# arunsethuraman/multiclust

Measured on AMD Instinct MI355X. Metric: EM iterations/sec, IxLxK admixture, higher is better.
Workload: dtype f64; 1 GPU; c3: 10000 diploid x 100000 loci, M_l~U{2,3,4}, admixture K=8, SQUAREM-3 (-s 3); I=10000, L=100000, T=300302, ploidy=2, K=8, accel_scheme=3, units=1 initialisation(s), one per GPU

## Files before the change

multiclust_amd/csrc/mchip.hip:

```cpp
#include "mchip_context.h"
#include "mchip_finalize.h"

#include <math.h>
#include <stdio.h>
#include <stdlib.h>
#include <string.h>
#include <sys/syscall.h>
#include <unistd.h>

mchip_progress_slot mchip_progress_slots[MCHIP_PROGRESS_SLOTS];
std::atomic<unsigned long long> mchip_progress_events{0};
static std::atomic<int> progress_next_slot{0};

mchip_progress_slot *mchip_progress_my_slot(void)
{
	static thread_local mchip_progress_slot *mine = nullptr;
	if (!mine) {
		int x = progress_next_slot.fetch_add(1, std::memory_order_relaxed);
		if (x >= MCHIP_PROGRESS_SLOTS) x = MCHIP_PROGRESS_SLOTS - 1;
		mine = &mchip_progress_slots[x];
		mine->tid.store((long)syscall(SYS_gettid), std::memory_order_relaxed);
	}
	return mine;
}

#define DECL_KT(n) const mchip_ktable *mchip_ktable_get_##n();
DECL_KT(1) DECL_KT(2) DECL_KT(3) DECL_KT(4) DECL_KT(5) DECL_KT(6) DECL_KT(7) DECL_KT(8)
DECL_KT(9) DECL_KT(10) DECL_KT(11) DECL_KT(12) DECL_KT(13) DECL_KT(14) DECL_KT(15) DECL_KT(16)
DECL_KT(17) DECL_KT(18) DECL_KT(19) DECL_KT(20) DECL_KT(21) DECL_KT(22) DECL_KT(23) DECL_KT(24)
DECL_KT(25) DECL_KT(26) DECL_KT(27) DECL_KT(28) DECL_KT(29) DECL_KT(30) DECL_KT(31) DECL_KT(32)
DECL_KT(33) DECL_KT(34) DECL_KT(35) DECL_KT(36) DECL_KT(37) DECL_KT(38) DECL_KT(39) DECL_KT(40)
DECL_KT(41) DECL_KT(42) DECL_KT(43) DECL_KT(44) DECL_KT(45) DECL_KT(46) DECL_KT(47) DECL_KT(48)
DECL_KT(49) DECL_KT(50) DECL_KT(51) DECL_KT(52) DECL_KT(53) DECL_KT(54) DECL_KT(55) DECL_KT(56)
DECL_KT(57) DECL_KT(58) DECL_KT(59) DECL_KT(60) DECL_KT(61) DECL_KT(62) DECL_KT(63) DECL_KT(64)

const mchip_ktable *mchip_get_ktable(int K)
{
	typedef const mchip_ktable *(*getter)();
	static const getter tabs[MCHIP_MAX_K + 1] = {
		nullptr,
		mchip_ktable_get_1, mchip_ktable_get_2, mchip_ktable_get_3, mchip_ktable_get_4, mchip_ktable_get_5, mchip_ktable_get_6, mchip_ktable_get_7, mchip_ktable_get_8,
		mchip_ktable_get_9, mchip_ktable_get_10, mchip_ktable_get_11, mchip_ktable_get_12, mchip_ktable_get_13, mchip_ktable_get_14, mchip_ktable_get_15, mchip_ktable_get_16,
		mchip_ktable_get_17, mchip_ktable_get_18, mchip_ktable_get_19, mchip_ktable_get_20, mchip_ktable_get_21, mchip_ktable_get_22, mchip_ktable_get_23, mchip_ktable_get_24,
		mchip_ktable_get_25, mchip_ktable_get_26, mchip_ktable_get_27, mchip_ktable_get_28, mchip_ktable_get_29, mchip_ktable_get_30, mchip_ktable_get_31, mchip_ktable_get_32,
		mchip_ktable_get_33, mchip_ktable_get_34, mchip_ktable_get_35, mchip_ktable_get_36, mchip_ktable_get_37, mchip_ktable_get_38, mchip_ktable_get_39, mchip_ktable_get_40,
		mchip_ktable_get_41, mchip_ktable_get_42, mchip_ktable_get_43, mchip_ktable_get_44, mchip_ktable_get_45, mchip_ktable_get_46, mchip_ktable_get_47, mchip_ktable_get_48,
		mchip_ktable_get_49, mchip_ktable_get_50, mchip_ktable_get_51, mchip_ktable_get_52, mchip_ktable_get_53, mchip_ktable_get_54, mchip_ktable_get_55, mchip_ktable_get_56,
		mchip_ktable_get_57, mchip_ktable_get_58, mchip_ktable_get_59, mchip_ktable_get_60, mchip_ktable_get_61, mchip_ktable_get_62, mchip_ktable_get_63, mchip_ktable_get_64,
	};
	static_assert(MCHIP_MAX_K == 64, "one kernel translation unit per K (Makefile: KS)");
	return (K >= 1 && K <= MCHIP_MAX_K) ? tabs[K]() : nullptr;
}

static void read_knobs(mchip_context *ctx)
{
	auto on = [](const char *name) { return getenv(name) != nullptr ? 1 : 0; };
	auto num = [](const char *name, int dflt) { const char *e = getenv(name); return (e && atoi(e) > 0) ? atoi(e) : dflt; };
	ctx->knob.no_bial = on("MCHIP_NO_BIAL");
	ctx->knob.no_counts = on("MCHIP_NO_COUNTS");
	ctx->knob.force_dense = on("MCHIP_FORCE_DENSE");
	ctx->knob.force_safe = on("MCHIP_FORCE_SAFE");
	ctx->knob.no_graph = on("MCHIP_NO_GRAPH");
	ctx->knob.no_dual = on("MCHIP_NO_DUAL");
	ctx->knob.no_slab_sum = on("MCHIP_NO_SLAB_SUM");
	ctx->knob.no_fused_finalize = on("MCHIP_NO_FUSED_FINALIZE");
	ctx->knob.no_pair = on("MCHIP_NO_PAIR");
	ctx->knob.no_col_split = on("MCHIP_NO_COL_SPLIT");
	ctx->knob.part_no_tile = on("MCHIP_PART_NO_TILE");
	ctx->knob.sim_no_tile = on("MCHIP_SIM_NO_TILE");
	const int both = num("MCHIP_BLOCKS_PER_CU", 64);
	ctx->knob.per_cu_col = num("MCHIP_BLOCKS_PER_CU_COL", both);
	ctx->knob.per_cu_ind = num("MCHIP_BLOCKS_PER_CU_IND", both);
	const char *f = getenv("MCHIP_SLAB_FRAC");
	ctx->knob.slab_frac = (f && atof(f) > 0) ? atof(f) : 0.3;
	ctx->knob.no_roundup = on("MCHIP_NO_CHUNK_ROUNDUP");
	ctx->knob.geometry_given = on("MCHIP_BLOCKS_PER_CU") || on("MCHIP_BLOCKS_PER_CU_COL") || on("MCHIP_SLAB_FRAC");
}


constexpr int RT_I = 64;

__global__ __launch_bounds__(256) void k_relayout(const uint8_t *__restrict__ raw, int I, int L, int pl, const int32_t *__restrict__ ua,
			   int limit, uint8_t *gtA, uint8_t *gtS, int n_ltiles, int RT_L, int *bad)
{
	extern __shared__ __attribute__((aligned(16))) uint8_t tile[];
	const int rowb = RT_L * pl;
	const int l0 = (blockIdx.x % n_ltiles) * RT_L, i0 = (blockIdx.x / n_ltiles) * RT_I;
	int flags = 0;
	const int roww = rowb / 4;
	const bool words = ((((size_t)L * pl) | ((size_t)l0 * pl) | (size_t)raw) & 3) == 0 && l0 + RT_L <= L;
	for (int x = threadIdx.x; x < RT_I * roww; x += 256) {
		const int r = x / roww, w = x % roww;
		const int i = i0 + r;
		uint32_t v4 = 0xFFFFFFFFu;
		if (i < I) {
			const uint8_t *src = raw + ((size_t)i * L + l0) * pl + (size_t)w * 4;
			if (words) {
				v4 = *reinterpret_cast<const uint32_t *>(src);
			} else {
				v4 = 0;
				for (int y = 0; y < 4; y++) {
					const int l = l0 + (w * 4 + y) / pl;
					const uint32_t v = l < L ? src[y] : 0xFFu;
					v4 |= v << (8 * y);
				}
			}
			for (int y = 0; y < 4; y++) {
				const int l = l0 + (w * 4 + y) / pl;
				const uint32_t v = (v4 >> (8 * y)) & 0xFFu;
				if (l >= L) continue;
				const int lim = ua ? ua[l] : limit;
				if (v != 0xFFu && (int)v >= lim) flags |= 1;
				if (v == 0xFFu) flags |= 2;
			}
		}
		reinterpret_cast<uint32_t *>(tile)[x] = v4;
	}
	if (flags) atomicOr(bad, flags);
	__syncthreads();
	const int grp = 8 * pl, grpw = 2 * pl;
	for (int x = threadIdx.x; x < (RT_I / 8) * RT_L * grpw; x += 256) {
		const int w = x % grpw, ll = (x / grpw) % RT_L, ibl = x / (grpw * RT_L);
		const int l = l0 + ll;
		const size_t ib = (size_t)(i0 / 8) + ibl;
		if (l >= L || ib * 8 >= (size_t)I) continue;
		uint32_t v4 = 0;
		for (int y = 0; y < 4; y++) {
			const int e = w * 4 + y, j = e / pl, a = e % pl;
			v4 |= (uint32_t)tile[(ibl * 8 + j) * rowb + ll * pl + a] << (8 * y);
		}
		reinterpret_cast<uint32_t *>(gtA + (ib * L + l) * (size_t)grp)[w] = v4;
	}
	for (int x = threadIdx.x; x < (RT_L / 8) * RT_I * grpw; x += 256) {
		const int w = x % grpw, r = (x / grpw) % RT_I, lbl = x / (grpw * RT_I);
		const int i = i0 + r;
		const size_t lb = (size_t)(l0 / 8) + lbl;
		if (i >= I || lb * 8 >= (size_t)L) continue;
		reinterpret_cast<uint32_t *>(gtS + (lb * I + i) * (size_t)grp)[w] = reinterpret_cast<const uint32_t *>(tile + r * rowb + lbl * grp)[w];
	}
}

static int launch_relayout(hipStream_t stream, const uint8_t *raw, int I, int L, int pl, const int32_t *ua, int limit,
			   uint8_t *gtA, uint8_t *gtS, int *bad)
{
	int RT_L = 64;
	while (RT_L > 8 && RT_I * RT_L * pl > 32 * 1024) RT_L -= 8;
	const int n_ltiles = (L + RT_L - 1) / RT_L, n_itiles = (I + RT_I - 1) / RT_I;
	const size_t blocks = (size_t)n_ltiles * n_itiles;
	if (blocks >= ((size_t)1 << 31) || (size_t)RT_I * RT_L * pl > 64 * 1024) return -1;
	hipLaunchKernelGGL(k_relayout, dim3((unsigned)blocks), dim3(256), (size_t)RT_I * RT_L * pl, stream, raw, I, L, pl, ua, limit, gtA, gtS,
			   n_ltiles, RT_L, bad);
	return 0;
}

template <int PLT>
__global__ __launch_bounds__(256) void k_center_distance(const uint8_t *__restrict__ gtS, int I, int L, int pl_rt, int K,
		const int32_t *__restrict__ centers, int chunk_groups, int tile_groups, uint32_t *__restrict__ part)
{
	extern __shared__ uint32_t cd_lds[];
	const int pl = PLT ? PLT : pl_rt, nthr = blockDim.x, tid = threadIdx.x, grp = 8 * pl;
	uint32_t *acc = cd_lds;
	uint32_t *cen32 = acc + (size_t)K * nthr;
	const uint8_t *cen = reinterpret_cast<const uint8_t *>(cen32);
	uint8_t *own = reinterpret_cast<uint8_t *>(cen32 + (size_t)tile_groups * K * 2 * pl);
	const int i = blockIdx.x * nthr + tid;
	const bool live = i < I;
	const int n_groups = (L + 7) >> 3;
	const int g_begin = blockIdx.y * chunk_groups, g_end = n_groups - g_begin < chunk_groups ? n_groups : g_begin + chunk_groups;
	for (int k = 0; k < K; k++) acc[k * nthr + tid] = 0;
	for (int g0 = g_begin; g0 < g_end; g0 += tile_groups) {
		const int ng = g_end - g0 < tile_groups ? g_end - g0 : tile_groups;
		__syncthreads();
		for (int x = tid; x < ng * K * 2 * pl; x += nthr) {
			const int w = x % (2 * pl), k = (x / (2 * pl)) % K, g = x / (2 * pl * K);
			cen32[x] = reinterpret_cast<const uint32_t *>(gtS + ((size_t)(g0 + g) * I + centers[k]) * grp)[w];
		}
		__syncthreads();
		if (!live) continue;
		for (int g = 0; g < ng; g++) {
			const uint8_t *src = gtS + ((size_t)(g0 + g) * I + i) * grp;
			if constexpr (PLT > 0) {
				unsigned long long run[PLT ? PLT : 1];
#pragma unroll
				for (int x = 0; x < PLT; x++) run[x] = reinterpret_cast<const unsigned long long *>(src)[x];
				for (int k = 0; k < K; k++) {
					unsigned long long crun[PLT ? PLT : 1];
#pragma unroll
					for (int x = 0; x < PLT; x++) crun[x] = reinterpret_cast<const unsigned long long *>(cen + (size_t)(g * K + k) * grp)[x];
					int d = 0;
#pragma unroll
					for (int t = 0; t < 8; t++) {
						unsigned used = 0;
#pragma unroll
						for (int b = 0; b < PLT; b++) {
							const int at = t * PLT + b;
							d += ((unsigned)(crun[at >> 3] >> (8 * (at & 7))) & 0xFFu) != MCHIP_MISSING;
						}
#pragma unroll
						for (int a = 0; a < PLT; a++) {
							const int at = t * PLT + a;
							const unsigned gi = (unsigned)(run[at >> 3] >> (8 * (at & 7))) & 0xFFu;
							const bool obs = gi != MCHIP_MISSING;
							bool found = false;
#pragma unroll
							for (int b = 0; b < PLT; b++) {
								const int bt = t * PLT + b;
								const unsigned cb = (unsigned)(crun[bt >> 3] >> (8 * (bt & 7))) & 0xFFu;
								const bool hit = obs && !found && !((used >> b) & 1u) && cb == gi;
								used |= (unsigned)hit << b;
								found = found || hit;
							}
							d += (int)obs - 2 * (int)found;
						}
					}
					acc[k * nthr + tid] += (uint32_t)d;
				}
			} else {
				for (int t = 0; t < 8; t++) {
					for (int a = 0; a < pl; a++) own[a * nthr + tid] = src[t * pl + a];
// ... 73 lines not shown
					for (int y = 0; y < 4; y++) {
						const uint32_t mb = (v4 >> (8 * y)) & 0xFFu;
						const int l = g * 8 + (w * 4 + y) / pl;
						if (mb == MCHIP_MISSING || l >= t1) continue;
						const int c = toff[l] + (int)mb;
						if (tile) atomicAdd(&cc_lds[(size_t)(c - col0) * K + k], 1u);
						else atomicAdd(&cnt[(size_t)c * K + k], 1u);
					}
				}
			}
		if (tile) {
			__syncthreads();
			for (int x = threadIdx.x; x < nwords; x += 256)
				if (cc_lds[x]) atomicAdd(&cnt[(size_t)col0 * K + x], cc_lds[x]);
			__syncthreads();
		}
	}
}

__global__ void k_center_finish(int I, int L, int K, const int32_t *__restrict__ toff, const uint32_t *__restrict__ cnt,
		const uint32_t *__restrict__ nk, double *__restrict__ eta, double *__restrict__ P)
{
	const size_t idx = (size_t)blockIdx.x * blockDim.x + threadIdx.x;
	if (idx < (size_t)K) eta[idx] = (double)(1u + nk[idx]) / (double)(I + K);
	if (idx >= (size_t)K * L) return;
	const int k = (int)(idx % K), l = (int)(idx / K);
	const int c0 = toff[l], M = toff[l + 1] - c0;
	double temp = 0.0;
	for (int m = 0; m < M; m++) temp += 1.0 + (double)(K - k) * (double)cnt[(size_t)(c0 + m) * K + k];
	for (int m = 0; m < M; m++) P[(size_t)(c0 + m) * K + k] = (1.0 + (double)(K - k) * (double)cnt[(size_t)(c0 + m) * K + k]) / temp;
}

__global__ __launch_bounds__(256) void k_assign_by_centers(const uint8_t *__restrict__ gtA, int I, int L, int pl, int K,
		const uint8_t *__restrict__ centers, const unsigned long long *__restrict__ draw_offset,
		const uint8_t *__restrict__ draws, unsigned long long n_draws, uint8_t *raw, int *bad)
{
	const int l = blockIdx.x * 256 + threadIdx.x;
	if (l >= L) return;
	uint8_t cen[MCHIP_MAX_K];
	for (int k = 0; k < K; k++) cen[k] = centers[(size_t)l * K + k];
	unsigned long long next = draw_offset[l];
	for (int ib = 0; ib < (I + 7) / 8; ib++) {
		const uint8_t *src = gtA + ((size_t)ib * L + l) * 8 * (size_t)pl;
		for (int j = 0; j < 8; j++) {
			const int i = ib * 8 + j;
			if (i >= I) break;
			for (int b = 0; b < pl; b++) {
				const uint8_t g = src[j * pl + b];
				int kk = -1;
				if (g != MCHIP_MISSING)
					for (int k = 0; k < K; k++) {
						if (cen[k] == 0xFF) break;
						if (cen[k] == g) { kk = k; break; }
					}
				if (kk < 0) {
					if (K == 1) kk = 0;
					else if (next < n_draws) kk = draws[next++];
					else { kk = 0; atomicOr(bad, 1); }
				}
				raw[((size_t)i * L + l) * pl + b] = (uint8_t)kk;
			}
		}
	}
}

__global__ void k_unlayout(const uint8_t *__restrict__ gtA, int I, int L, int pl, uint8_t *raw)
{
	const size_t n = (size_t)I * L * pl, stride = (size_t)gridDim.x * blockDim.x;
	for (size_t idx = (size_t)blockIdx.x * blockDim.x + threadIdx.x; idx < n; idx += stride) {
		size_t r = idx;
		const int a = (int)(r % pl); r /= pl;
		const int l = (int)(r % L);
		const size_t i = r / L;
		raw[idx] = gtA[(((i >> 3) * L + l) * 8 + (i & 7)) * (size_t)pl + a];
	}
}

template <int BITS>
__global__ void k_build_counts(const uint8_t *__restrict__ gtA, int I, int L, int pl, int T,
			       const int32_t *__restrict__ col_locus, const uint8_t *__restrict__ col_allele, uint4 *gtC)
{
	constexpr int PERWORD = 32 / BITS, G = 4 * PERWORD;
	const size_t idx = (size_t)blockIdx.x * blockDim.x + threadIdx.x;
	const size_t ngroups = (size_t)(I + G - 1) / G;
	if (idx >= ngroups * T) return;
	const int c = (int)(idx % T);
	const size_t g = idx / T;
	const int l = col_locus[c];
	const unsigned m = col_allele[c];
	unsigned out[4] = {0, 0, 0, 0};
	for (int x = 0; x < G; x++) {
		const size_t i = g * G + x;
		if (i >= (size_t)I) break;
		const uint8_t *src = gtA + (((i >> 3) * L + l) * 8 + (i & 7)) * (size_t)pl;
		unsigned n = 0;
		for (int b = 0; b < pl; b++) n += (src[b] == m);
		out[x / PERWORD] |= n << (BITS * (x % PERWORD));
	}
	gtC[idx] = make_uint4(out[0], out[1], out[2], out[3]);
}

__global__ __launch_bounds__(256) void k_count_cells(const uint8_t *__restrict__ gtA, int I, int L, int pl, int T,
		const int32_t *__restrict__ col_locus, const uint8_t *__restrict__ col_allele, unsigned long long *out)
{
	__shared__ unsigned red[2][256];
	const size_t n = (size_t)((I + 7) / 8) * T, stride = (size_t)gridDim.x * 256;
	unsigned cells = 0, copies = 0;
	for (size_t idx = (size_t)blockIdx.x * 256 + threadIdx.x; idx < n; idx += stride) {
		const int c = (int)(idx % T);
		const size_t ib = idx / T;
		const int l = col_locus[c];
		const unsigned m = col_allele[c];
		const uint8_t *src = gtA + (ib * L + l) * 8 * (size_t)pl;
		for (int j = 0; j < 8; j++) {
			unsigned cnt = 0;
			for (int b = 0; b < pl; b++) cnt += (src[j * pl + b] == m);
			cells += cnt != 0;
			copies += cnt;
		}
	}
	red[0][threadIdx.x] = cells;
	red[1][threadIdx.x] = copies;
	__syncthreads();
	for (int w = 128; w > 0; w >>= 1) {
		if ((int)threadIdx.x < w) {
			red[0][threadIdx.x] += red[0][threadIdx.x + w];
			red[1][threadIdx.x] += red[1][threadIdx.x + w];
		}
		__syncthreads();
	}
	if (threadIdx.x == 0) {
		atomicAdd(&out[0], (unsigned long long)red[0][0]);
		atomicAdd(&out[1], (unsigned long long)red[1][0]);
	}
}

__global__ void k_transpose_kt_to_tk(const double *__restrict__ src, double *__restrict__ dst, int K, int T)
{
	const size_t idx = (size_t)blockIdx.x * blockDim.x + threadIdx.x;
	if (idx >= (size_t)K * T) return;
	const int k = (int)(idx % K);
	const size_t c = idx / K;
	dst[idx] = src[(size_t)k * T + c];
}
__global__ void k_transpose_tk_to_kt(const double *__restrict__ src, double *__restrict__ dst, int K, int T)
{
	const size_t idx = (size_t)blockIdx.x * blockDim.x + threadIdx.x;
	if (idx >= (size_t)K * T) return;
	const size_t c = idx % T;
	const int k = (int)(idx / T);
	dst[idx] = src[c * K + k];
}

__device__ __forceinline__ double ordered_sum(double acc, const double *__restrict__ in, size_t first, size_t stride, int count)
{
	int x = 0;
	for (; x + 8 <= count; x += 8) {
		double v[8];
#pragma unroll
		for (int y = 0; y < 8; y++) v[y] = in[first + (size_t)(x + y) * stride];
#pragma unroll
		for (int y = 0; y < 8; y++) acc += v[y];
	}
	for (; x < count; x++) acc += in[first + (size_t)x * stride];
	return acc;
}

__device__ __forceinline__ double block_ordered_sum(const double *__restrict__ in, int n, double *red)
{
	const double s = (int)threadIdx.x < n ? ordered_sum(0.0, in, threadIdx.x, MCHIP_BLOCK, (n - (int)threadIdx.x + MCHIP_BLOCK - 1) / MCHIP_BLOCK) : 0.0;
	red[threadIdx.x] = s;
	__syncthreads();
	for (int w = MCHIP_BLOCK / 2; w > 0; w >>= 1) {
		if ((int)threadIdx.x < w) red[threadIdx.x] += red[threadIdx.x + w];
		__syncthreads();
	}
	const double v = red[0];
	__syncthreads();
	return v;
}
__global__ __launch_bounds__(MCHIP_BLOCK) void k_reduce_sum(const double *__restrict__ in, int n, double *out, const int *stop = nullptr)
{
	__shared__ double red[MCHIP_BLOCK];
	if (stop && *stop) return;
	const double v = block_ordered_sum(in, n, red);
	if (threadIdx.x == 0) *out = v;
}
__global__ __launch_bounds__(MCHIP_BLOCK) void k_reduce_accept(const double *__restrict__ in1, const double *__restrict__ in2, int n, double *sc,
		int *cyc, const int *stop)
{
	__shared__ double red[MCHIP_BLOCK];
	if (stop && *stop) return;
	if (in1) {
		const double v = block_ordered_sum(in1, n, red);
		if (threadIdx.x == 0) sc[1] = v;
	}
	const double v2 = block_ordered_sum(in2, n, red);
	if (threadIdx.x == 0) {
		sc[2] = v2;
		cyc[1] = (!cyc[0] && sc[2] > sc[1]) ? 1 : 0;
	}
}

__global__ __launch_bounds__(MCHIP_BLOCK) void k_reduce_dots(const double *__restrict__ part_q, int gq, const double *__restrict__ part_p, int gp,
		int nout, double *sc, const int *stop)
{
	__shared__ double red[MCHIP_BLOCK];
	if (stop && *stop) return;
	const int x = blockIdx.x;
	const double *in = x < nout ? part_q + (size_t)x * gq : part_p + (size_t)(x - nout) * gp;
	const int n = x < nout ? gq : gp;
	double *out = x < nout ? sc + 16 + x : sc + 20 + (x - nout);
	const double v = block_ordered_sum(in, n, red);
	if (threadIdx.x == 0) *out = v;
}

__global__ __launch_bounds__(MCHIP_BLOCK) void k_sum_slabs(const double *__restrict__ slabs, int n_slabs, size_t n, double *out,
		const int *stop)
{
	__shared__ double part[8][32];
	if (stop && *stop) return;
	const int e_local = threadIdx.x & 31, s = threadIdx.x >> 5;
	const size_t e = (size_t)blockIdx.x * 32 + e_local;
	double acc = 0.0;
	if (e < n && s < n_slabs) acc = ordered_sum(0.0, slabs, (size_t)s * n + e, 8 * n, (n_slabs - s + 7) / 8);
	part[s][e_local] = acc;
	__syncthreads();
	if (s == 0 && e < n) {
		double t = part[0][e_local];
#pragma unroll
		for (int x = 1; x < 8; x++) t += part[x][e_local];
		out[e] = t;
	}
}


__global__ __launch_bounds__(MCHIP_BLOCK) void k_finalize_p(int L, int K, int T, const int32_t *__restrict__ toff,
		int n_ichunks, const double *__restrict__ Apart, const double *Pfrom, double *Pto,
		int weighted, double add_lb, int do_projection, double lb, uint8_t *flags, const int *stop = nullptr)
{
	const size_t idx = (size_t)blockIdx.x * MCHIP_BLOCK + threadIdx.x;
	if (idx >= (size_t)L * K || (stop && *stop)) return;
	const int k = (int)(idx % K);
	const int l = (int)(idx / K);
	const int c0 = toff[l], M = toff[l + 1] - c0;
	double temp = 0.0;
	if (M <= 8) {
		double v[8];
#pragma unroll
		for (int m = 0; m < 8; m++) {
			v[m] = 0.0;
			if (m < M) {
				const size_t e = (size_t)(c0 + m) * K + k;
				double s = ordered_sum(0.0, Apart, e, (size_t)T * K, n_ichunks);
				if (weighted) s *= Pfrom[e];
				s += add_lb;
				v[m] = s;
				temp += s;
			}
		}
#pragma unroll
		for (int m = 0; m < 8; m++)
			if (m < M) v[m] /= temp;
		if (do_projection) michelot_small(v, M, lb);
#pragma unroll
		for (int m = 0; m < 8; m++)
			if (m < M) Pto[(size_t)(c0 + m) * K + k] = v[m];
		return;
	}
	for (int m = 0; m < M; m++) {
		const size_t e = (size_t)(c0 + m) * K + k;
		double s = ordered_sum(0.0, Apart, e, (size_t)T * K, n_ichunks);
		if (weighted) s *= Pfrom[e];
		s += add_lb;
		Pto[e] = s;
		temp += s;
	}
	for (int m = 0; m < M; m++) Pto[(size_t)(c0 + m) * K + k] /= temp;
	if (do_projection) michelot_strided(Pto + (size_t)c0 * K + k, K, M, lb, flags ? flags + (size_t)c0 * K + k : nullptr);
}

__global__ __launch_bounds__(MCHIP_BLOCK) void k_finalize_p_tile(int L, int K, int T, const int32_t *__restrict__ toff, int loci_per_block,
		int n_slabs, const double *__restrict__ Apart, const double *Pfrom, double *Pto,
		int weighted, double add_lb, int do_projection, double lb, const int *stop = nullptr)
{
	__shared__ double tile[FP_TILE];
	if (stop && *stop) return;
	finalize_p_tile_body(blockIdx.x, tile, L, K, T, toff, loci_per_block, n_slabs, Apart, Pfrom, Pto, weighted, add_lb, do_projection, lb);
}

static int finalize_p_loci(int K, int max_M)
{
	if (max_M > 64 || max_M < 1) return 0;
	const int n = FP_TILE / (max_M * K);
	return n >= 4 ? n : 0;
}

__global__ __launch_bounds__(MCHIP_BLOCK) void k_project_p(int L, int K, const int32_t *__restrict__ toff, double *P,
		double lb, uint8_t *flags, const int *stop = nullptr)
{
	const size_t idx = (size_t)blockIdx.x * MCHIP_BLOCK + threadIdx.x;
	if (idx >= (size_t)L * K || (stop && *stop)) return;
	const int k = (int)(idx % K);
	const int l = (int)(idx / K);
	const int c0 = toff[l], M = toff[l + 1] - c0;
	if (M <= 8) {
		double v[8];
#pragma unroll
		for (int m = 0; m < 8; m++) v[m] = m < M ? P[(size_t)(c0 + m) * K + k] : 0.0;
		michelot_small(v, M, lb);
#pragma unroll
		for (int m = 0; m < 8; m++)
			if (m < M) P[(size_t)(c0 + m) * K + k] = v[m];
		return;
	}
	michelot_strided(P + (size_t)c0 * K + k, K, M, lb, flags ? flags + (size_t)c0 * K + k : nullptr);
}

__global__ __launch_bounds__(MCHIP_BLOCK) void k_column_sums(const double *__restrict__ sik, int I, int K, double *out, const int *stop = nullptr)
{
	__shared__ double red[MCHIP_BLOCK];
	if (stop && *stop) return;
	const int k = blockIdx.x;
	double s = 0.0;
	for (int i = threadIdx.x; i < I; i += MCHIP_BLOCK) s += sik[(size_t)i * K + k];
	red[threadIdx.x] = s;
	__syncthreads();
	for (int w = MCHIP_BLOCK / 2; w > 0; w >>= 1) {
		if ((int)threadIdx.x < w) red[threadIdx.x] += red[threadIdx.x + w];
		__syncthreads();
	}
	if (threadIdx.x == 0) out[k] = red[0];
}
__global__ void k_normalize_row(const double *__restrict__ sums, int K, double *eta, const int *stop = nullptr, double add = 0.0)
{
	if (threadIdx.x || blockIdx.x || (stop && *stop)) return;
	double temp = 0.0;
	for (int k = 0; k < K; k++) temp += sums[k] + add;
	for (int k = 0; k < K; k++) eta[k] = (sums[k] + add) / temp;
}

__global__ void k_logp(const double *__restrict__ p, double *__restrict__ out, size_t n, int skip_zero, const int *stop = nullptr)
{
	const size_t idx = (size_t)blockIdx.x * blockDim.x + threadIdx.x;
	if (idx >= n || (stop && *stop)) return;
	const double v = p[idx];
	out[idx] = (skip_zero && v == 0.0) ? 0.0 : log(v);
}

__global__ __launch_bounds__(MCHIP_BLOCK) void k_stop_check(mchip_run_state *s, double *ll, const double *__restrict__ part = nullptr, int n = 0)
{
	__shared__ double red[MCHIP_BLOCK];
	if (s->stopped) return;
	if (part) {
		const double acc = (int)threadIdx.x < n ? ordered_sum(0.0, part, threadIdx.x, MCHIP_BLOCK, (n - (int)threadIdx.x + MCHIP_BLOCK - 1) / MCHIP_BLOCK) : 0.0;
		red[threadIdx.x] = acc;
		__syncthreads();
		for (int w = MCHIP_BLOCK / 2; w > 0; w >>= 1) {
			if ((int)threadIdx.x < w) red[threadIdx.x] += red[threadIdx.x + w];
			__syncthreads();
		}
		if (threadIdx.x == 0) *ll = red[0];
	}
	if (threadIdx.x) return;
	const double loglik = part ? red[0] : *ll;
	s->n_iter++;
	if (loglik != loglik) {
		s->fatal = 1;
		s->bad_loglik = loglik;
		s->stopped = 1;
		return;
	}
	int stop;
	if (s->max_iter && s->n_iter > s->max_iter) {
		s->iter_stop = 1;
		stop = 1;
	} else {
		double abs_diff = 0, rel_diff = 0;
		stop = 1;
		if (s->abs_error != 0) abs_diff = fabs(loglik - s->logL);
		if (s->rel_error != 0) rel_diff = abs_diff / fabs(s->logL);
		if (s->abs_error != 0 && abs_diff > s->abs_error) stop = 0;
		if (s->rel_error != 0 && rel_diff > s->rel_error) stop = 0;
		if (stop) s->converged = 1;
	}
	s->stopped = stop;
	if (loglik < s->logL && !stop) {
		s->fatal = 2;
		s->bad_loglik = loglik;
		s->stopped = 1;
		return;
	}
	s->logL = loglik;
}

__global__ void k_diff(const double *__restrict__ a, const double *__restrict__ b, double *out, size_t n, const int *stop = nullptr)
{
	const size_t idx = (size_t)blockIdx.x * blockDim.x + threadIdx.x;
	if (stop && *stop) return;
	if (idx < n) out[idx] = a[idx] - b[idx];
}

__global__ __launch_bounds__(MCHIP_BLOCK) void k_dots(const double *__restrict__ u, const double *__restrict__ v,
		const double *__restrict__ u2, size_t n, int mode, double *part, const int *stop = nullptr)
{
	__shared__ double red[3][MCHIP_BLOCK];
	if (stop && *stop) return;
	double s0 = 0, s1 = 0, s2 = 0;
	for (size_t x = (size_t)blockIdx.x * MCHIP_BLOCK + threadIdx.x; x < n; x += (size_t)gridDim.x * MCHIP_BLOCK) {
		if (mode == 0) {
			const double uu = u[x], d = v[x] - uu;
			s0 += uu * uu; s1 += uu * d; s2 += d * d;
		} else {
			const double uu = u[x];
			s0 += uu * u2[x]; s1 += uu * v[x];
		}
	}
	red[0][threadIdx.x] = s0; red[1][threadIdx.x] = s1; red[2][threadIdx.x] = s2;
	__syncthreads();
	for (int w = MCHIP_BLOCK / 2; w > 0; w >>= 1) {
		if ((int)threadIdx.x < w) {
			red[0][threadIdx.x] += red[0][threadIdx.x + w];
			red[1][threadIdx.x] += red[1][threadIdx.x + w];
			red[2][threadIdx.x] += red[2][threadIdx.x + w];
		}
		__syncthreads();
	}
	if (threadIdx.x == 0) {
		part[blockIdx.x] = red[0][0];
		part[gridDim.x + blockIdx.x] = red[1][0];
		part[2 * gridDim.x + blockIdx.x] = red[2][0];
	}
}

__device__ __forceinline__ void dots_slots_body(const double *__restrict__ x0, const double *__restrict__ x1, const double *__restrict__ x2,
		size_t n, double *part, unsigned bid, unsigned gdim, double (*red)[MCHIP_BLOCK])
{
	double s0 = 0, s1 = 0, s2 = 0;
	for (size_t x = (size_t)bid * MCHIP_BLOCK + threadIdx.x; x < n; x += (size_t)gdim * MCHIP_BLOCK) {
		const double uu = x1[x] - x0[x], vv = x2[x] - x1[x];
		const double d = vv - uu;
		s0 += uu * uu; s1 += uu * d; s2 += d * d;
	}
	red[0][threadIdx.x] = s0; red[1][threadIdx.x] = s1; red[2][threadIdx.x] = s2;
	__syncthreads();
	for (int w = MCHIP_BLOCK / 2; w > 0; w >>= 1) {
		if ((int)threadIdx.x < w) {
			red[0][threadIdx.x] += red[0][threadIdx.x + w];
			red[1][threadIdx.x] += red[1][threadIdx.x + w];
			red[2][threadIdx.x] += red[2][threadIdx.x + w];
		}
		__syncthreads();
	}
	if (threadIdx.x == 0) {
		part[bid] = red[0][0];
		part[gdim + bid] = red[1][0];
		part[2 * gdim + bid] = red[2][0];
	}
}
__global__ __launch_bounds__(MCHIP_BLOCK) void k_dots_slots(const double *__restrict__ q0, const double *__restrict__ q1,
		const double *__restrict__ q2, size_t nq, double *part_q, unsigned gq, const double *__restrict__ p0,
		const double *__restrict__ p1, const double *__restrict__ p2, size_t np, double *part_p, const int *stop)
{
	__shared__ double red[3][MCHIP_BLOCK];
	if (stop && *stop) return;
	if (blockIdx.x < gq) dots_slots_body(q0, q1, q2, nq, part_q, blockIdx.x, gq, red);
	else dots_slots_body(p0, p1, p2, np, part_p, blockIdx.x - gq, gridDim.x - gq, red);
}
__global__ void k_accel_update_slots(const double *__restrict__ q0, const double *q1, const double *__restrict__ q2, double *qout, size_t nq,
				     const double *__restrict__ p0, const double *p1, const double *__restrict__ p2, double *pout, size_t np,
				     int qn_form, const double *s_dev, const int *stop)
{
#pragma clang fp contract(off)
	size_t idx = (size_t)blockIdx.x * blockDim.x + threadIdx.x;
	if (idx >= nq + np || (stop && *stop)) return;
	const double *x0 = q0, *x1 = q1, *x2 = q2;
	double *out = qout;
	if (idx >= nq) { idx -= nq; x0 = p0; x1 = p1; x2 = p2; out = pout; }
	const double s = *s_dev;
	const double u = x1[idx] - x0[idx], v = x2[idx] - x1[idx];
	if (qn_form) out[idx] = x0[idx] + u + s * v;
	else out[idx] = x0[idx] - 2 * s * u + s * s * (v - u);
}

__global__ void k_accel_update(const double *__restrict__ base, const double *__restrict__ u, const double *__restrict__ v,
			       double *out, size_t n, double s, int qn_form, const double *s_dev = nullptr, const int *stop = nullptr)
{
#pragma clang fp contract(off)
	const size_t idx = (size_t)blockIdx.x * blockDim.x + threadIdx.x;
	if (idx >= n || (stop && *stop)) return;
	if (s_dev) s = *s_dev;
	if (qn_form) out[idx] = base[idx] + u[idx] + s * v[idx];
	else out[idx] = base[idx] - 2 * s * u[idx] + s * s * (v[idx] - u[idx]);
}
__global__ void k_axpy2(const double *__restrict__ v, double *out, size_t n, double ca, double cb)
{
#pragma clang fp contract(off)
	const size_t idx = (size_t)blockIdx.x * blockDim.x + threadIdx.x;
	if (idx < n) out[idx] += v[idx] * ca * cb;
}
__global__ void k_add(const double *__restrict__ a, const double *__restrict__ b, double *out, size_t n)
{
	const size_t idx = (size_t)blockIdx.x * blockDim.x + threadIdx.x;
	if (idx < n) out[idx] = a[idx] + b[idx];
}

__device__ __forceinline__ void step_size_body(double *sc, int scheme, int *cyc)
{
	const double utu = sc[16] + sc[20], utvu = sc[17] + sc[21], vutvu = sc[18] + sc[22];
	double s;
	if (scheme == 1) s = utu / utvu;
	else if (scheme == 2) s = utvu / vutvu;
	else if (scheme == 3) s = (sqrt(utu) < 1e-8) ? (double)NAN : -sqrt(utu / vutvu);
	else s = -utu / utvu;
	if (scheme < 4 && s > -1) s = -1;
	sc[24] = s;
	cyc[0] = (s != s || s - s != 0.0) ? 1 : 0;
}
__global__ __launch_bounds__(MCHIP_BLOCK) void k_reduce_dots_step(const double *__restrict__ part_q, int gq, const double *__restrict__ part_p,
		int gp, double *sc, int scheme, int *cyc, const int *stop)
{
	__shared__ double red[MCHIP_BLOCK];
	if (stop && *stop) return;
	for (int x = 0; x < 6; x++) {
		const double *in = x < 3 ? part_q + (size_t)x * gq : part_p + (size_t)(x - 3) * gp;
		const int n = x < 3 ? gq : gp;
		const double v = block_ordered_sum(in, n, red);
		if (threadIdx.x == 0) sc[(x < 3 ? 16 : 20) + (x % 3)] = v;
	}
	if (threadIdx.x == 0) step_size_body(sc, scheme, cyc);
}
__global__ void k_accept(const double *sc, int *cyc, const int *stop)
{
	if (threadIdx.x || blockIdx.x || (stop && *stop)) return;
	cyc[1] = (!cyc[0] && sc[2] > sc[1]) ? 1 : 0;
}

__global__ void k_select_copy(double *qdst, const double *__restrict__ q_if_accepted, const double *__restrict__ q_otherwise, size_t nq,
			      double *pdst, const double *__restrict__ p_if_accepted, const double *__restrict__ p_otherwise, size_t np,
			      const int *cyc, const int *stop)
{
	size_t idx = (size_t)blockIdx.x * blockDim.x + threadIdx.x;
	if (idx >= nq + np || (stop && *stop)) return;
	if (idx < nq) qdst[idx] = cyc[1] ? q_if_accepted[idx] : q_otherwise[idx];
	else { idx -= nq; pdst[idx] = cyc[1] ? p_if_accepted[idx] : p_otherwise[idx]; }
}

int check_slot(mchip_context *ctx, int slot)
{
	if (!ctx) return MCHIP_ERR_INVALID;
	if (!ctx->K) return fail(ctx, MCHIP_ERR_STATE, "no model set%s", nullptr);
	if (slot < 0 || slot > 2) return fail(ctx, MCHIP_ERR_INVALID, "slot out of range%s", nullptr);
	return MCHIP_OK;
}

static void prof_mark(mchip_context *ctx, int kind, bool start)
{
	if (!ctx->profiling) return;
	if (ctx->ev_used >= ctx->ev_pool.size()) {
		hipEvent_t e;
		if (hipEventCreate(&e) != hipSuccess) return;
		ctx->ev_pool.push_back(e);
	}
	(void)hipEventRecord(ctx->ev_pool[ctx->ev_used++], ctx->stream);
	if (start) ctx->ev_kind.push_back(kind);
}

constexpr size_t PAIR_SPAN_CHUNK = 1024;
constexpr int PAIR_SPAN_THREADS = 1024;
__global__ __launch_bounds__(PAIR_SPAN_THREADS) void k_pair_spans(const unsigned long long *__restrict__ marks, unsigned n_blocks, mchip_pair_runs runs,
								  mchip_pair_span *out)
{
	__shared__ unsigned long long red[4][PAIR_SPAN_THREADS];
	unsigned long long lo[2] = { ~0ull, ~0ull }, hi[2] = { 0ull, 0ull };
	for (unsigned r = threadIdx.x; r < n_blocks / MCHIP_PAIR_RUN; r += PAIR_SPAN_THREADS) {
		unsigned logical;
		const int kind = mchip_pair_is_ind(r * MCHIP_PAIR_RUN, runs, &logical) ? 1 : 0;
#pragma unroll
		for (int x = 0; x < MCHIP_PAIR_RUN; x++) {
			const size_t b = (size_t)r * MCHIP_PAIR_RUN + x;
			const unsigned long long t0 = marks[2 * b], t1 = marks[2 * b + 1];
			if (t0 > t1) continue;
			lo[kind] = t0 < lo[kind] ? t0 : lo[kind];
			hi[kind] = t1 > hi[kind] ? t1 : hi[kind];
		}
	}
	red[0][threadIdx.x] = lo[0]; red[1][threadIdx.x] = lo[1]; red[2][threadIdx.x] = hi[0]; red[3][threadIdx.x] = hi[1];
	__syncthreads();
	for (int s = PAIR_SPAN_THREADS / 2; s > 0; s >>= 1) {
		if ((int)threadIdx.x < s) {
			for (int x = 0; x < 2; x++) {
				const unsigned long long l2 = red[x][threadIdx.x + s], h2 = red[2 + x][threadIdx.x + s];
				if (l2 < red[x][threadIdx.x]) red[x][threadIdx.x] = l2;
				if (h2 > red[2 + x][threadIdx.x]) red[2 + x][threadIdx.x] = h2;
			}
		}
		__syncthreads();
	}
	if (threadIdx.x == 0) {
		out->start[0] = red[0][0]; out->start[1] = red[1][0];
		out->end[0] = red[2][0]; out->end[1] = red[3][0];
	}
}

static int pair_profile_slot(mchip_context *ctx, const mchip_pass_args &a, unsigned long long **marks)
{
	mchip_pair_runs runs;
	const size_t n_blocks = ctx->kt->pair_blocks(a, &runs);
	if (n_blocks > ctx->pair_marks_cap) {
		HIPCHK(hipStreamSynchronize(ctx->stream));
		dfree(ctx->d_pair_marks);
		ctx->pair_marks_cap = 0;
		HIPCHK(hipMalloc((void **)&ctx->d_pair_marks, 2 * n_blocks * sizeof(unsigned long long)));
		ctx->pair_marks_cap = n_blocks;
	}
	if (ctx->pair_used / PAIR_SPAN_CHUNK >= ctx->pair_spans.size()) {
		mchip_pair_span *chunk = nullptr;
		HIPCHK(hipMalloc((void **)&chunk, PAIR_SPAN_CHUNK * sizeof(mchip_pair_span)));
		ctx->pair_spans.push_back(chunk);
	}
	*marks = ctx->d_pair_marks;
	return MCHIP_OK;
}

static void drop_graphs(mchip_context *ctx)
{
	for (int s = 0; s < 3; s++)
		if (ctx->step_graph[s]) { (void)MCHIP_WAIT(hipGraphExecDestroy(ctx->step_graph[s])); ctx->step_graph[s] = nullptr; }
	for (int s = 0; s < 3; s++)
		for (int m = 0; m < 5; m++)
			if (ctx->cycle_graph[s][m]) { (void)MCHIP_WAIT(hipGraphExecDestroy(ctx->cycle_graph[s][m])); ctx->cycle_graph[s][m] = nullptr; }
}

void free_model(mchip_context *ctx)
{
	drop_graphs(ctx);
	for (int s = 0; s < 3; s++) { dfree(ctx->d_p[s]); dfree(ctx->d_q[s]); }
	for (int s = 0; s < MCHIP_MAX_SECANTS; s++) { dfree(ctx->d_up[s]); dfree(ctx->d_vp[s]); dfree(ctx->d_uq[s]); dfree(ctx->d_vq[s]); }
	dfree(ctx->d_sik); dfree(ctx->d_stage); dfree(ctx->d_logp); dfree(ctx->d_Apart); dfree(ctx->d_Spart); dfree(ctx->d_llpart); dfree(ctx->d_llpart2);
	dfree(ctx->d_redpart); dfree(ctx->d_flags);
	ctx->K = 0;
	ctx->parked_K = 0;
	ctx->kt = nullptr;
	ctx->have_ll = 0;
	ctx->s_cache_slot = -1;
}

void drop_saved(saved_set &set)
{
	dfree(set.d_raw);
	set.L = 0;
	set.ua.clear();
	set.empty.clear();
}

void free_data(mchip_context *ctx, int keep)
{
	drop_cv(ctx);
	drop_generators(ctx);
	if (!(keep & KEEP_RS_BASE)) drop_saved(ctx->rs_base);
	dfree(ctx->d_ua); dfree(ctx->d_toff); dfree(ctx->d_col_locus); dfree(ctx->d_col_allele);
	dfree(ctx->d_gtA); dfree(ctx->d_gtS); dfree(ctx->d_gtC); dfree(ctx->d_asA); dfree(ctx->d_asS);
	dfree(ctx->d_initA); dfree(ctx->d_initS);
	dfree(ctx->d_draw);
	dfree(ctx->d_cand_span); dfree(ctx->d_cand_centers); dfree(ctx->d_cand_off);
	ctx->cand_span_bytes = ctx->cand_loci = ctx->cand_center_bytes = 0;
	dfree(ctx->d_cen_part); dfree(ctx->d_cen_work);
	ctx->cen_part_bytes = ctx->cen_work_bytes = 0;
	ctx->init_geno_set = 0;
	ctx->h_ua.clear();
	ctx->I = ctx->L = ctx->T = 0;
}

static mchip_pass_args pass_args(mchip_context *ctx, int slot)
{
	mchip_pass_args a;
	memset(&a, 0, sizeof a);
	a.I = ctx->I; a.L = ctx->L; a.T = ctx->T; a.ploidy = ctx->ploidy; a.K = ctx->K;
	a.gtA = ctx->d_gtA; a.gtS = ctx->d_gtS; a.gtC = ctx->d_gtC; a.count_bits = ctx->count_bits; a.has_missing = ctx->has_missing;
	a.ua = ctx->d_ua; a.toff = ctx->d_toff; a.col_locus = ctx->d_col_locus; a.col_allele = ctx->d_col_allele;
	a.P = ctx->d_p[slot]; a.Q = ctx->d_q[slot]; a.qstride = ctx->qstride;
	a.ichunk = ctx->ichunk; a.n_ichunks = ctx->n_ichunks; a.Apart = ctx->d_Apart; a.llpart = ctx->d_llpart;
	a.flush_blocks = ctx->flush_blocks;
	a.safe_rcp = ctx->safe_rcp;
	a.lchunk = ctx->lchunk; a.n_lchunks = ctx->n_lchunks; a.Spart = ctx->d_Spart;
	a.asA = ctx->d_asA; a.asS = ctx->d_asS;
	a.sparse = ctx->sparse; a.tile_cols = 8 * ctx->max_M;
	a.biallelic = (ctx->min_M == 2 && ctx->max_M == 2 && !ctx->knob.no_bial) ? 1 : 0;
	a.ind_waves = ctx->ind_waves;
	a.xcd_rows = ctx->xcd_rows;
	a.no_col_split = ctx->knob.no_col_split;
	return a;
}

static void launch_finalize_p(mchip_context *ctx, int n_slabs, const double *slabs, int from, int to, int weighted, double add_lb,
			      int do_projection, const int *stop)
{
	const int per = finalize_p_loci(ctx->K, ctx->max_M);
	if (per)
		hipLaunchKernelGGL(k_finalize_p_tile, dim3((ctx->L + per - 1) / per), dim3(MCHIP_BLOCK), 0, ctx->stream,
				   ctx->L, ctx->K, ctx->T, ctx->d_toff, per, n_slabs, slabs, ctx->d_p[from], ctx->d_p[to],
				   weighted, add_lb, do_projection, ctx->p_lb, stop);
	else
		hipLaunchKernelGGL(k_finalize_p, dim3(nblk((size_t)ctx->L * ctx->K)), dim3(MCHIP_BLOCK), 0, ctx->stream,
				   ctx->L, ctx->K, ctx->T, ctx->d_toff, n_slabs, slabs, ctx->d_p[from], ctx->d_p[to],
				   weighted, add_lb, do_projection, ctx->p_lb, ctx->d_flags, stop);
}

extern "C" {

int mchip_abi_version(void) { return MCHIP_ABI_VERSION; }

int mchip_device_count(int *count)
{
	MCHIP_ENTRY();
	if (!count) return MCHIP_ERR_INVALID;
	int n = 0;
	if (MCHIP_WAIT(hipGetDeviceCount(&n)) != hipSuccess) n = 0;
	*count = n;
	return MCHIP_OK;
}

int mchip_create(mchip_context **out, int device)
{
	MCHIP_ENTRY();
	if (!out) return MCHIP_ERR_INVALID;
	*out = nullptr;
	int n = 0;
	if (MCHIP_WAIT(hipGetDeviceCount(&n)) != hipSuccess || n <= 0) return MCHIP_ERR_NO_DEVICE;
	if (device < 0 || device >= n) return MCHIP_ERR_INVALID;
	mchip_context *ctx = new mchip_context();
	ctx->first_empty = -1;
	ctx->cv_fold = -1;
	ctx->device = device;
	ctx->err[0] = 0;
	ctx->ind_waves = 1;
	read_knobs(ctx);
	if (MCHIP_WAIT(hipSetDevice(device)) != hipSuccess || MCHIP_WAIT(hipStreamCreateWithFlags(&ctx->stream, hipStreamNonBlocking)) != hipSuccess) {
		delete ctx;
		return MCHIP_ERR_HIP;
	}
	hipDeviceProp_t prop;
	ctx->n_cu = (MCHIP_WAIT(hipGetDeviceProperties(&prop, device)) == hipSuccess) ? prop.multiProcessorCount : 256;
	if (MCHIP_WAIT(hipHostMalloc((void **)&ctx->h_pinned, 64 * sizeof(double), hipHostMallocDefault)) != hipSuccess ||
	    MCHIP_WAIT(hipMalloc((void **)&ctx->d_scalars, 64 * sizeof(double))) != hipSuccess ||
	    MCHIP_WAIT(hipMalloc((void **)&ctx->d_run, sizeof(mchip_run_state))) != hipSuccess ||
	    MCHIP_WAIT(hipMalloc((void **)&ctx->d_cyc, 4 * sizeof(int))) != hipSuccess ||
	    MCHIP_WAIT(hipEventCreate(&ctx->ev_begin)) != hipSuccess || MCHIP_WAIT(hipEventCreate(&ctx->ev_end)) != hipSuccess) {
		delete ctx;
		return MCHIP_ERR_ALLOC;
	}
	*out = ctx;
	return MCHIP_OK;
}

int mchip_destroy(mchip_context *ctx)
{
	MCHIP_ENTRY();
	if (!ctx) return MCHIP_OK;
	(void)MCHIP_WAIT(hipSetDevice(ctx->device));
	(void)MCHIP_WAIT(hipStreamSynchronize(ctx->stream));
	free_model(ctx);
	free_data(ctx);
	dfree(ctx->d_scalars);
	dfree(ctx->d_cyc);
	dfree(ctx->d_run);
	if (ctx->h_pinned) (void)MCHIP_WAIT(hipHostFree(ctx->h_pinned));
	for (hipEvent_t e : ctx->ev_pool) (void)MCHIP_WAIT(hipEventDestroy(e));
	dfree(ctx->d_pair_marks);
	for (mchip_pair_span *&chunk : ctx->pair_spans) dfree(chunk);
	(void)MCHIP_WAIT(hipEventDestroy(ctx->ev_begin));
	(void)MCHIP_WAIT(hipEventDestroy(ctx->ev_end));
	(void)MCHIP_WAIT(hipStreamDestroy(ctx->stream));
	delete ctx;
	return MCHIP_OK;
}

const char *mchip_last_error(const mchip_context *ctx) { return ctx ? ctx->err : "null context"; }

int mchip_synchronize(mchip_context *ctx)
{
	MCHIP_ENTRY();
	if (!ctx) return MCHIP_ERR_INVALID;
	HIPCHK(hipStreamSynchronize(ctx->stream));
	return MCHIP_OK;
}

int mchip_device_info(mchip_context *ctx, char *name, int name_len, int *compute_units, double *hbm_bytes)
{
	MCHIP_ENTRY();
	if (!ctx) return MCHIP_ERR_INVALID;
	hipDeviceProp_t prop;
	HIPCHK(hipGetDeviceProperties(&prop, ctx->device));
	if (name && name_len > 0) snprintf(name, name_len, "%s (%s)", prop.name, prop.gcnArchName);
	if (compute_units) *compute_units = prop.multiProcessorCount;
	if (hbm_bytes) *hbm_bytes = (double)prop.totalGlobalMem;
	return MCHIP_OK;
}

}

static int set_shape_impl(mchip_context *ctx, int I, int L, int ploidy, const int32_t *ua, int keep)
{
	if (I <= 0 || L <= 0 || ploidy <= 0 || ploidy > 64 || !ua)
		return fail(ctx, MCHIP_ERR_INVALID, "set_genotypes: bad shape or null pointer%s", nullptr);
	read_knobs(ctx);
	HIPCHK(hipSetDevice(ctx->device));
	HIPCHK(hipStreamSynchronize(ctx->stream));
	drop_cv(ctx);
	if (!(keep & KEEP_RS_BASE)) drop_saved(ctx->rs_base);
	if (ctx->T && ctx->I == I && ctx->L == L && ctx->ploidy == ploidy && (int)ctx->h_ua.size() == L &&
	    !memcmp(ctx->h_ua.data(), ua, sizeof(int32_t) * (size_t)L)) {
		if (ctx->K) ctx->parked_K = ctx->K;
		ctx->K = 0;
		ctx->have_ll = 0;
		ctx->s_cache_slot = -1;
		if (!(keep & KEEP_INIT)) ctx->init_geno_set = 0;
		return MCHIP_OK;
	}
	free_model(ctx);
	free_data(ctx, keep);

	std::vector<int32_t> toff(L + 25);
	toff[0] = 0;
	int maxM = 0, minM = 1 << 30;
	for (int l = 0; l < L; l++) {
		if (ua[l] < minM) minM = ua[l];
		if (ua[l] < 0 || ua[l] > 255) return fail(ctx, MCHIP_ERR_INVALID, "uniquealleles[l] must be in [0,255]%s", nullptr);
		if ((long long)toff[l] + ua[l] > 2000000000LL) return fail(ctx, MCHIP_ERR_INVALID, "too many allele columns%s", nullptr);
		toff[l + 1] = toff[l] + ua[l];
		if (ua[l] > maxM) maxM = ua[l];
	}
	const int T = toff[L];
	for (int x = L + 1; x < L + 25; x++) toff[x] = T;
	if (T <= 0) return fail(ctx, MCHIP_ERR_INVALID, "no alleles%s", nullptr);
	std::vector<int32_t> col_locus(T);
	std::vector<uint8_t> col_allele(T);
	for (int l = 0; l < L; l++)
		for (int m = 0; m < ua[l]; m++) {
			col_locus[toff[l] + m] = l;
			col_allele[toff[l] + m] = (uint8_t)m;
		}
	ctx->I = I; ctx->L = L; ctx->ploidy = ploidy; ctx->T = T; ctx->max_M = maxM; ctx->min_M = minM;
	ctx->h_ua.assign(ua, ua + L);
	ctx->geno_bytes_A = (size_t)((I + 7) / 8) * L * 8 * ploidy;
	ctx->geno_bytes_S = (size_t)((L + 7) / 8) * I * 8 * ploidy;
	HIPCHK(hipMalloc((void **)&ctx->d_ua, sizeof(int32_t) * L));
	HIPCHK(hipMalloc((void **)&ctx->d_toff, sizeof(int32_t) * (L + 25)));
	HIPCHK(hipMalloc((void **)&ctx->d_col_locus, sizeof(int32_t) * T));
	HIPCHK(hipMalloc((void **)&ctx->d_col_allele, T));
	HIPCHK(hipMalloc((void **)&ctx->d_gtA, ctx->geno_bytes_A));
	HIPCHK(hipMalloc((void **)&ctx->d_gtS, ctx->geno_bytes_S));
	HIPCHK(hipMemcpyAsync(ctx->d_ua, ua, sizeof(int32_t) * L, hipMemcpyHostToDevice, ctx->stream));
	HIPCHK(hipMemcpyAsync(ctx->d_toff, toff.data(), sizeof(int32_t) * (L + 25), hipMemcpyHostToDevice, ctx->stream));
	HIPCHK(hipMemcpyAsync(ctx->d_col_locus, col_locus.data(), sizeof(int32_t) * T, hipMemcpyHostToDevice, ctx->stream));
	HIPCHK(hipMemcpyAsync(ctx->d_col_allele, col_allele.data(), T, hipMemcpyHostToDevice, ctx->stream));
	HIPCHK(hipStreamSynchronize(ctx->stream));
	return MCHIP_OK;
}

int set_shape(mchip_context *ctx, int I, int L, int ploidy, const int32_t *ua, int keep)
{
	const int rc = set_shape_impl(ctx, I, L, ploidy, ua, keep);
	if (rc == MCHIP_ERR_HIP || rc == MCHIP_ERR_ALLOC) {
		free_model(ctx);
		free_data(ctx, keep);
	}
	return rc;
}

int stream_buffer(mchip_context *ctx)
{
	if (ctx->d_draw) return MCHIP_OK;
	const size_t n = (size_t)ctx->I * ctx->L * ctx->ploidy;
	HIPCHK(hipMalloc((void **)&ctx->d_draw, ((n + RNG_CHUNK - 1) / RNG_CHUNK) * RNG_CHUNK));
	return MCHIP_OK;
}

int install_layouts(mchip_context *ctx, int has_missing)
{
	const int I = ctx->I, L = ctx->L, ploidy = ctx->ploidy, T = ctx->T;
	if (ctx->has_missing != has_missing) drop_graphs(ctx);
	ctx->has_missing = has_missing;
	ctx->counts_valid = 0;
	ctx->count_bits = ploidy <= 3 ? 2 : (ploidy <= 15 ? 4 : 0);
	if (ctx->knob.no_counts) ctx->count_bits = 0;
	if (ctx->count_bits) {
		const int G = 128 / ctx->count_bits;
		const size_t nwords = (size_t)((I + G - 1) / G) * T;
		if (!ctx->d_gtC) HIPCHK(hipMalloc((void **)&ctx->d_gtC, nwords * 16));
		if (ctx->count_bits == 2)
			hipLaunchKernelGGL(k_build_counts<2>, dim3(nblk(nwords)), dim3(256), 0, ctx->stream, ctx->d_gtA, I, L, ploidy, T,
					   ctx->d_col_locus, ctx->d_col_allele, (uint4 *)ctx->d_gtC);
		else
			hipLaunchKernelGGL(k_build_counts<4>, dim3(nblk(nwords)), dim3(256), 0, ctx->stream, ctx->d_gtA, I, L, ploidy, T,
					   ctx->d_col_locus, ctx->d_col_allele, (uint4 *)ctx->d_gtC);
		HIPCHK(hipGetLastError());
		HIPCHK(hipStreamSynchronize(ctx->stream));
	}
	return MCHIP_OK;
}

int install_raw(mchip_context *ctx, const uint8_t *d_raw)
{
	const int I = ctx->I, L = ctx->L, ploidy = ctx->ploidy;
	int *d_bad = bad_flag(ctx);
	HIPCHK(hipMemsetAsync(d_bad, 0, sizeof(int), ctx->stream));
	if (launch_relayout(ctx->stream, d_raw, I, L, ploidy, ctx->d_ua, 0, ctx->d_gtA, ctx->d_gtS, d_bad))
		return fail(ctx, MCHIP_ERR_UNSUPPORTED, "data set too large for the layout kernel%s", nullptr);
	HIPCHK(hipGetLastError());
	int bad = 0;
	HIPCHK(hipMemcpyAsync(&bad, d_bad, sizeof(int), hipMemcpyDeviceToHost, ctx->stream));
	HIPCHK(hipStreamSynchronize(ctx->stream));
	if (bad & 1) {
		free_data(ctx);
		return fail(ctx, MCHIP_ERR_INVALID, "genotype allele index >= uniquealleles[l]%s", nullptr);
	}
	return install_layouts(ctx, (bad & 2) ? 1 : 0);
}

void set_empty_rows(mchip_context *ctx, std::vector<int> rows)
{
// ... 334 lines not shown
int mchip_q_length(const mchip_context *ctx, int *n)
{
	MCHIP_ENTRY();
	if (!ctx || !n || !ctx->K) return MCHIP_ERR_STATE;
	*n = ctx->nq;
	return MCHIP_OK;
}
int mchip_p_length(const mchip_context *ctx, int *n)
{
	MCHIP_ENTRY();
	if (!ctx || !n || !ctx->K) return MCHIP_ERR_STATE;
	*n = ctx->K * ctx->T;
	return MCHIP_OK;
}

int mchip_set_p(mchip_context *ctx, int slot, const double *p)
{
	MCHIP_ENTRY();
	int rc = check_slot(ctx, slot);
	if (rc) return rc;
	ctx->s_cache_slot = -1;
	if (!p) return fail(ctx, MCHIP_ERR_INVALID, "null pointer%s", nullptr);
	const size_t KT = (size_t)ctx->K * ctx->T;
	HIPCHK(hipSetDevice(ctx->device));
	HIPCHK(hipMemcpyAsync(ctx->d_stage, p, KT * sizeof(double), hipMemcpyHostToDevice, ctx->stream));
	hipLaunchKernelGGL(k_transpose_kt_to_tk, dim3(nblk(KT)), dim3(256), 0, ctx->stream, ctx->d_stage, ctx->d_p[slot], ctx->K, ctx->T);
	HIPCHK(hipGetLastError());
	HIPCHK(hipStreamSynchronize(ctx->stream));
	return MCHIP_OK;
}

int mchip_get_p(mchip_context *ctx, int slot, double *p)
{
	MCHIP_ENTRY();
	int rc = check_slot(ctx, slot);
	if (rc) return rc;
	if (!p) return fail(ctx, MCHIP_ERR_INVALID, "null pointer%s", nullptr);
	const size_t KT = (size_t)ctx->K * ctx->T;
	HIPCHK(hipSetDevice(ctx->device));
	hipLaunchKernelGGL(k_transpose_tk_to_kt, dim3(nblk(KT)), dim3(256), 0, ctx->stream, ctx->d_p[slot], ctx->d_stage, ctx->K, ctx->T);
	HIPCHK(hipGetLastError());
	HIPCHK(hipMemcpyAsync(p, ctx->d_stage, KT * sizeof(double), hipMemcpyDeviceToHost, ctx->stream));
	HIPCHK(hipStreamSynchronize(ctx->stream));
	return MCHIP_OK;
}

int mchip_set_q(mchip_context *ctx, int slot, const double *q)
{
	MCHIP_ENTRY();
	int rc = check_slot(ctx, slot);
	if (rc) return rc;
	ctx->s_cache_slot = -1;
	if (!q) return fail(ctx, MCHIP_ERR_INVALID, "null pointer%s", nullptr);
	HIPCHK(hipSetDevice(ctx->device));
	int nan_rows = 0;
	if (ctx->qstride)
		for (int i : ctx->empty_rows)
			for (int k = 0; k < ctx->K; k++) nan_rows |= (q[(size_t)i * ctx->K + k] != q[(size_t)i * ctx->K + k]);
	if (nan_rows) {
		std::vector<double> clean(q, q + ctx->nq);
		for (int i : ctx->empty_rows) {
			bool bad = false;
			for (int k = 0; k < ctx->K; k++) bad |= (clean[(size_t)i * ctx->K + k] != clean[(size_t)i * ctx->K + k]);
			if (bad)
				for (int k = 0; k < ctx->K; k++) clean[(size_t)i * ctx->K + k] = 1.0 / ctx->K;
		}
		HIPCHK(hipMemcpyAsync(ctx->d_q[slot], clean.data(), (size_t)ctx->nq * sizeof(double), hipMemcpyHostToDevice, ctx->stream));
		HIPCHK(hipStreamSynchronize(ctx->stream));
	} else {
		HIPCHK(hipMemcpyAsync(ctx->d_q[slot], q, (size_t)ctx->nq * sizeof(double), hipMemcpyHostToDevice, ctx->stream));
		HIPCHK(hipStreamSynchronize(ctx->stream));
	}
	ctx->empty_rows_nan[slot] = nan_rows;
	return MCHIP_OK;
}

int mchip_get_q(mchip_context *ctx, int slot, double *q)
{
	MCHIP_ENTRY();
	int rc = check_slot(ctx, slot);
	if (rc) return rc;
	if (!q) return fail(ctx, MCHIP_ERR_INVALID, "null pointer%s", nullptr);
	HIPCHK(hipSetDevice(ctx->device));
	HIPCHK(hipMemcpyAsync(q, ctx->d_q[slot], (size_t)ctx->nq * sizeof(double), hipMemcpyDeviceToHost, ctx->stream));
	HIPCHK(hipStreamSynchronize(ctx->stream));
	if (ctx->qstride && ctx->empty_rows_nan[slot])
		for (int i : ctx->empty_rows)
			for (int k = 0; k < ctx->K; k++) q[(size_t)i * ctx->K + k] = -__builtin_nan("");
	return MCHIP_OK;
}

int mchip_empty_individuals(const mchip_context *ctx, int *first)
{
	MCHIP_ENTRY();
	if (!ctx) return 0;
	if (first) *first = ctx->first_empty;
	return (int)ctx->empty_rows.size();
}

static int fetch_scalars(mchip_context *ctx, int first, int count, double *out)
{
	HIPCHK(hipMemcpyAsync(ctx->h_pinned, ctx->d_scalars + first, count * sizeof(double), hipMemcpyDeviceToHost, ctx->stream));
	HIPCHK(hipStreamSynchronize(ctx->stream));
	for (int x = 0; x < count; x++) out[x] = ctx->h_pinned[x];
	return MCHIP_OK;
}

static int finalize_shared_eta(mchip_context *ctx, int to, const int *stop = nullptr, double add = 0.0, int project = 1)
{
	hipLaunchKernelGGL(k_column_sums, dim3(ctx->K), dim3(MCHIP_BLOCK), 0, ctx->stream, ctx->d_sik, ctx->I, ctx->K, ctx->d_scalars + 8, stop);
	hipLaunchKernelGGL(k_normalize_row, dim3(1), dim3(64), 0, ctx->stream, ctx->d_scalars + 8, ctx->K, ctx->d_q[to], stop, add);
	if (ctx->do_projection && project) ctx->kt->project_q(1, ctx->K, ctx->d_q[to], ctx->eta_lb, stop, ctx->stream);
	HIPCHK(hipGetLastError());
	return MCHIP_OK;
}

static int run_mixture(mchip_context *ctx, int from, int to, int do_mstep, int mode, const int *stop = nullptr, int ll_slot = -1,
		       bool defer_ll = false)
{
	if (ll_slot < 0) ll_slot = mode ? 1 : 0;
	const size_t KT = (size_t)ctx->K * ctx->T;
	hipLaunchKernelGGL(k_logp, dim3(nblk(KT)), dim3(256), 0, ctx->stream, ctx->d_p[from], ctx->d_logp, KT, mode == 0, stop);
	mchip_pass_args a = pass_args(ctx, from);
	a.P = ctx->d_logp;
	a.stop = stop;
	prof_mark(ctx, mode == 0 ? MCHIP_KERN_ACCUM_Q : MCHIP_KERN_LOGLIK, true);
	ctx->kt->mix_gather(a, ctx->stream);
	prof_mark(ctx, mode == 0 ? MCHIP_KERN_ACCUM_Q : MCHIP_KERN_LOGLIK, false);
	const int nb = (ctx->I + MCHIP_BLOCK - 1) / MCHIP_BLOCK;
	ctx->kt->mix_finalize(ctx->I, ctx->n_lchunks, ctx->d_Spart, ctx->d_q[from], ctx->d_sik, ctx->d_llpart, mode, stop, ctx->stream);
	ctx->ll_parts = nb;
	if (!defer_ll)
		hipLaunchKernelGGL(k_reduce_sum, dim3(1), dim3(MCHIP_BLOCK), 0, ctx->stream, ctx->d_llpart, nb, ctx->d_scalars + ll_slot, stop);
	if (do_mstep) {
		int rc = finalize_shared_eta(ctx, to, stop);
		if (rc) return rc;
		mchip_pass_args b = pass_args(ctx, from);
		b.Q = ctx->d_sik;
		b.qstride = ctx->K;
		b.stop = stop;
		prof_mark(ctx, MCHIP_KERN_ACCUM_P, true);
		ctx->kt->mix_column(b, ctx->stream);
		prof_mark(ctx, MCHIP_KERN_ACCUM_P, false);
		launch_finalize_p(ctx, ctx->kt->col_slabs(b, 1), ctx->d_Apart, from, to, 0, ctx->p_lb, ctx->do_projection, stop);
	}
	HIPCHK(hipGetLastError());
	if (mode == 0) ctx->have_ll = 1;
	return MCHIP_OK;
}

static int run_estep(mchip_context *ctx, int from, int to, int do_mstep, const int *stop = nullptr, const int *skip_ind = nullptr,
		     bool defer_ll = false)
{
	if (!ctx->admixture) return run_mixture(ctx, from, to, do_mstep, 0, stop, -1, defer_ll);
	mchip_pass_args a = pass_args(ctx, from);
	a.stop = stop;
	a.skip_ind = skip_ind;
	const bool s_cached = ctx->sparse && do_mstep && !stop && ctx->s_cache_slot == from;
	const bool paired = do_mstep && !s_cached && !ctx->knob.no_pair && ctx->kt->pair_available(a);
	if (paired) {
		unsigned long long *marks = nullptr;
		if (ctx->profiling) {
			int rc = pair_profile_slot(ctx, a, &marks);
			if (rc) return rc;
		}
		ctx->kt->estep_pair(a, marks, ctx->stream);
		if (marks) {
			mchip_pair_runs runs;
			const unsigned n_blocks = ctx->kt->pair_blocks(a, &runs);
			hipLaunchKernelGGL(k_pair_spans, dim3(1), dim3(PAIR_SPAN_THREADS), 0, ctx->stream, marks, n_blocks, runs,
					   ctx->pair_spans[ctx->pair_used / PAIR_SPAN_CHUNK] + ctx->pair_used % PAIR_SPAN_CHUNK);
			ctx->pair_used++;
		}
		ctx->ll_parts = ctx->kt->ind_ll_parts(a);
		if (!defer_ll)
			hipLaunchKernelGGL(k_reduce_sum, dim3(1), dim3(MCHIP_BLOCK), 0, ctx->stream, ctx->d_llpart, ctx->ll_parts, ctx->d_scalars, stop);
	}
	if (!paired && (do_mstep || !ctx->sparse)) {
		prof_mark(ctx, MCHIP_KERN_ACCUM_P, true);
		if (do_mstep) ctx->kt->accum_p(a, ctx->stream); else ctx->kt->loglik(a, ctx->stream);
		prof_mark(ctx, MCHIP_KERN_ACCUM_P, false);
	}
	if (paired) {
	} else if (s_cached) {
		HIPCHK(hipMemcpyAsync(ctx->d_scalars, ctx->d_scalars + 2, sizeof(double), hipMemcpyDeviceToDevice, ctx->stream));
	} else {
		prof_mark(ctx, MCHIP_KERN_ACCUM_Q, true);
		ctx->kt->accum_q(a, ctx->stream);
		prof_mark(ctx, MCHIP_KERN_ACCUM_Q, false);
		ctx->ll_parts = ctx->kt->ind_ll_parts(a);
		if (!defer_ll)
			hipLaunchKernelGGL(k_reduce_sum, dim3(1), dim3(MCHIP_BLOCK), 0, ctx->stream, ctx->d_llpart, ctx->ll_parts, ctx->d_scalars, stop);
	}
	ctx->s_cache_slot = -1;
	const int indiv = ctx->qstride != 0;
	const int s_slabs = ctx->kt->ind_slabs(a), n_slabs = ctx->kt->col_slabs(a, 0);
	const int p_loci = finalize_p_loci(ctx->K, ctx->max_M);
	if (do_mstep && indiv && p_loci && !(n_slabs > 8 && !ctx->knob.no_slab_sum) && !ctx->knob.no_fused_finalize) {
		mchip_finalize_p_args p;
		p.L = ctx->L; p.K = ctx->K; p.T = ctx->T; p.loci_per_block = p_loci; p.n_slabs = n_slabs; p.weighted = 1;
		p.do_projection = ctx->do_projection; p.toff = ctx->d_toff; p.Apart = ctx->d_Apart; p.Pfrom = ctx->d_p[from];
		p.Pto = ctx->d_p[to]; p.add_lb = 0.0; p.lb = ctx->p_lb;
		ctx->kt->finalize_qp(ctx->I, s_slabs, ctx->d_Spart, ctx->d_q[from], ctx->qstride, ctx->d_q[to], ctx->d_sik,
				     ctx->do_projection, ctx->eta_lb, p, stop, ctx->stream);
		ctx->empty_rows_nan[to] = 1;
		HIPCHK(hipGetLastError());
		ctx->have_ll = 1;
		return MCHIP_OK;
	}
	ctx->kt->finalize_q(ctx->I, ctx->K, s_slabs, ctx->d_Spart, ctx->d_q[from], ctx->qstride,
			    ctx->d_q[to], ctx->d_sik, do_mstep && indiv, 1, ctx->do_projection, ctx->eta_lb, stop, ctx->stream, 0.0);
	if (do_mstep && indiv) ctx->empty_rows_nan[to] = 1;
	if (do_mstep) {
		if (!indiv) {
			int rc = finalize_shared_eta(ctx, to, stop);
			if (rc) return rc;
		}
		if (n_slabs > 8 && !ctx->knob.no_slab_sum) {
			const size_t n = (size_t)ctx->K * ctx->T;
			hipLaunchKernelGGL(k_sum_slabs, dim3(nblk(n, 32)), dim3(MCHIP_BLOCK), 0, ctx->stream, ctx->d_Apart, n_slabs, n, ctx->d_stage, stop);
			launch_finalize_p(ctx, 1, ctx->d_stage, from, to, 1, 0.0, ctx->do_projection, stop);
		} else {
			launch_finalize_p(ctx, n_slabs, ctx->d_Apart, from, to, 1, 0.0, ctx->do_projection, stop);
		}
	}
	HIPCHK(hipGetLastError());
	ctx->have_ll = 1;
	return MCHIP_OK;
}

int mchip_em_run(mchip_context *ctx, int slot, int n_steps, mchip_run_state *state)
{
	MCHIP_ENTRY();
	int rc = check_slot(ctx, slot);
	if (rc) return rc;
	if (!state || n_steps < 1) return fail(ctx, MCHIP_ERR_INVALID, "em_run: bad arguments%s", nullptr);
	if (ctx->qstride) ctx->empty_rows_nan[slot] = 1;
	HIPCHK(hipSetDevice(ctx->device));
	HIPCHK(hipMemcpyAsync(ctx->d_run, state, sizeof *state, hipMemcpyHostToDevice, ctx->stream));
	const int *stop = &ctx->d_run->stopped;
	bool use_graph = !ctx->profiling && n_steps >= 4 && !ctx->knob.no_graph;
	if (use_graph && !ctx->step_graph[slot]) {
		hipGraph_t graph = nullptr;
		if (MCHIP_WAIT(hipStreamBeginCapture(ctx->stream, hipStreamCaptureModeThreadLocal)) == hipSuccess) {
			rc = run_estep(ctx, slot, slot, 1, stop, nullptr, true);
			hipLaunchKernelGGL(k_stop_check, dim3(1), dim3(MCHIP_BLOCK), 0, ctx->stream, ctx->d_run, ctx->d_scalars, ctx->d_llpart, ctx->ll_parts);
			const hipError_t e = MCHIP_WAIT(hipStreamEndCapture(ctx->stream, &graph));
			if (rc || e != hipSuccess || !graph || MCHIP_WAIT(hipGraphInstantiate(&ctx->step_graph[slot], graph, nullptr, nullptr, 0)) != hipSuccess)
				ctx->step_graph[slot] = nullptr;
			if (graph) (void)MCHIP_WAIT(hipGraphDestroy(graph));
			(void)hipGetLastError();
		}
		if (!ctx->step_graph[slot]) use_graph = false;
	}
	for (int s = 0; s < n_steps; s++) {
		if (use_graph) {
			HIPCHK(hipGraphLaunch(ctx->step_graph[slot], ctx->stream));
			continue;
		}
		if ((rc = run_estep(ctx, slot, slot, 1, stop, nullptr, true))) return rc;
		hipLaunchKernelGGL(k_stop_check, dim3(1), dim3(MCHIP_BLOCK), 0, ctx->stream, ctx->d_run, ctx->d_scalars, ctx->d_llpart, ctx->ll_parts);
	}
	HIPCHK(hipGetLastError());
	HIPCHK(hipMemcpyAsync(state, ctx->d_run, sizeof *state, hipMemcpyDeviceToHost, ctx->stream));
	HIPCHK(hipStreamSynchronize(ctx->stream));
	return MCHIP_OK;
}

int mchip_em_step(mchip_context *ctx, int from, int to, double *loglik)
{
	MCHIP_ENTRY();
	int rc = check_slot(ctx, from);
	if (rc) return rc;
	if ((rc = check_slot(ctx, to))) return rc;
	HIPCHK(hipSetDevice(ctx->device));
	if ((rc = run_estep(ctx, from, to, 1))) return rc;
	if (ctx->qstride) ctx->empty_rows_nan[to] = 1;
	if (loglik) return fetch_scalars(ctx, 0, 1, loglik);
	return MCHIP_OK;
}

int mchip_last_loglik(mchip_context *ctx, double *loglik)
{
	MCHIP_ENTRY();
	if (!ctx || !loglik) return MCHIP_ERR_INVALID;
	if (!ctx->have_ll) return fail(ctx, MCHIP_ERR_STATE, "no log likelihood computed yet%s", nullptr);
	HIPCHK(hipSetDevice(ctx->device));
	return fetch_scalars(ctx, 0, 1, loglik);
}

int mchip_e_step(mchip_context *ctx, int slot, double *loglik)
{
	MCHIP_ENTRY();
	int rc = check_slot(ctx, slot);
	if (rc) return rc;
	HIPCHK(hipSetDevice(ctx->device));
	if ((rc = run_estep(ctx, slot, slot, 0))) return rc;
	if (loglik) return fetch_scalars(ctx, 0, 1, loglik);
	return MCHIP_OK;
}

int mchip_loglik(mchip_context *ctx, int slot, double *loglik)
{
	MCHIP_ENTRY();
	int rc = check_slot(ctx, slot);
	if (rc) return rc;
	HIPCHK(hipSetDevice(ctx->device));
	if (!ctx->admixture) {
		if ((rc = run_mixture(ctx, slot, slot, 0, 1))) return rc;
		if (loglik) return fetch_scalars(ctx, 1, 1, loglik);
		return MCHIP_OK;
	}
	mchip_pass_args a = pass_args(ctx, slot);
	prof_mark(ctx, MCHIP_KERN_LOGLIK, true);
	ctx->kt->loglik(a, ctx->stream);
	prof_mark(ctx, MCHIP_KERN_LOGLIK, false);
	hipLaunchKernelGGL(k_reduce_sum, dim3(1), dim3(MCHIP_BLOCK), 0, ctx->stream, ctx->d_llpart, ctx->kt->ind_ll_parts(a), ctx->d_scalars + 1);
	HIPCHK(hipGetLastError());
	if (loglik) return fetch_scalars(ctx, 1, 1, loglik);
	return MCHIP_OK;
}

int mchip_loglik_prefetch(mchip_context *ctx, int slot, double *loglik)
{
	MCHIP_ENTRY();
	int rc = check_slot(ctx, slot);
	if (rc) return rc;
	if (!ctx->admixture || !ctx->sparse) return mchip_loglik(ctx, slot, loglik);
	HIPCHK(hipSetDevice(ctx->device));
	mchip_pass_args a = pass_args(ctx, slot);
	prof_mark(ctx, MCHIP_KERN_ACCUM_Q, true);
	ctx->kt->accum_q(a, ctx->stream);
	prof_mark(ctx, MCHIP_KERN_ACCUM_Q, false);
	hipLaunchKernelGGL(k_reduce_sum, dim3(1), dim3(MCHIP_BLOCK), 0, ctx->stream, ctx->d_llpart, ctx->kt->ind_ll_parts(a), ctx->d_scalars + 2);
	HIPCHK(hipGetLastError());
	ctx->s_cache_slot = slot;
	if (loglik) return fetch_scalars(ctx, 2, 1, loglik);
	return MCHIP_OK;
}

}

int partition_finalize(mchip_context *ctx, int to, int counts, int n_aslabs)
{
	int rc;
	const int indiv = ctx->qstride != 0;
	const int project = counts ? 0 : ctx->do_projection;
	const double add = counts ? 1.0 : 0.0;
	ctx->empty_rows_nan[to] = counts ? 0 : (ctx->qstride ? 1 : 0);
	ctx->kt->finalize_q(ctx->I, ctx->K, ctx->n_lchunks, ctx->d_Spart, ctx->d_q[to], ctx->qstride,
			    ctx->d_q[to], ctx->d_sik, indiv, 0, project, ctx->eta_lb, nullptr, ctx->stream, add);
	if (!indiv && (rc = finalize_shared_eta(ctx, to, nullptr, add, !counts))) return rc;
	hipLaunchKernelGGL(k_finalize_p, dim3(nblk((size_t)ctx->L * ctx->K)), dim3(MCHIP_BLOCK), 0, ctx->stream,
			   ctx->L, ctx->K, ctx->T, ctx->d_toff, n_aslabs, ctx->d_Apart, ctx->d_p[to], ctx->d_p[to],
			   0, add, project, ctx->p_lb, ctx->d_flags);
	HIPCHK(hipGetLastError());
	HIPCHK(hipStreamSynchronize(ctx->stream));
	return MCHIP_OK;
}

int partition_mstep(mchip_context *ctx, const uint8_t *d_raw, int to, int counts)
{
	if (!ctx->d_asA) HIPCHK(hipMalloc((void **)&ctx->d_asA, ctx->geno_bytes_A));
	if (!ctx->d_asS) HIPCHK(hipMalloc((void **)&ctx->d_asS, ctx->geno_bytes_S));
	int *d_bad = bad_flag(ctx);
	HIPCHK(hipMemsetAsync(d_bad, 0, sizeof(int), ctx->stream));
	if (launch_relayout(ctx->stream, d_raw, ctx->I, ctx->L, ctx->ploidy, nullptr, ctx->K, ctx->d_asA, ctx->d_asS, d_bad))
		return fail(ctx, MCHIP_ERR_UNSUPPORTED, "data set too large for the layout kernel%s", nullptr);
	HIPCHK(hipGetLastError());
	int bad = 0;
	HIPCHK(hipMemcpyAsync(&bad, d_bad, sizeof(int), hipMemcpyDeviceToHost, ctx->stream));
	HIPCHK(hipStreamSynchronize(ctx->stream));
	if (bad) return fail(ctx, MCHIP_ERR_INVALID, "partition assignment >= K%s", nullptr);

	mchip_pass_args a = pass_args(ctx, to);
	if (ctx->init_geno_set) {
		a.gtA = ctx->d_initA;
		a.gtS = ctx->d_initS;
	}
	a.part_counts = counts;
	ctx->kt->part_p(a, ctx->stream);
	ctx->kt->part_q(a, ctx->stream);
	return partition_finalize(ctx, to, counts, ctx->n_ichunks);
}

int check_partition_call(mchip_context *ctx, const void *arg, int to)
{
	int rc = check_slot(ctx, to);
	if (rc) return rc;
	ctx->s_cache_slot = -1;
	if (!arg) return fail(ctx, MCHIP_ERR_INVALID, "null pointer%s", nullptr);
	if (!ctx->admixture) return fail(ctx, MCHIP_ERR_STATE, "allele partitions initialise the admixture model only%s", nullptr);
	return MCHIP_OK;
}

void launch_reduce_sum(mchip_context *ctx, const double *in, int n, double *out)
{
	hipLaunchKernelGGL(k_reduce_sum, dim3(1), dim3(MCHIP_BLOCK), 0, ctx->stream, in, n, out, (const int *)nullptr);
}

extern "C" {

int mchip_mstep_from_partition(mchip_context *ctx, const uint8_t *assign, int to)
{
	MCHIP_ENTRY();
	int rc = check_partition_call(ctx, assign, to);
	if (rc) return rc;
	HIPCHK(hipSetDevice(ctx->device));
	const size_t raw_bytes = (size_t)ctx->I * ctx->L * ctx->ploidy;
	scoped_dev<uint8_t> d_raw;
	HIPCHK(d_raw.alloc(raw_bytes));
	HIPCHK(hipMemcpyAsync(d_raw, assign, raw_bytes, hipMemcpyHostToDevice, ctx->stream));
	return partition_mstep(ctx, d_raw, to);
}
// ... 122 lines not shown
			   ctx->d_p[to]);
	HIPCHK(hipGetLastError());
	ctx->empty_rows_nan[to] = 0;
	if (assign_out) HIPCHK(hipMemcpyAsync(assign_out, d_assign, sizeof(int32_t) * (size_t)I, hipMemcpyDeviceToHost, ctx->stream));
	HIPCHK(hipStreamSynchronize(ctx->stream));
	return MCHIP_OK;
}

int mchip_get_expected_counts(mchip_context *ctx, double *sik)
{
	MCHIP_ENTRY();
	if (!ctx || !sik) return MCHIP_ERR_INVALID;
	if (!ctx->K) return fail(ctx, MCHIP_ERR_STATE, "no model set%s", nullptr);
	HIPCHK(hipSetDevice(ctx->device));
	HIPCHK(hipMemcpyAsync(sik, ctx->d_sik, (size_t)ctx->I * ctx->K * sizeof(double), hipMemcpyDeviceToHost, ctx->stream));
	HIPCHK(hipStreamSynchronize(ctx->stream));
	return MCHIP_OK;
}

static int check_secant(mchip_context *ctx, int j)
{
	if (!ctx) return MCHIP_ERR_INVALID;
	if (!ctx->K) return fail(ctx, MCHIP_ERR_STATE, "no model set%s", nullptr);
	if (j < 0 || j >= ctx->nsec) return fail(ctx, MCHIP_ERR_INVALID, "secant index out of range%s", nullptr);
	return MCHIP_OK;
}

int mchip_set_secant(mchip_context *ctx, int which, int j, const double *p_part, const double *q_part)
{
	MCHIP_ENTRY();
	int rc = check_secant(ctx, j);
	if (rc) return rc;
	if (!p_part || !q_part || (which != 0 && which != 1)) return fail(ctx, MCHIP_ERR_INVALID, "set_secant: bad arguments%s", nullptr);
	const size_t KT = (size_t)ctx->K * ctx->T;
	HIPCHK(hipSetDevice(ctx->device));
	HIPCHK(hipMemcpyAsync(ctx->d_stage, p_part, KT * sizeof(double), hipMemcpyHostToDevice, ctx->stream));
	hipLaunchKernelGGL(k_transpose_kt_to_tk, dim3(nblk(KT)), dim3(256), 0, ctx->stream, ctx->d_stage, which ? ctx->d_vp[j] : ctx->d_up[j], ctx->K, ctx->T);
	HIPCHK(hipGetLastError());
	HIPCHK(hipMemcpyAsync(which ? ctx->d_vq[j] : ctx->d_uq[j], q_part, (size_t)ctx->nq * sizeof(double), hipMemcpyHostToDevice, ctx->stream));
	HIPCHK(hipStreamSynchronize(ctx->stream));
	return MCHIP_OK;
}
int mchip_get_secant(mchip_context *ctx, int which, int j, double *p_part, double *q_part)
{
	MCHIP_ENTRY();
	int rc = check_secant(ctx, j);
	if (rc) return rc;
	if (!p_part || !q_part || (which != 0 && which != 1)) return fail(ctx, MCHIP_ERR_INVALID, "get_secant: bad arguments%s", nullptr);
	const size_t KT = (size_t)ctx->K * ctx->T;
	HIPCHK(hipSetDevice(ctx->device));
	hipLaunchKernelGGL(k_transpose_tk_to_kt, dim3(nblk(KT)), dim3(256), 0, ctx->stream, which ? ctx->d_vp[j] : ctx->d_up[j], ctx->d_stage, ctx->K, ctx->T);
	HIPCHK(hipGetLastError());
	HIPCHK(hipMemcpyAsync(p_part, ctx->d_stage, KT * sizeof(double), hipMemcpyDeviceToHost, ctx->stream));
	HIPCHK(hipMemcpyAsync(q_part, which ? ctx->d_vq[j] : ctx->d_uq[j], (size_t)ctx->nq * sizeof(double), hipMemcpyDeviceToHost, ctx->stream));
	HIPCHK(hipStreamSynchronize(ctx->stream));
	return MCHIP_OK;
}

int mchip_secant(mchip_context *ctx, int which, int j, int to, int from)
{
	MCHIP_ENTRY();
	int rc = check_secant(ctx, j);
	if (rc) return rc;
	if ((rc = check_slot(ctx, to)) || (rc = check_slot(ctx, from))) return rc;
	HIPCHK(hipSetDevice(ctx->device));
	const size_t KT = (size_t)ctx->K * ctx->T;
	double *dp = which ? ctx->d_vp[j] : ctx->d_up[j];
	double *dq = which ? ctx->d_vq[j] : ctx->d_uq[j];
	hipLaunchKernelGGL(k_diff, dim3(nblk(KT)), dim3(256), 0, ctx->stream, ctx->d_p[to], ctx->d_p[from], dp, KT);
	hipLaunchKernelGGL(k_diff, dim3(nblk(ctx->nq)), dim3(256), 0, ctx->stream, ctx->d_q[to], ctx->d_q[from], dq, (size_t)ctx->nq);
	HIPCHK(hipGetLastError());
	return MCHIP_OK;
}

static void dots_enqueue(mchip_context *ctx, const double *uq, const double *vq, const double *u2q,
			 const double *up, const double *vp, const double *u2p, int mode, int nout, const int *stop = nullptr)
{
	const size_t KT = (size_t)ctx->K * ctx->T;
	const int gq = (int)((ctx->nq + 4095) / 4096) > 512 ? 512 : (int)((ctx->nq + 4095) / 4096);
	const int gp = (int)((KT + 4095) / 4096) > 512 ? 512 : (int)((KT + 4095) / 4096);
	double *part_q = ctx->d_redpart, *part_p = ctx->d_redpart + 3 * 512;
	hipLaunchKernelGGL(k_dots, dim3(gq), dim3(MCHIP_BLOCK), 0, ctx->stream, uq, vq, u2q, (size_t)ctx->nq, mode, part_q, stop);
	hipLaunchKernelGGL(k_dots, dim3(gp), dim3(MCHIP_BLOCK), 0, ctx->stream, up, vp, u2p, KT, mode, part_p, stop);
	hipLaunchKernelGGL(k_reduce_dots, dim3(2 * nout), dim3(MCHIP_BLOCK), 0, ctx->stream, part_q, gq, part_p, gp, nout, ctx->d_scalars, stop);
}

static int dots_common(mchip_context *ctx, const double *uq, const double *vq, const double *u2q,
		       const double *up, const double *vp, const double *u2p, int mode, int nout, double *out)
{
	dots_enqueue(ctx, uq, vq, u2q, up, vp, u2p, mode, nout);
	HIPCHK(hipGetLastError());
	double tmp[8];
	int rc = fetch_scalars(ctx, 16, 8, tmp);
	if (rc) return rc;
	for (int x = 0; x < nout; x++) out[x] = tmp[x] + tmp[4 + x];
	return MCHIP_OK;
}

int mchip_step_dots(mchip_context *ctx, int j, double *out3)
{
	MCHIP_ENTRY();
	int rc = check_secant(ctx, j);
	if (rc) return rc;
	if (!out3) return MCHIP_ERR_INVALID;
	HIPCHK(hipSetDevice(ctx->device));
	return dots_common(ctx, ctx->d_uq[j], ctx->d_vq[j], nullptr, ctx->d_up[j], ctx->d_vp[j], nullptr, 0, 3, out3);
}

int mchip_secant_dots(mchip_context *ctx, int j1, int j2, double *out2)
{
	MCHIP_ENTRY();
	int rc = check_secant(ctx, j1);
	if (rc) return rc;
	if ((rc = check_secant(ctx, j2))) return rc;
	if (!out2) return MCHIP_ERR_INVALID;
	HIPCHK(hipSetDevice(ctx->device));
	return dots_common(ctx, ctx->d_uq[j1], ctx->d_vq[j2], ctx->d_uq[j2], ctx->d_up[j1], ctx->d_vp[j2], ctx->d_up[j2], 1, 2, out2);
}

static int project_slot(mchip_context *ctx, int to, const int *stop = nullptr)
{
	if (!ctx->do_projection) return MCHIP_OK;
	hipLaunchKernelGGL(k_project_p, dim3(nblk((size_t)ctx->L * ctx->K)), dim3(MCHIP_BLOCK), 0, ctx->stream,
			   ctx->L, ctx->K, ctx->d_toff, ctx->d_p[to], ctx->p_lb, ctx->d_flags, stop);
	ctx->kt->project_q(ctx->qstride ? ctx->I : 1, ctx->K, ctx->d_q[to], ctx->eta_lb, stop, ctx->stream);
	HIPCHK(hipGetLastError());
	return MCHIP_OK;
}

int mchip_accel_update(mchip_context *ctx, int to, int base, int j, double s, int qn_form)
{
	MCHIP_ENTRY();
	int rc = check_secant(ctx, j);
	if (rc) return rc;
	ctx->s_cache_slot = -1;
	if ((rc = check_slot(ctx, to)) || (rc = check_slot(ctx, base))) return rc;
	HIPCHK(hipSetDevice(ctx->device));
	const size_t KT = (size_t)ctx->K * ctx->T;
	hipLaunchKernelGGL(k_accel_update, dim3(nblk(KT)), dim3(256), 0, ctx->stream, ctx->d_p[base], ctx->d_up[j], ctx->d_vp[j], ctx->d_p[to], KT, s, qn_form);
	hipLaunchKernelGGL(k_accel_update, dim3(nblk(ctx->nq)), dim3(256), 0, ctx->stream, ctx->d_q[base], ctx->d_uq[j], ctx->d_vq[j], ctx->d_q[to], (size_t)ctx->nq, s, qn_form);
	HIPCHK(hipGetLastError());
	ctx->empty_rows_nan[to] = ctx->empty_rows_nan[base];
	return project_slot(ctx, to);
}

static int accel_cycle_enqueue(mchip_context *ctx, int A, int scheme)
{
	const int B = (A + 1) % 3, C = (A + 2) % 3;
	const int *stop = &ctx->d_run->stopped;
	int *cyc = ctx->d_cyc;
	const size_t KT = (size_t)ctx->K * ctx->T, nq = (size_t)ctx->nq;
	int rc;
	if ((rc = run_estep(ctx, A, B, 1, stop, cyc + 1, true))) return rc;
	hipLaunchKernelGGL(k_stop_check, dim3(1), dim3(MCHIP_BLOCK), 0, ctx->stream, ctx->d_run, ctx->d_scalars, ctx->d_llpart, ctx->ll_parts);
	if ((rc = run_estep(ctx, B, C, 1, stop, nullptr, true))) return rc;
	hipLaunchKernelGGL(k_stop_check, dim3(1), dim3(MCHIP_BLOCK), 0, ctx->stream, ctx->d_run, ctx->d_scalars, ctx->d_llpart, ctx->ll_parts);
	mchip_pass_args dual = pass_args(ctx, B);
	dual.stop = stop;
	dual.P2 = ctx->d_p[C];
	dual.Q2 = ctx->d_q[C];
	dual.llpart2 = ctx->d_llpart2;
	const bool use_dual = ctx->admixture && !ctx->knob.no_dual && ctx->kt->dual_available(dual);
	if (!ctx->admixture) {
		if ((rc = run_mixture(ctx, C, C, 0, 1, stop, 1))) return rc;
	} else if (!use_dual) {
		mchip_pass_args a = pass_args(ctx, C);
		a.stop = stop;
		prof_mark(ctx, MCHIP_KERN_LOGLIK, true);
		ctx->kt->loglik(a, ctx->stream);
		prof_mark(ctx, MCHIP_KERN_LOGLIK, false);
		hipLaunchKernelGGL(k_reduce_sum, dim3(1), dim3(MCHIP_BLOCK), 0, ctx->stream, ctx->d_llpart, ctx->kt->ind_ll_parts(a), ctx->d_scalars + 1, stop);
	}
	{
		const int gq = (int)((ctx->nq + 4095) / 4096) > 512 ? 512 : (int)((ctx->nq + 4095) / 4096);
		const int gp = (int)((KT + 4095) / 4096) > 512 ? 512 : (int)((KT + 4095) / 4096);
		double *part_q = ctx->d_redpart, *part_p = ctx->d_redpart + 3 * 512;
		hipLaunchKernelGGL(k_dots_slots, dim3(gq + gp), dim3(MCHIP_BLOCK), 0, ctx->stream, ctx->d_q[A], ctx->d_q[B], ctx->d_q[C], nq, part_q, (unsigned)gq,
				   ctx->d_p[A], ctx->d_p[B], ctx->d_p[C], KT, part_p, stop);
		hipLaunchKernelGGL(k_reduce_dots_step, dim3(1), dim3(MCHIP_BLOCK), 0, ctx->stream, part_q, gq, part_p, gp, ctx->d_scalars, scheme, cyc, stop);
	}
	hipLaunchKernelGGL(k_accel_update_slots, dim3(nblk(nq + KT)), dim3(256), 0, ctx->stream, ctx->d_q[A], ctx->d_q[B], ctx->d_q[C], ctx->d_q[B], nq,
			   ctx->d_p[A], ctx->d_p[B], ctx->d_p[C], ctx->d_p[B], KT, scheme == 4, ctx->d_scalars + 24, stop);
	if ((rc = project_slot(ctx, B, stop))) return rc;
	if (!ctx->admixture) {
		if ((rc = run_mixture(ctx, B, B, 0, 1, stop, 2))) return rc;
	} else {
		if (use_dual) {
			prof_mark(ctx, MCHIP_KERN_DUAL, true);
			ctx->kt->accum_q_dual(dual, ctx->stream);
			prof_mark(ctx, MCHIP_KERN_DUAL, false);
		} else {
			mchip_pass_args a = pass_args(ctx, B);
			a.stop = stop;
			prof_mark(ctx, MCHIP_KERN_ACCUM_Q, true);
			ctx->kt->accum_q(a, ctx->stream);
			prof_mark(ctx, MCHIP_KERN_ACCUM_Q, false);
		}
	}
	if (ctx->admixture)
		hipLaunchKernelGGL(k_reduce_accept, dim3(1), dim3(MCHIP_BLOCK), 0, ctx->stream, use_dual ? ctx->d_llpart2 : (const double *)nullptr, ctx->d_llpart,
				   ctx->kt->ind_ll_parts(dual), ctx->d_scalars, cyc, stop);
	else
		hipLaunchKernelGGL(k_accept, dim3(1), dim3(64), 0, ctx->stream, ctx->d_scalars, cyc, stop);
	hipLaunchKernelGGL(k_select_copy, dim3(nblk(nq + KT)), dim3(256), 0, ctx->stream, ctx->d_q[A], ctx->d_q[B], ctx->d_q[C], nq,
			   ctx->d_p[A], ctx->d_p[B], ctx->d_p[C], KT, cyc, stop);
	HIPCHK(hipGetLastError());
	return MCHIP_OK;
}

int mchip_accel_run(mchip_context *ctx, int slot, int scheme, int n_cycles, mchip_run_state *state)
{
	MCHIP_ENTRY();
	int rc = check_slot(ctx, slot);
	if (rc) return rc;
	if (!state || n_cycles < 1 || scheme < 1 || scheme > 4) return fail(ctx, MCHIP_ERR_INVALID, "accel_run: bad arguments%s", nullptr);
	if ((ctx->admixture && !ctx->sparse) || ctx->nsec < 1)
		return fail(ctx, MCHIP_ERR_UNSUPPORTED, "accel_run: needs a secant pair; loci with more than 32 alleles run cycle by cycle%s", nullptr);
	if (ctx->qstride) ctx->empty_rows_nan[0] = ctx->empty_rows_nan[1] = ctx->empty_rows_nan[2] = 1;
	HIPCHK(hipSetDevice(ctx->device));
	HIPCHK(hipMemcpyAsync(ctx->d_run, state, sizeof *state, hipMemcpyHostToDevice, ctx->stream));
	const int cyc0[4] = { 0, (ctx->admixture && ctx->s_cache_slot == slot) ? 1 : 0, 0, 0 };
	HIPCHK(hipMemcpyAsync(ctx->d_cyc, cyc0, sizeof cyc0, hipMemcpyHostToDevice, ctx->stream));
	HIPCHK(hipStreamSynchronize(ctx->stream));
	ctx->s_cache_slot = -1;
	bool use_graph = !ctx->profiling && !ctx->knob.no_graph;
	hipGraphExec_t &exec = ctx->cycle_graph[slot][scheme];
	if (use_graph && !exec) {
		hipGraph_t graph = nullptr;
		if (MCHIP_WAIT(hipStreamBeginCapture(ctx->stream, hipStreamCaptureModeThreadLocal)) == hipSuccess) {
			rc = accel_cycle_enqueue(ctx, slot, scheme);
			const hipError_t e = MCHIP_WAIT(hipStreamEndCapture(ctx->stream, &graph));
			if (rc || e != hipSuccess || !graph || MCHIP_WAIT(hipGraphInstantiate(&exec, graph, nullptr, nullptr, 0)) != hipSuccess) exec = nullptr;
			if (graph) (void)MCHIP_WAIT(hipGraphDestroy(graph));
			(void)hipGetLastError();
		}
		if (!exec) use_graph = false;
	}
	for (int c = 0; c < n_cycles; c++) {
		if (use_graph) HIPCHK(hipGraphLaunch(exec, ctx->stream));
		else if ((rc = accel_cycle_enqueue(ctx, slot, scheme))) return rc;
	}
	int cyc_out[4] = { 0, 0, 0, 0 };
	HIPCHK(hipMemcpyAsync(state, ctx->d_run, sizeof *state, hipMemcpyDeviceToHost, ctx->stream));
	HIPCHK(hipMemcpyAsync(cyc_out, ctx->d_cyc, sizeof cyc_out, hipMemcpyDeviceToHost, ctx->stream));
	HIPCHK(hipStreamSynchronize(ctx->stream));
	ctx->s_cache_slot = (ctx->admixture && !state->stopped && cyc_out[1]) ? slot : -1;
	ctx->have_ll = 1;
	return MCHIP_OK;
}

int mchip_multisecant_update(mchip_context *ctx, int to, int base, int u_index, int n_terms,
			     const int *v_index, const double *coef_a, const double *coef_b)
{
	MCHIP_ENTRY();
	int rc = check_secant(ctx, u_index);
	if (rc) return rc;
	ctx->s_cache_slot = -1;
	if ((rc = check_slot(ctx, to)) || (rc = check_slot(ctx, base))) return rc;
	if (n_terms < 0 || (n_terms && (!v_index || !coef_a || !coef_b))) return MCHIP_ERR_INVALID;
	for (int t = 0; t < n_terms; t++) if ((rc = check_secant(ctx, v_index[t]))) return rc;
	HIPCHK(hipSetDevice(ctx->device));
	const size_t KT = (size_t)ctx->K * ctx->T;
	hipLaunchKernelGGL(k_add, dim3(nblk(KT)), dim3(256), 0, ctx->stream, ctx->d_p[base], ctx->d_up[u_index], ctx->d_p[to], KT);
	hipLaunchKernelGGL(k_add, dim3(nblk(ctx->nq)), dim3(256), 0, ctx->stream, ctx->d_q[base], ctx->d_uq[u_index], ctx->d_q[to], (size_t)ctx->nq);
	for (int t = 0; t < n_terms; t++) {
		hipLaunchKernelGGL(k_axpy2, dim3(nblk(KT)), dim3(256), 0, ctx->stream, ctx->d_vp[v_index[t]], ctx->d_p[to], KT, coef_a[t], coef_b[t]);
		hipLaunchKernelGGL(k_axpy2, dim3(nblk(ctx->nq)), dim3(256), 0, ctx->stream, ctx->d_vq[v_index[t]], ctx->d_q[to], (size_t)ctx->nq, coef_a[t], coef_b[t]);
	}
	HIPCHK(hipGetLastError());
	ctx->empty_rows_nan[to] = ctx->empty_rows_nan[base];
	return project_slot(ctx, to);
}

int mchip_profile_begin(mchip_context *ctx)
{
	MCHIP_ENTRY();
	if (!ctx) return MCHIP_ERR_INVALID;
	HIPCHK(hipSetDevice(ctx->device));
	ctx->profiling = 1;
	ctx->ev_used = 0;
	ctx->ev_kind.clear();
	ctx->pair_used = 0;
	HIPCHK(hipEventRecord(ctx->ev_begin, ctx->stream));
	return MCHIP_OK;
}

int mchip_profile_end(mchip_context *ctx, double *total_ms, double *kernel_ms, int *launches)
{
	MCHIP_ENTRY();
	if (!ctx) return MCHIP_ERR_INVALID;
	if (!ctx->profiling) return fail(ctx, MCHIP_ERR_STATE, "profile_end without profile_begin%s", nullptr);
	HIPCHK(hipSetDevice(ctx->device));
	HIPCHK(hipEventRecord(ctx->ev_end, ctx->stream));
	HIPCHK(hipEventSynchronize(ctx->ev_end));
	ctx->profiling = 0;
	float ms = 0;
	HIPCHK(hipEventElapsedTime(&ms, ctx->ev_begin, ctx->ev_end));
	if (total_ms) *total_ms = ms;
	double km[MCHIP_KERN_COUNT] = {0}, longest[MCHIP_KERN_COUNT] = {0};
	int kl[MCHIP_KERN_COUNT] = {0};
	std::vector<float> each(ctx->ev_kind.size(), 0.0f);
	std::vector<int> kind_of(ctx->ev_kind);
	for (size_t p = 0; 2 * p + 1 < ctx->ev_used && p < ctx->ev_kind.size(); p++)
		HIPCHK(hipEventElapsedTime(&each[p], ctx->ev_pool[2 * p], ctx->ev_pool[2 * p + 1]));
	if (ctx->pair_used) {
		int khz = 0;
		if (MCHIP_WAIT(hipDeviceGetAttribute(&khz, hipDeviceAttributeWallClockRate, ctx->device)) != hipSuccess || khz <= 0) khz = 100000;
		std::vector<mchip_pair_span> spans(ctx->pair_used);
		for (size_t p = 0; p < ctx->pair_used; p += PAIR_SPAN_CHUNK) {
			const size_t n = ctx->pair_used - p < PAIR_SPAN_CHUNK ? ctx->pair_used - p : PAIR_SPAN_CHUNK;
			HIPCHK(hipMemcpy(&spans[p], ctx->pair_spans[p / PAIR_SPAN_CHUNK], n * sizeof(mchip_pair_span), hipMemcpyDeviceToHost));
		}
		for (const mchip_pair_span &sp : spans)
			for (int x = 0; x < 2; x++) {
				each.push_back(sp.end[x] > sp.start[x] ? (float)((double)(sp.end[x] - sp.start[x]) / khz) : 0.0f);
				kind_of.push_back(x ? MCHIP_KERN_ACCUM_Q : MCHIP_KERN_ACCUM_P);
			}
		ctx->pair_used = 0;
	}
	for (size_t p = 0; p < each.size(); p++)
		if (each[p] > longest[kind_of[p]]) longest[kind_of[p]] = each[p];
	for (size_t p = 0; p < each.size(); p++) {
		const int kind = kind_of[p];
		if (each[p] <= 0.0f || each[p] < 0.05 * longest[kind]) continue;
		km[kind] += each[p];
		kl[kind]++;
	}
	for (int x = 0; x < MCHIP_KERN_COUNT; x++) {
		if (kernel_ms) kernel_ms[x] = km[x];
		if (launches) launches[x] = kl[x];
	}
	return MCHIP_OK;
}

int mchip_progress_note(const char *what)
{
	mchip_progress_slot *s = mchip_progress_my_slot();
	s->note.store(what, std::memory_order_relaxed);
	s->since_ns.store(mchip_progress_now(), std::memory_order_relaxed);
	mchip_progress_events.fetch_add(1, std::memory_order_relaxed);
	return MCHIP_OK;
}

int mchip_progress_report(char *buf, int buf_len, unsigned long long *events)
{
	if (events) *events = mchip_progress_events.load(std::memory_order_relaxed);
	if (!buf || buf_len <= 0) return MCHIP_OK;
	int n = progress_next_slot.load(std::memory_order_relaxed), used = 0;
	if (n > MCHIP_PROGRESS_SLOTS) n = MCHIP_PROGRESS_SLOTS;
	const long long now = mchip_progress_now();
	buf[0] = 0;
	for (int x = 0; x < n && used < buf_len - 1; x++) {
		const mchip_progress_slot &s = mchip_progress_slots[x];
		const char *entry = s.entry.load(std::memory_order_relaxed), *wait = s.wait.load(std::memory_order_relaxed);
		const char *note = s.note.load(std::memory_order_relaxed);
		const int w = snprintf(buf + used, (size_t)(buf_len - used), "thread %ld: %s%s%s%s%s%s, %.1f s since its last event\n",
				       s.tid.load(std::memory_order_relaxed), entry ? "in " : "outside the library", entry ? entry : "",
				       wait ? ", waiting in " : "", wait ? wait : "", note ? "; last phase: " : "", note ? note : "",
				       1e-9 * (double)(now - s.since_ns.load(std::memory_order_relaxed)));
		if (w < 0) break;
		used += w < buf_len - used ? w : buf_len - used - 1;
	}
	return MCHIP_OK;
}

}
```

multiclust_amd/csrc/mchip_context.h:

```cpp
#ifndef MCHIP_CONTEXT_H
#define MCHIP_CONTEXT_H

#include "mchip_internal.h"
#include "mchip_progress.h"

#include <functional>
#include <type_traits>
#include <stdio.h>
#include <string.h>

constexpr int RNG_LAG = 31;
constexpr int RNG_CHUNK = 4 * RNG_LAG * 32;

struct saved_set {
	uint8_t *d_raw = nullptr;
	int L = 0;
	std::vector<int32_t> ua;
	std::vector<int> empty;
};

struct mchip_context {
	int device;
	hipStream_t stream;
	char err[512];
	int n_cu;
	int I, L, ploidy, T, max_M, min_M;
	std::vector<int32_t> h_ua;
	int parked_K;
	int sig_admixture, sig_constrained, sig_projection, sig_nsec;
	double sig_eta_lb, sig_p_lb;
	int init_geno_set;
	int32_t *d_ua, *d_toff, *d_col_locus;
	uint8_t *d_col_allele;
	uint8_t *d_gtA, *d_gtS, *d_gtC;
	int count_bits, has_missing;
	int first_empty;
	std::vector<int> empty_rows;
	int empty_rows_nan[3];
	unsigned long long nnz_cells, n_copies;
	int counts_valid;
	size_t geno_bytes_A, geno_bytes_S;
	uint8_t *d_asA, *d_asS;
	uint8_t *d_initA, *d_initS;
	uint8_t *d_draw;
	uint8_t *d_cv_fold;
	int cv_n_folds;
	saved_set cv_full;
	int cv_fold;
	double *d_cv_part;
	size_t cv_part_cap;
	unsigned long long *d_cv_out;
	saved_set rs_base;
	uint8_t *d_cand_span, *d_cand_centers;
	unsigned long long *d_cand_off;
	size_t cand_span_bytes, cand_loci, cand_center_bytes;
	uint32_t *d_jump_hi, *d_jump_lo;
	size_t n_jump_hi;
	struct lattice { uint32_t *d_i, *d_r; uint64_t A, B; unsigned nA, nB; } lat[2];
	uint32_t *d_part_slabs;
	size_t part_slab_bytes;
	uint8_t *d_sim_cluster;
	uint32_t *d_cen_part, *d_cen_work;
	size_t cen_part_bytes, cen_work_bytes;
	int K, admixture, constrained, do_projection, nsec, nq, qstride;
	double eta_lb, p_lb;
	const mchip_ktable *kt;
	double *d_p[3], *d_q[3];
	double *d_up[MCHIP_MAX_SECANTS], *d_vp[MCHIP_MAX_SECANTS], *d_uq[MCHIP_MAX_SECANTS], *d_vq[MCHIP_MAX_SECANTS];
	double *d_sik;
	double *d_stage;
	double *d_logp;
	int ichunk, n_ichunks, lchunk, n_lchunks, n_llpart, flush_blocks, safe_rcp, sparse;
	int ind_waves;
	int xcd_rows;
	struct {
		int no_bial, no_counts, force_dense, force_safe, no_graph, no_dual, no_slab_sum, no_col_split, part_no_tile, sim_no_tile;
		int no_fused_finalize, no_pair;
		int per_cu_col, per_cu_ind, geometry_given, no_roundup;
		double slab_frac;
	} knob;
	double *d_Apart, *d_Spart, *d_llpart, *d_scalars;
	double *d_llpart2;
	double *d_redpart;
	uint8_t *d_flags;
	double *h_pinned;
	mchip_run_state *d_run;
	hipGraphExec_t step_graph[3];
	hipGraphExec_t cycle_graph[3][5];
	int *d_cyc;
	int have_ll;
	int ll_parts;
	int s_cache_slot;
	int profiling;
	hipEvent_t ev_begin, ev_end;
	std::vector<hipEvent_t> ev_pool;
	std::vector<int> ev_kind;
	size_t ev_used;
	unsigned long long *d_pair_marks;
	size_t pair_marks_cap;
	std::vector<mchip_pair_span *> pair_spans;
	size_t pair_used;
};

static int fail(mchip_context *ctx, int code, const char *fmt, const char *detail)
{
	if (ctx) snprintf(ctx->err, sizeof ctx->err, fmt, detail ? detail : "");
	return code;
}

#define HIPCHK(call)                                                                                  \
	do {                                                                                          \
		hipError_t e_ = MCHIP_WAIT(call);                                                     \
		if (e_ != hipSuccess) {                                                               \
			snprintf(ctx->err, sizeof ctx->err, "%s failed: %s (%s:%d)", #call,           \
				 hipGetErrorString(e_), __FILE__, __LINE__);                          \
			return MCHIP_ERR_HIP;                                                         \
		}                                                                                     \
	} while (0)

template <typename Tp> static void dfree(Tp *&p)
{
	if (p) (void)MCHIP_WAIT(hipFree(p));
	p = nullptr;
}

template <typename Tp> struct scoped_dev {
	Tp *p = nullptr;
	scoped_dev() = default;
	scoped_dev(const scoped_dev &) = delete;
	scoped_dev &operator=(const scoped_dev &) = delete;
	~scoped_dev() { if (p) (void)MCHIP_WAIT(hipFree(p)); }
	hipError_t alloc(size_t count) { return hipMalloc((void **)&p, count * sizeof(Tp)); }
	operator Tp *() const { return p; }
};

template <typename Tp> static hipError_t grow_dev(mchip_context *ctx, Tp **p, size_t *have_bytes, size_t want_bytes)
{
	if (*have_bytes >= want_bytes) return hipSuccess;
	if (*p) { (void)MCHIP_WAIT(hipStreamSynchronize(ctx->stream)); (void)MCHIP_WAIT(hipFree(*p)); *p = nullptr; *have_bytes = 0; }
	const hipError_t e = hipMalloc((void **)p, want_bytes);
	if (e == hipSuccess) *have_bytes = want_bytes;
	return e;
}

template <typename F> static void with_ploidy(int pl, F &&f)
{
	switch (pl) {
	case 1: f(std::integral_constant<int, 1>()); break;
	case 2: f(std::integral_constant<int, 2>()); break;
	case 3: f(std::integral_constant<int, 3>()); break;
	case 4: f(std::integral_constant<int, 4>()); break;
	case 5: f(std::integral_constant<int, 5>()); break;
	case 6: f(std::integral_constant<int, 6>()); break;
	case 7: f(std::integral_constant<int, 7>()); break;
	default: f(std::integral_constant<int, 8>()); break;
	}
}

static inline unsigned nblk(size_t n, unsigned b = 256) { return (unsigned)((n + b - 1) / b); }
static inline unsigned nblk_capped(size_t n, unsigned b = 256)
{
	const size_t blocks = (n + b - 1) / b, cap = ((size_t)1 << 30) / b;
	return (unsigned)(blocks < cap ? blocks : cap);
}

static int *bad_flag(mchip_context *ctx) { return reinterpret_cast<int *>(ctx->d_scalars + 63); }

#pragma GCC visibility push(hidden)

int check_slot(mchip_context *ctx, int slot);
void free_model(mchip_context *ctx);
enum { KEEP_INIT = 1, KEEP_RS_BASE = 2 };
void free_data(mchip_context *ctx, int keep = 0);
int set_shape(mchip_context *ctx, int I, int L, int ploidy, const int32_t *ua, int keep = 0);
int install_layouts(mchip_context *ctx, int has_missing);

void set_empty_rows(mchip_context *ctx, std::vector<int> rows);
void set_empty_rows_unseen(mchip_context *ctx, const std::vector<uint8_t> &seen);
int save_installed(mchip_context *ctx, saved_set &set);
void drop_saved(saved_set &set);
int install_saved(mchip_context *ctx, const saved_set &set);
int install_derived(mchip_context *ctx, const std::function<void(uint8_t *d_out, uint8_t *d_seen)> &fill);
int stream_buffer(mchip_context *ctx);
int install_raw(mchip_context *ctx, const uint8_t *d_raw);
int check_partition_call(mchip_context *ctx, const void *arg, int to);
int partition_mstep(mchip_context *ctx, const uint8_t *d_raw, int to, int counts = 0);
int partition_finalize(mchip_context *ctx, int to, int counts, int n_aslabs);
void launch_reduce_sum(mchip_context *ctx, const double *in, int n, double *out);

int draw_mod_stream(mchip_context *ctx, const uint32_t *window, size_t n_draws, int m, uint8_t *d_out);
void drop_generators(mchip_context *ctx);

void drop_cv(mchip_context *ctx);

#pragma GCC visibility pop

#endif
```

multiclust_amd/csrc/mchip_finalize.h:

```cpp
#ifndef MCHIP_FINALIZE_H
#define MCHIP_FINALIZE_H

#include <hip/hip_runtime.h>
#include <stdint.h>

#include "mchip_internal.h"

static __device__ void michelot_strided(double *x, int stride, int len, double mn, uint8_t *flags)
{
	unsigned long long fixed = 0ull;
	int n = len;
	if (len > 64) for (int j = 0; j < len; j++) flags[(size_t)j * stride] = 0;
	while (n) {
		double csum = 0.0;
		for (int j = 0; j < len; j++) csum += x[(size_t)j * stride];
		const double shift = (csum - 1.0) / (double)n;
		bool can_terminate = true;
		for (int j = 0; j < len; j++) {
			const bool is_fixed = (len > 64) ? (flags[(size_t)j * stride] != 0) : (((fixed >> j) & 1ull) != 0);
			if (is_fixed) continue;
			double v = x[(size_t)j * stride] - shift;
			if (v < mn) {
				v = mn;
				if (len > 64) flags[(size_t)j * stride] = 1; else fixed |= 1ull << j;
				n--;
				can_terminate = false;
			}
			x[(size_t)j * stride] = v;
		}
		if (can_terminate) break;
	}
}

__device__ __forceinline__ void michelot_small(double (&x)[8], int len, double mn)
{
	unsigned fixed = 0u;
	int n = len;
	while (n) {
		double csum = 0.0;
#pragma unroll
		for (int j = 0; j < 8; j++)
			if (j < len) csum += x[j];
		const double shift = (csum - 1.0) / (double)n;
		bool can_terminate = true;
#pragma unroll
		for (int j = 0; j < 8; j++) {
			if (j >= len || ((fixed >> j) & 1u)) continue;
			double v = x[j] - shift;
			if (v < mn) {
				v = mn;
				fixed |= 1u << j;
				n--;
				can_terminate = false;
			}
			x[j] = v;
		}
		if (can_terminate) break;
	}
}

constexpr int FP_TILE = 1024;
__device__ __forceinline__ void finalize_p_tile_body(int block, double *tile, int L, int K, int T, const int32_t *__restrict__ toff, int loci_per_block,
		int n_slabs, const double *__restrict__ Apart, const double *Pfrom, double *Pto,
		int weighted, double add_lb, int do_projection, double lb)
{
	const int l0 = block * loci_per_block, l1 = min(L, l0 + loci_per_block);
	const int c0 = toff[l0], c1 = toff[l1];
	const int nel = (c1 - c0) * K;
	const size_t e0 = (size_t)c0 * K, slab = (size_t)T * K;
	if (nel > 0) {
		double v[FP_TILE / MCHIP_BLOCK];
#pragma unroll
		for (int y = 0; y < FP_TILE / MCHIP_BLOCK; y++) v[y] = 0.0;
		for (int sl = 0; sl < n_slabs; sl++) {
			double w[FP_TILE / MCHIP_BLOCK];
#pragma unroll
			for (int y = 0; y < FP_TILE / MCHIP_BLOCK; y++) {
				const int x = min((int)threadIdx.x + y * MCHIP_BLOCK, nel - 1);
				w[y] = Apart[(size_t)sl * slab + e0 + x];
			}
#pragma unroll
			for (int y = 0; y < FP_TILE / MCHIP_BLOCK; y++) v[y] += w[y];
		}
#pragma unroll
		for (int y = 0; y < FP_TILE / MCHIP_BLOCK; y++) {
			const int x = threadIdx.x + y * MCHIP_BLOCK;
			if (x < nel) {
				double t = v[y];
				if (weighted) t *= Pfrom[e0 + x];
				tile[x] = t + add_lb;
			}
		}
	}
	__syncthreads();
	for (int y = threadIdx.x; y < (l1 - l0) * K; y += MCHIP_BLOCK) {
		const int k = y % K, l = l0 + y / K;
		const int m0 = toff[l] - c0, M = toff[l + 1] - toff[l];
		double *col = tile + (size_t)m0 * K + k;
		double temp = 0.0;
		if (M <= 8) {
			double v[8];
#pragma unroll
			for (int m = 0; m < 8; m++) {
				v[m] = 0.0;
				if (m < M) {
					v[m] = col[(size_t)m * K];
					temp += v[m];
				}
			}
#pragma unroll
			for (int m = 0; m < 8; m++)
				if (m < M) v[m] /= temp;
			if (do_projection) michelot_small(v, M, lb);
#pragma unroll
			for (int m = 0; m < 8; m++)
				if (m < M) col[(size_t)m * K] = v[m];
		} else {
			for (int m = 0; m < M; m++) temp += col[(size_t)m * K];
			for (int m = 0; m < M; m++) col[(size_t)m * K] /= temp;
			if (do_projection) michelot_strided(col, K, M, lb, nullptr);
		}
	}
	__syncthreads();
	for (int x = threadIdx.x; x < nel; x += MCHIP_BLOCK) Pto[e0 + x] = tile[x];
}


#endif
```

multiclust_amd/csrc/mchip_internal.h:

```cpp
#ifndef MCHIP_INTERNAL_H
#define MCHIP_INTERNAL_H

#include <hip/hip_runtime.h>
#include <stdint.h>
#include <vector>
#include "multiclust_hip.h"

#define MCHIP_BLOCK 256
#define MCHIP_SPARSE_MAX_M 32
#ifndef MCHIP_QBLOCK
#define MCHIP_QBLOCK 128
#endif

#ifdef MCHIP_FORCE_SPLIT1
constexpr int mchip_ind_split(int) { return 1; }
#else
constexpr int mchip_ind_split(int K) { return K <= 27 ? 1 : (K <= 48 ? 2 : 4); }
#endif
#ifdef MCHIP_FORCE_SPLIT1
constexpr int mchip_qblock(int) { return MCHIP_QBLOCK; }
#else
constexpr int mchip_qblock(int K) { return K > 48 ? 2 * MCHIP_QBLOCK : MCHIP_QBLOCK; }
#endif
#ifndef MCHIP_COL_SPLIT2_ABOVE
#define MCHIP_COL_SPLIT2_ABOVE 36
#endif
#ifndef MCHIP_COL_SPLIT4_ABOVE
#define MCHIP_COL_SPLIT4_ABOVE 9999
#endif
constexpr int mchip_col_split(int K) { return K > MCHIP_COL_SPLIT4_ABOVE ? 4 : (K > MCHIP_COL_SPLIT2_ABOVE ? 2 : 1); }
constexpr bool mchip_parts_conflict(int split, int stride)
{
	for (int a = 0; a < split; a++)
		for (int b = a + 1; b < split; b++) {
			const int d = (2 * stride * (b - a)) % 64;
			if (d < 4 || d > 60) return true;
		}
	return false;
}
constexpr int mchip_ind_pstride(int K)
{
	const int split = mchip_ind_split(K);
	int stride = ((((K + split - 1) / split) + 1) & ~1);
	while (split > 1 && mchip_parts_conflict(split, stride)) stride += 2;
	return stride;
}
constexpr int mchip_kp(int K)
{
	const int split = mchip_ind_split(K);
	const int per_lane = mchip_ind_pstride(K) * split;
	const int base = per_lane > ((K + 1) & ~1) ? per_lane : ((K + 1) & ~1);
	return base + ((base % 16 == 0) ? 2 : 0);
}

constexpr int MCHIP_COL_WAVES = MCHIP_BLOCK / 64;
#ifndef MCHIP_IND_WAVES_MAX
#define MCHIP_IND_WAVES_MAX 4
#endif
inline int mchip_ind_waves(int K, int tile_cols);

enum { MCHIP_KERN_ACCUM_P = 0, MCHIP_KERN_ACCUM_Q = 1, MCHIP_KERN_LOGLIK = 2, MCHIP_KERN_DUAL = 3, MCHIP_KERN_COUNT = 4 };

struct mchip_pass_args {
	int I, L, T, ploidy, K;
	const uint8_t *gtA, *gtS;
	const uint8_t *gtC;
	int count_bits;
	int has_missing;
	const int32_t *ua, *toff, *col_locus;
	const uint8_t *col_allele;
	const double *P;
	const double *Q;
	int qstride;
	int ichunk, n_ichunks;
	double *Apart;
	double *llpart;
	int flush_blocks;
	int safe_rcp;
	int lchunk, n_lchunks;
	double *Spart;
	int xcd_rows;
	int no_col_split;
	int ind_waves;
	int sparse;
	int tile_cols;
	int biallelic;
	const int *stop;
	const int *skip_ind;
	const double *P2, *Q2;
	double *llpart2;
	const uint8_t *asA, *asS;
	int part_counts;
};

#define MCHIP_PAIR_RUN 8
struct mchip_pair_runs { unsigned col_runs, ind_runs; };
__host__ __device__ inline bool mchip_pair_is_ind(unsigned block, mchip_pair_runs r, unsigned *logical)
{
	const unsigned run = block / MCHIP_PAIR_RUN, total = r.col_runs + r.ind_runs;
	const unsigned before = run * r.ind_runs / total, upto = (run + 1) * r.ind_runs / total;
	const bool ind = upto > before;
	*logical = (ind ? before : run - before) * MCHIP_PAIR_RUN + block % MCHIP_PAIR_RUN;
	return ind;
}
struct mchip_pair_span { unsigned long long start[2], end[2]; };

struct mchip_finalize_p_args {
	int L, K, T, loci_per_block, n_slabs, weighted, do_projection;
	const int32_t *toff;
	const double *Apart, *Pfrom;
	double *Pto;
	double add_lb, lb;
};

struct mchip_ktable {
	void (*accum_p)(const mchip_pass_args &a, hipStream_t s);
	void (*loglik)(const mchip_pass_args &a, hipStream_t s);
	void (*accum_q)(const mchip_pass_args &a, hipStream_t s);
	void (*part_p)(const mchip_pass_args &a, hipStream_t s);
	void (*part_q)(const mchip_pass_args &a, hipStream_t s);
	void (*finalize_q)(int I, int K, int n_lchunks, const double *Spart, const double *Qfrom, int qstride_from,
			   double *Qto, double *sik, int do_mstep, int weighted, int do_projection, double lb, const int *stop, hipStream_t s,
			   double add);
	void (*project_q)(int nrows, int K, double *Q, double lb, const int *stop, hipStream_t s);
	void (*mix_gather)(const mchip_pass_args &a, hipStream_t s);
	void (*mix_finalize)(int I, int n_lchunks, const double *Vpart, const double *eta, double *vik, double *llpart, int mode,
			     const int *stop, hipStream_t s);
	void (*mix_column)(const mchip_pass_args &a, hipStream_t s);
	int (*dual_available)(const mchip_pass_args &a);
	void (*accum_q_dual)(const mchip_pass_args &a, hipStream_t s);
	int (*col_slabs)(const mchip_pass_args &a, int mix);
	int (*ind_slabs)(const mchip_pass_args &a);
	int (*ind_ll_parts)(const mchip_pass_args &a);
	void (*finalize_qp)(int I, int n_slabs_q, const double *Spart, const double *Qfrom, int qstride_from, double *Qto, double *sik,
			    int do_projection_q, double lb_q, const mchip_finalize_p_args &p, const int *stop, hipStream_t s);
	int (*pair_available)(const mchip_pass_args &a);
	unsigned (*pair_blocks)(const mchip_pass_args &a, mchip_pair_runs *runs);
	void (*estep_pair)(const mchip_pass_args &a, unsigned long long *marks, hipStream_t s);
};

const mchip_ktable *mchip_get_ktable(int K);

inline int mchip_ind_waves(int K, int tile_cols)
{
	const size_t per_wave = (size_t)(K <= 12 ? 4 : 2) * ((((size_t)tile_cols * (size_t)mchip_kp(K) + 127) / 128) * 128) * sizeof(double);
	for (int w = MCHIP_IND_WAVES_MAX; w > 1; w >>= 1)
		if ((size_t)w * per_wave <= 48 * 1024) return w;
	return 1;
}
__host__ __device__ inline int mchip_ind_slabs(const mchip_pass_args &a) { return (a.n_lchunks + a.ind_waves - 1) / a.ind_waves; }
__host__ __device__ inline int mchip_col_slabs(const mchip_pass_args &a) { return (a.n_ichunks + MCHIP_COL_WAVES - 1) / MCHIP_COL_WAVES; }

#endif
```

multiclust_amd/csrc/mchip_kernels_k.hip:

```cpp
#include "mchip_internal.h"
#include "mchip_finalize.h"

#ifndef MCHIP_K
#error "compile with -DMCHIP_K=<K>"
#endif

namespace {

constexpr int K = MCHIP_K;

__device__ __forceinline__ double rcp_full(double t)
{
	const double r = __builtin_amdgcn_rcp(t);
	const double e = __builtin_fma(-t, r, 1.0);
	const double p = __builtin_fma(e, e, e);
	return __builtin_fma(r, p, r);
}

__device__ __forceinline__ void rcp4(const double (&t)[4], double (&rc)[4])
{
	const double p01 = t[0] * t[1], p23 = t[2] * t[3];
	const double rp = rcp_full(p01 * p23);
	const double r01 = rp * p23, r23 = rp * p01;
	rc[0] = r01 * t[1];
// ... 900 lines not shown
						for (int b = 0; b < 4; b++)
#pragma unroll
							for (int k = 0; k < K; k++) acc[k] = __builtin_fma(pc[b][k], r[b], acc[k]);
						prod *= p01;
						prod *= p23;
					} else
#pragma unroll
					for (int b = 0; b < PL; b += 2) {
						const double pp = t[b] * t[b + 1];
						if (ACCUM) {
							double r0, r1;
							if (SAFE) {
								r0 = miss[b] ? 0.0 : rcp_full(t[b]);
								r1 = miss[b + 1] ? 0.0 : rcp_full(t[b + 1]);
							} else {
								const double rp = rcp_full(pp);
								r0 = miss[b] ? 0.0 : rp * t[b + 1];
								r1 = miss[b + 1] ? 0.0 : rp * t[b];
							}
#pragma unroll
							for (int k = 0; k < K; k++) acc[k] = __builtin_fma(pc[b][k], r0, acc[k]);
#pragma unroll
							for (int k = 0; k < K; k++) acc[k] = __builtin_fma(pc[b + 1][k], r1, acc[k]);
						}
						if (SAFE) {
							prod *= t[b] < 0.0 ? __builtin_nan("") : t[b];
							rescale(prod, ex);
							prod *= t[b + 1] < 0.0 ? __builtin_nan("") : t[b + 1];
							rescale(prod, ex);
						} else {
							prod *= pp;
						}
						if constexpr (DUAL) {
							double t2[2];
#pragma unroll
							for (int bb = 0; bb < 2; bb++) {
								const double2 *pr = reinterpret_cast<const double2 *>(tile2 + (size_t)row[b + bb] * KP);
								double pc2[KP];
#pragma unroll
								for (int k = 0; k < KP / 2; k++) {
									const double2 v = pr[k];
									pc2[2 * k] = v.x;
									pc2[2 * k + 1] = v.y;
								}
								t2[bb] = q2[0] * pc2[0];
#pragma unroll
								for (int k = 1; k < K; k++) t2[bb] = __builtin_fma(q2[k], pc2[k], t2[bb]);
								if (!NOMISS) t2[bb] = miss[b + bb] ? 1.0 : t2[bb];
							}
							prod2 *= t2[0] * t2[1];
						}
					}
				} else {
					for (int bb = 0; bb < pl; bb++) {
						const unsigned mraw = g.copy(j, bb, pl);
						const bool miss = (mraw == MCHIP_MISSING) || !active;
						const unsigned mm = miss ? 0u : mraw;
						const double *pr = tile + (size_t)(base + (int)mm) * KP;
						double pc[K];
#pragma unroll
						for (int k = 0; k < K; k++) pc[k] = pr[k];
						double t = q[0] * pc[0];
#pragma unroll
						for (int k = 1; k < K; k++) t = __builtin_fma(q[k], pc[k], t);
						if (ACCUM) {
							const double r = miss ? 0.0 : rcp_full(t);
#pragma unroll
							for (int k = 0; k < K; k++) acc[k] = __builtin_fma(pc[k], r, acc[k]);
						}
						prod *= miss ? 1.0 : (t < 0.0 ? __builtin_nan("") : t);
						rescale(prod, ex);
					}
				}
			};
			auto tick = [&]() __attribute__((always_inline)) {
				if (!SAFE) {
					if (++blk >= a.flush_blocks) {
						blk = 0;
						rescale(prod, ex);
						if (DUAL) rescale(prod2, ex2);
					}
				}
			};
			const int nloc = l1 - lb * 8;
#pragma unroll
			for (int j = 0; j < 8; j++) {
				if (j < nloc) one_locus(j);
				if (PL == 4 && j == 3) tick();
			}
			tick();
			if constexpr (GLDS) {
				glds_wait();
			} else if (staged) {
#pragma unroll
				for (int s2 = 0; s2 < WSTAGE; s2++) {
					const int x = lane + s2 * 64;
					if (x < nel_next) dst[(x / K) * KP + (x % K)] = stage[s2];
					if constexpr (DUAL) { if (x < nel_next) dst2[(x / K) * KP + (x % K)] = stage2[s2]; }
				}
			}
			g = gn;
#pragma unroll
			for (int x = 0; x <= 8; x++) E[x] = E[x + 8];
#pragma unroll
			for (int x = 0; x < 8; x++) E[9 + x] = En[x];
		}
	}
	double ll = (double)ex * 0.693147180559945309417 + log(prod);
	double ll2 = DUAL ? (double)ex2 * 0.693147180559945309417 + log(prod2) : 0.0;
	if (W > 1) {
		__syncthreads();
		for (int x = 1; x < W; x++) {
			if (wv == x) {
#pragma unroll
				for (int k = 0; k < K; k++) lds[k * 64 + lane] = acc[k];
				lds[K * 64 + lane] = ll;
				if (DUAL) lds[(K + 1) * 64 + lane] = ll2;
			}
			__syncthreads();
			if (wv == 0) {
#pragma unroll
				for (int k = 0; k < K; k++) acc[k] += lds[k * 64 + lane];
				ll += lds[K * 64 + lane];
				if (DUAL) ll2 += lds[(K + 1) * 64 + lane];
			}
			__syncthreads();
		}
	}
	if (wv == 0) {
		if (ACCUM && active) {
			double *out = a.Spart + ((size_t)by * a.I + i) * K;
#pragma unroll
			for (int k = 0; k < K; k++) out[k] = acc[k];
		}
		const double tot = wave_total(active ? ll : 0.0);
		if (lane == 0) a.llpart[(size_t)by * n_tiles + bx] = tot;
		if (DUAL) {
			const double tot2 = wave_total(active ? ll2 : 0.0);
			if (lane == 0) a.llpart2[(size_t)by * n_tiles + bx] = tot2;
		}
	}
}

template <int PL, bool ACCUM, bool SAFE, bool NOMISS, bool DUAL = false>
__global__ __launch_bounds__(64 * MCHIP_IND_WAVES_MAX) void k_individual_sparse_w(mchip_pass_args a)
{
	if (a.stop && *a.stop) return;
	if (ACCUM && !DUAL && a.skip_ind && *a.skip_ind) return;
	extern __shared__ __attribute__((aligned(16))) double lds[];
	individual_sparse_w_body<PL, ACCUM, SAFE, NOMISS, DUAL>(a, blockIdx.x, lds);
}

template <int BITS, int PL, bool SAFE, bool NOMISS>
__global__ __launch_bounds__(MCHIP_BLOCK) void k_estep_pair(mchip_pass_args a, mchip_pair_runs runs, unsigned long long *marks)
{
	static_assert(64 * MCHIP_IND_WAVES_MAX == MCHIP_BLOCK, "both bodies at 256 threads");
	extern __shared__ __attribute__((aligned(16))) double lds[];
	unsigned logical;
	const bool ind = mchip_pair_is_ind(blockIdx.x, runs, &logical);
	const unsigned n_col = (unsigned)((a.T + 63) / 64), n_mine = ind ? (unsigned)(((a.I + 63) / 64) * mchip_ind_slabs(a)) : n_col * (unsigned)mchip_col_slabs(a);
	const bool idle = logical >= n_mine || (a.stop && *a.stop) || (ind && a.skip_ind && *a.skip_ind);
	if (idle) {
		if (marks && threadIdx.x == 0) {
			marks[2 * (size_t)blockIdx.x] = ~0ull;
			marks[2 * (size_t)blockIdx.x + 1] = 0ull;
		}
		return;
	}
	const unsigned long long t_start = marks ? __builtin_amdgcn_s_memrealtime() : 0ull;
	if (ind) individual_sparse_w_body<PL, true, SAFE, NOMISS, false>(a, logical, lds);
	else column_counts_body<BITS, false, SAFE>(a, (int)(logical % n_col), (int)(logical / n_col), reinterpret_cast<double (*)[64]>(lds));
	if (marks) {
		unsigned long long (*wave_mark)[MCHIP_COL_WAVES] = reinterpret_cast<unsigned long long (*)[MCHIP_COL_WAVES]>(lds);
		if ((threadIdx.x & 63) == 0) {
			wave_mark[0][threadIdx.x >> 6] = t_start;
			wave_mark[1][threadIdx.x >> 6] = __builtin_amdgcn_s_memrealtime();
		}
		__syncthreads();
		if (threadIdx.x == 0) {
			unsigned long long t0 = wave_mark[0][0], t1 = wave_mark[1][0];
			for (int w = 1; w < MCHIP_COL_WAVES; w++) {
				t0 = wave_mark[0][w] < t0 ? wave_mark[0][w] : t0;
				t1 = wave_mark[1][w] > t1 ? wave_mark[1][w] : t1;
			}
			marks[2 * (size_t)blockIdx.x] = t0;
			marks[2 * (size_t)blockIdx.x + 1] = t1;
		}
	}
}

template <bool ACCUM, bool NOMISS>
__global__ __launch_bounds__(64 * MCHIP_IND_WAVES_MAX) void k_individual_bial(mchip_pass_args a)
{
	if (a.stop && *a.stop) return;
	if (ACCUM && a.skip_ind && *a.skip_ind) return;
	__shared__ double xch[K + 1][64];
	const int lane = threadIdx.x & 63;
	const int wv = __builtin_amdgcn_readfirstlane((int)(threadIdx.x >> 6));
	const int W = a.ind_waves;
	const int i_raw = blockIdx.x * 64 + lane;
	const bool active = i_raw < a.I;
	const int i = active ? i_raw : a.I - 1;
	double q[K], acc[K];
#pragma unroll
	for (int k = 0; k < K; k++) {
		q[k] = a.Q[(size_t)i * a.qstride + k];
		acc[k] = 0.0;
	}
	const int l0raw = (int)(blockIdx.y * W + wv) * a.lchunk;
	const bool any = l0raw < a.L;
	const int l0 = any ? l0raw : 0;
	const int l1 = any ? min(a.L, l0 + a.lchunk) : 0;
	const int lb0 = l0 >> 3, lb_end = any ? (l1 + 7) >> 3 : lb0;
	double prod = 1.0;
	int blk = 0, ex = 0;
	geno_group<2> g, gn;
	g.load(a.gtS, (size_t)lb0 * a.I + i, 2);
	for (int lb = lb0; lb < lb_end; lb++) {
		gn.load(a.gtS, (size_t)min(lb + 1, lb_end - 1) * a.I + i, 2);
		const int nloc = l1 - lb * 8;
#pragma unroll
		for (int j = 0; j < 8; j++) {
			if (j < nloc) {
				const double *__restrict__ r0 = a.P + (size_t)(lb * 8 + j) * 2 * K;
				double t0 = q[0] * r0[0], t1 = q[0] * r0[K];
#pragma unroll
				for (int k = 1; k < K; k++) {
					t0 = __builtin_fma(q[k], r0[k], t0);
					t1 = __builtin_fma(q[k], r0[K + k], t1);
				}
				const unsigned ma = g.copy(j, 0, 2), mb = g.copy(j, 1, 2);
				double ta, tb;
				if (NOMISS) {
					ta = ma ? t1 : t0;
					tb = mb ? t1 : t0;
				} else {
					ta = !active ? 1.0 : (ma == 0u ? t0 : (ma == 1u ? t1 : 1.0));
					tb = !active ? 1.0 : (mb == 0u ? t0 : (mb == 1u ? t1 : 1.0));
				}
				if (ACCUM) {
					const double rp = rcp_full(t0 * t1);
					const double n0 = (double)((int)(ma == 0u) + (int)(mb == 0u)), n1 = (double)((int)(ma == 1u) + (int)(mb == 1u));
					const double R0 = n0 * (rp * t1), R1 = n1 * (rp * t0);
#pragma unroll
					for (int k = 0; k < K; k++) {
						acc[k] = __builtin_fma(r0[k], R0, acc[k]);
						acc[k] = __builtin_fma(r0[K + k], R1, acc[k]);
					}
				}
				prod *= ta * tb;
			}
		}
		if (++blk >= a.flush_blocks) {
			blk = 0;
			rescale(prod, ex);
		}
		g = gn;
	}
	double ll = (double)ex * 0.693147180559945309417 + log(prod);
	for (int x = 1; x < W; x++) {
		if (wv == x) {
#pragma unroll
			for (int k = 0; k < K; k++) xch[k][lane] = acc[k];
			xch[K][lane] = ll;
		}
		__syncthreads();
		if (wv == 0) {
#pragma unroll
			for (int k = 0; k < K; k++) acc[k] += xch[k][lane];
			ll += xch[K][lane];
		}
		__syncthreads();
	}
	if (wv == 0) {
		if (ACCUM && active) {
			double *out = a.Spart + ((size_t)blockIdx.y * a.I + i) * K;
#pragma unroll
			for (int k = 0; k < K; k++) out[k] = acc[k];
		}
		const double tot = wave_total(active ? ll : 0.0);
		if (lane == 0) a.llpart[(size_t)blockIdx.y * gridDim.x + blockIdx.x] = tot;
	}
}

template <int PL, bool STAGED>
__global__ __launch_bounds__(QBLOCK) void k_mix_gather(mchip_pass_args a)
{
	if (a.stop && *a.stop) return;
	extern __shared__ __attribute__((aligned(16))) double lds[];
	const int i_raw = blockIdx.x * QBLOCK + threadIdx.x;
	const bool active = i_raw < a.I;
	const int i = active ? i_raw : a.I - 1;
	const int pl = PL ? PL : a.ploidy;
	double acc[K];
#pragma unroll
	for (int k = 0; k < K; k++) acc[k] = 0.0;
	const int l0 = blockIdx.y * a.lchunk;
	const int l1 = min(a.L, l0 + a.lchunk);
	const int lb0 = l0 >> 3, lb_end = (l1 + 7) >> 3;
	if (STAGED) {
		const int c_lo = a.toff[lb0 * 8], c_hi = a.toff[min(lb0 * 8 + 8, a.L)];
		const int nel = (c_hi - c_lo) * K;
		for (int x = threadIdx.x; x < nel; x += QBLOCK)
			lds[(x / K) * KP + (x % K)] = a.P[(size_t)c_lo * K + x];
		__syncthreads();
	}
	for (int lb = lb0; lb < lb_end; lb++) {
		const int buf = (lb - lb0) & 1;
		const int c_lo = a.toff[lb * 8];
		const double *tile = STAGED ? lds + (size_t)buf * a.tile_cols * KP : a.P + (size_t)c_lo * K;
		if (STAGED && lb + 1 < lb_end) {
			const int n_lo = a.toff[(lb + 1) * 8], n_hi = a.toff[min((lb + 1) * 8 + 8, a.L)];
			const int nel = (n_hi - n_lo) * K;
			double *dst = lds + (size_t)(buf ^ 1) * a.tile_cols * KP;
			for (int x = threadIdx.x; x < nel; x += QBLOCK)
				dst[(x / K) * KP + (x % K)] = a.P[(size_t)n_lo * K + x];
		}
		geno_group<PL> g;
		g.load(a.gtS, (size_t)lb * a.I + i, pl);
		for (int j = 0; j < 8; j++) {
			const int l = lb * 8 + j;
			if (l >= l1) break;
			const int base = a.toff[l] - c_lo;
			for (int b = 0; b < pl; b++) {
				const unsigned mraw = g.copy(j, b, pl);
				if (mraw == MCHIP_MISSING || !active) continue;
				const double *pr = tile + (size_t)(base + (int)mraw) * (STAGED ? KP : K);
#pragma unroll
				for (int k = 0; k < K; k++) acc[k] += pr[k];
			}
		}
		if (STAGED) __syncthreads();
	}
	if (active) {
		double *out = a.Spart + ((size_t)blockIdx.y * a.I + i) * K;
#pragma unroll
		for (int k = 0; k < K; k++) out[k] = acc[k];
	}
}
// ... 154 lines not shown
	const int i = blockIdx.x * QBLOCK + threadIdx.x;
	if (i >= a.I) return;
	const int pl = PL ? PL : a.ploidy;
	double acc[K];
#pragma unroll
	for (int k = 0; k < K; k++) acc[k] = 0.0;
	const int l0 = blockIdx.y * a.lchunk;
	const int l1 = min(a.L, l0 + a.lchunk);
	for (int lb = l0 >> 3; lb < ((l1 + 7) >> 3); lb++) {
		geno_group<PL> g, s;
		g.load(a.gtS, (size_t)lb * a.I + i, pl);
		s.load(a.asS, (size_t)lb * a.I + i, pl);
		for (int j = 0; j < 8; j++) {
			if (lb * 8 + j >= l1) break;
			for (int b = 0; b < pl; b++) {
				const unsigned mb = g.copy(j, b, pl), kb = s.copy(j, b, pl);
				if (!a.part_counts) {
					if (mb == MCHIP_MISSING) continue;
					bool dup = false;
					for (int b2 = 0; b2 < b; b2++)
						dup |= (g.copy(j, b2, pl) == mb) && (s.copy(j, b2, pl) == kb);
					if (dup) continue;
				}
#pragma unroll
				for (int k = 0; k < K; k++) acc[k] += (kb == (unsigned)k) ? 1.0 : 0.0;
			}
		}
	}
	double *out = a.Spart + ((size_t)blockIdx.y * a.I + i) * K;
#pragma unroll
	for (int k = 0; k < K; k++) out[k] = acc[k];
}

__device__ __forceinline__ void michelot_k(double (&x)[K], double mn)
{
	unsigned long long fixed = 0;
	int n = K;
	while (n) {
		double csum = 0.0;
#pragma unroll
		for (int j = 0; j < K; j++) csum += x[j];
		const double shift = (csum - 1.0) / (double)n;
		bool can_terminate = true;
#pragma unroll
		for (int j = 0; j < K; j++)
			if (!((fixed >> j) & 1ull)) {
				x[j] -= shift;
				if (x[j] < mn) {
					x[j] = mn;
					fixed |= 1ull << j;
					n--;
					can_terminate = false;
				}
			}
		if (can_terminate) break;
	}
}

constexpr int FQ_LANES = 8, FQ_IND = MCHIP_BLOCK / FQ_LANES;
constexpr int FQ_XCH = (K <= 16 ? FQ_LANES - 1 : 1) * K * FQ_IND;
__device__ __forceinline__ void finalize_q_body(int block, double *xch_raw, int I, int n_lchunks, const double *__restrict__ Spart,
		const double *__restrict__ Qfrom, int qstride_from, double *Qto, double *sik,
		int do_mstep, int weighted, int do_projection, double lb, double add)
{
	constexpr int TURNS = K <= 16 ? 1 : FQ_LANES - 1;
	double (*xch)[K][FQ_IND] = reinterpret_cast<double (*)[K][FQ_IND]>(xch_raw);
	const int il = threadIdx.x % FQ_IND, g = threadIdx.x / FQ_IND;
	const int i = block * FQ_IND + il;
	const bool active = i < I;
	double s[K];
#pragma unroll
	for (int k = 0; k < K; k++) s[k] = 0.0;
	if (active) {
		const size_t row = (size_t)I * K;
		const double *src = Spart + (size_t)g * row + (size_t)i * K;
		int ch = g;
		for (; ch + 3 * FQ_LANES < n_lchunks; ch += 4 * FQ_LANES, src += 4 * FQ_LANES * row) {
			double v[4][K];
#pragma unroll
			for (int y = 0; y < 4; y++)
#pragma unroll
				for (int k = 0; k < K; k++) v[y][k] = src[(size_t)y * FQ_LANES * row + k];
#pragma unroll
			for (int y = 0; y < 4; y++)
#pragma unroll
				for (int k = 0; k < K; k++) s[k] += v[y][k];
		}
		for (; ch < n_lchunks; ch += FQ_LANES, src += FQ_LANES * row) {
#pragma unroll
			for (int k = 0; k < K; k++) s[k] += src[k];
		}
	}
	if constexpr (TURNS == 1) {
		if (g) {
#pragma unroll
			for (int k = 0; k < K; k++) xch[g - 1][k][il] = s[k];
		}
		__syncthreads();
		if (g == 0) {
#pragma unroll
			for (int x = 0; x < FQ_LANES - 1; x++)
#pragma unroll
				for (int k = 0; k < K; k++) s[k] += xch[x][k][il];
		}
	} else {
		for (int x = 1; x < FQ_LANES; x++) {
			if (g == x) {
#pragma unroll
				for (int k = 0; k < K; k++) xch[0][k][il] = s[k];
			}
			__syncthreads();
			if (g == 0) {
#pragma unroll
				for (int k = 0; k < K; k++) s[k] += xch[0][k][il];
			}
			__syncthreads();
		}
	}
	if (g || !active) return;
	if (weighted) {
#pragma unroll
		for (int k = 0; k < K; k++) s[k] *= Qfrom[(size_t)i * qstride_from + k];
	}
#pragma unroll
	for (int k = 0; k < K; k++) sik[(size_t)i * K + k] = s[k];
	if (!do_mstep) return;
	double temp = 0.0;
#pragma unroll
	for (int k = 0; k < K; k++) {
		s[k] += add;
		temp += s[k];
	}
	if (temp == 0.0) {
#pragma unroll
		for (int k = 0; k < K; k++) Qto[(size_t)i * K + k] = 1.0 / K;
		return;
	}
#pragma unroll
	for (int k = 0; k < K; k++) s[k] /= temp;
	if (do_projection) michelot_k(s, lb);
#pragma unroll
	for (int k = 0; k < K; k++) Qto[(size_t)i * K + k] = s[k];
}
__global__ __launch_bounds__(MCHIP_BLOCK) void k_finalize_q(int I, int n_lchunks, const double *__restrict__ Spart,
		const double *__restrict__ Qfrom, int qstride_from, double *Qto, double *sik,
		int do_mstep, int weighted, int do_projection, double lb, const int *stop, double add)
{
	__shared__ double xch[FQ_XCH];
	if (stop && *stop) return;
	finalize_q_body(blockIdx.x, xch, I, n_lchunks, Spart, Qfrom, qstride_from, Qto, sik, do_mstep, weighted, do_projection, lb, add);
}
__global__ __launch_bounds__(MCHIP_BLOCK) void k_finalize_qp(int q_blocks, int I, int n_lchunks, const double *__restrict__ Spart,
		const double *__restrict__ Qfrom, int qstride_from, double *Qto, double *sik,
		int do_projection_q, double lb_q, mchip_finalize_p_args p, const int *stop)
{
	__shared__ double lds[FQ_XCH > FP_TILE ? FQ_XCH : FP_TILE];
	if (stop && *stop) return;
	if ((int)blockIdx.x < q_blocks)
		finalize_q_body(blockIdx.x, lds, I, n_lchunks, Spart, Qfrom, qstride_from, Qto, sik, 1, 1, do_projection_q, lb_q, 0.0);
	else
		finalize_p_tile_body((int)blockIdx.x - q_blocks, lds, p.L, p.K, p.T, p.toff, p.loci_per_block, p.n_slabs, p.Apart, p.Pfrom, p.Pto,
				     p.weighted, p.add_lb, p.do_projection, p.lb);
}

__global__ __launch_bounds__(MCHIP_BLOCK) void k_project_q(int nrows, double *Q, double lb, const int *stop)
{
	const int i = blockIdx.x * MCHIP_BLOCK + threadIdx.x;
	if (i >= nrows || (stop && *stop)) return;
	double s[K];
#pragma unroll
	for (int k = 0; k < K; k++) s[k] = Q[(size_t)i * K + k];
	michelot_k(s, lb);
#pragma unroll
	for (int k = 0; k < K; k++) Q[(size_t)i * K + k] = s[k];
}

inline dim3 column_grid(const mchip_pass_args &a) { return dim3((a.T + MCHIP_BLOCK - 1) / MCHIP_BLOCK, a.n_ichunks); }
inline dim3 counts_grid(const mchip_pass_args &a) { return dim3((a.T + 63) / 64, mchip_col_slabs(a)); }
inline dim3 indiv_grid(const mchip_pass_args &a) { return dim3((a.I + QBLOCK - 1) / QBLOCK, a.n_lchunks); }
inline dim3 sparse_grid(const mchip_pass_args &a) { return dim3((a.I + QBLOCK / SPLIT - 1) / (QBLOCK / SPLIT), a.n_lchunks); }
inline dim3 coop_grid(const mchip_pass_args &a) { return dim3((a.I + 63) / 64, mchip_ind_slabs(a)); }
inline dim3 coop_rows(const mchip_pass_args &a) { return dim3((unsigned)(((a.I + 63) / 64) * mchip_ind_slabs(a))); }
inline size_t coop_lds_bytes(const mchip_pass_args &a, int sets)
{
	const size_t tiles = (size_t)a.ind_waves * 2 * sets * tile_stride(a.tile_cols), hand_over = (size_t)(K + 2) * 64;
	return (tiles > hand_over ? tiles : hand_over) * sizeof(double);
}

void launch_accum_p(const mchip_pass_args &a, hipStream_t s)
{
	if constexpr (CSPLIT > 1) {
		if (a.sparse && a.count_bits && !a.no_col_split) {
			const dim3 grid((a.T + MCHIP_BLOCK / CSPLIT - 1) / (MCHIP_BLOCK / CSPLIT), a.n_ichunks);
			if (a.count_bits == 2 && a.safe_rcp) hipLaunchKernelGGL((k_column_counts_split<2, true>), grid, dim3(MCHIP_BLOCK), 0, s, a);
			else if (a.count_bits == 2) hipLaunchKernelGGL((k_column_counts_split<2, false>), grid, dim3(MCHIP_BLOCK), 0, s, a);
			else if (a.safe_rcp) hipLaunchKernelGGL((k_column_counts_split<4, true>), grid, dim3(MCHIP_BLOCK), 0, s, a);
			else hipLaunchKernelGGL((k_column_counts_split<4, false>), grid, dim3(MCHIP_BLOCK), 0, s, a);
			return;
		}
	}
	if (a.sparse && a.count_bits == 2 && a.safe_rcp) { hipLaunchKernelGGL((k_column_counts<2, false, true>), counts_grid(a), dim3(MCHIP_BLOCK), 0, s, a); return; }
	if (a.sparse && a.count_bits == 4 && a.safe_rcp) { hipLaunchKernelGGL((k_column_counts<4, false, true>), counts_grid(a), dim3(MCHIP_BLOCK), 0, s, a); return; }
	if (a.sparse && a.count_bits == 2) { hipLaunchKernelGGL((k_column_counts<2, false>), counts_grid(a), dim3(MCHIP_BLOCK), 0, s, a); return; }
	if (a.sparse && a.count_bits == 4) { hipLaunchKernelGGL((k_column_counts<4, false>), counts_grid(a), dim3(MCHIP_BLOCK), 0, s, a); return; }
	if (a.sparse) {
		if (a.ploidy == 2) hipLaunchKernelGGL((k_column_pass<2, true, false, false>), column_grid(a), dim3(MCHIP_BLOCK), 0, s, a);
		else hipLaunchKernelGGL((k_column_pass<0, true, false, false>), column_grid(a), dim3(MCHIP_BLOCK), 0, s, a);
		return;
	}
	if (a.ploidy == 2 && a.flush_blocks >= 1) hipLaunchKernelGGL((k_column_pass<2, true, false, true>), column_grid(a), dim3(MCHIP_BLOCK), 0, s, a);
	else if (a.ploidy == 2) hipLaunchKernelGGL((k_column_pass<2, true, true, true>), column_grid(a), dim3(MCHIP_BLOCK), 0, s, a);
	else hipLaunchKernelGGL((k_column_pass<0, true, true, true>), column_grid(a), dim3(MCHIP_BLOCK), 0, s, a);
}
#ifdef MCHIP_EXP_SCATTER
inline size_t sparse_lds_bytes(const mchip_pass_args &a) { return (3 * (size_t)a.tile_cols * KP + QBLOCK) * sizeof(double); }
#else
inline size_t sparse_lds_bytes(const mchip_pass_args &a) { return (2 * (size_t)a.tile_cols * KP + QBLOCK) * sizeof(double); }
#endif
template <bool ACCUM> void launch_sparse(const mchip_pass_args &a, hipStream_t s)
{
	const size_t lds = sparse_lds_bytes(a);
	const bool nomiss = !a.has_missing;
	const bool safe = a.flush_blocks < 1;
	constexpr bool bial_pays = SPLIT == 1 && (ACCUM ? (K >= 10) : (K >= 6));
	if constexpr (SPLIT == 1) {
		const dim3 grid = coop_grid(a), rows = coop_rows(a), block(64 * a.ind_waves);
		const size_t cl = coop_lds_bytes(a, 1);
		if (bial_pays && a.biallelic && a.ploidy == 2 && !safe) {
			if (nomiss) hipLaunchKernelGGL((k_individual_bial<ACCUM, true>), grid, block, 0, s, a);
			else hipLaunchKernelGGL((k_individual_bial<ACCUM, false>), grid, block, 0, s, a);
			return;
		}
#define MCHIP_SPARSE_W(PLV) \
		do { \
			if (nomiss && !safe) hipLaunchKernelGGL((k_individual_sparse_w<PLV, ACCUM, false, true>), rows, block, cl, s, a); \
			else if (!safe) hipLaunchKernelGGL((k_individual_sparse_w<PLV, ACCUM, false, false>), rows, block, cl, s, a); \
			else hipLaunchKernelGGL((k_individual_sparse_w<PLV, ACCUM, true, false>), rows, block, cl, s, a); \
		} while (0)
		if (a.ploidy == 2) MCHIP_SPARSE_W(2);
		else if (a.ploidy == 4) MCHIP_SPARSE_W(4);
		else hipLaunchKernelGGL((k_individual_sparse_w<0, ACCUM, true, false>), rows, block, cl, s, a);
#undef MCHIP_SPARSE_W
	} else {
#define MCHIP_SPARSE(PLV) \
		do { \
			if (nomiss && !safe) hipLaunchKernelGGL((k_individual_sparse<PLV, ACCUM, false, true>), sparse_grid(a), dim3(QBLOCK), lds, s, a); \
			else if (!safe) hipLaunchKernelGGL((k_individual_sparse<PLV, ACCUM, false, false>), sparse_grid(a), dim3(QBLOCK), lds, s, a); \
			else hipLaunchKernelGGL((k_individual_sparse<PLV, ACCUM, true, false>), sparse_grid(a), dim3(QBLOCK), lds, s, a); \
		} while (0)
		if (a.ploidy == 2) MCHIP_SPARSE(2);
		else if (a.ploidy == 4) MCHIP_SPARSE(4);
		else hipLaunchKernelGGL((k_individual_sparse<0, ACCUM, true, false>), sparse_grid(a), dim3(QBLOCK), lds, s, a);
#undef MCHIP_SPARSE
	}
}
int dual_available(const mchip_pass_args &a)
{
	if (K > 12 || !a.sparse || a.flush_blocks < 1 || a.ploidy != 2) return 0;
	if (a.biallelic && K >= 6) return 0;
	return coop_lds_bytes(a, 2) <= 64 * 1024;
}
void launch_accum_q_dual(const mchip_pass_args &a, hipStream_t s)
{
	if constexpr (K <= 12) {
		const size_t lds = coop_lds_bytes(a, 2);
		if (!a.has_missing) hipLaunchKernelGGL((k_individual_sparse_w<2, true, false, true, true>), coop_rows(a), dim3(64 * a.ind_waves), lds, s, a);
		else hipLaunchKernelGGL((k_individual_sparse_w<2, true, false, false, true>), coop_rows(a), dim3(64 * a.ind_waves), lds, s, a);
	}
}
unsigned pair_blocks(const mchip_pass_args &a, mchip_pair_runs *runs)
{
	const dim3 cg = counts_grid(a);
	const unsigned n_col = cg.x * cg.y, n_ind = coop_rows(a).x;
	runs->col_runs = (n_col + MCHIP_PAIR_RUN - 1) / MCHIP_PAIR_RUN;
	runs->ind_runs = (n_ind + MCHIP_PAIR_RUN - 1) / MCHIP_PAIR_RUN;
	return (runs->col_runs + runs->ind_runs) * MCHIP_PAIR_RUN;
}
int pair_available(const mchip_pass_args &a)
{
	if (K > 12 || SPLIT != 1 || CSPLIT != 1) return 0;
	if (!a.sparse || a.count_bits != 2 || a.ploidy != 2 || a.ind_waves * 64 != MCHIP_BLOCK) return 0;
	if ((a.safe_rcp != 0) != (a.flush_blocks < 1)) return 0;
	if (a.biallelic && K >= 10 && a.flush_blocks >= 1) return 0;
	mchip_pair_runs r;
	pair_blocks(a, &r);
	if (r.col_runs == 0 || r.ind_runs == 0) return 0;
	return (unsigned long long)(r.col_runs + r.ind_runs) * r.ind_runs < (1ull << 32);
}
void launch_estep_pair(const mchip_pass_args &a, unsigned long long *marks, hipStream_t s)
{
	if constexpr (K <= 12 && SPLIT == 1 && CSPLIT == 1) {
		mchip_pair_runs r;
		const dim3 grid(pair_blocks(a, &r)), block(MCHIP_BLOCK);
		const size_t ind_lds = coop_lds_bytes(a, 1), col_lds = (size_t)K * 64 * sizeof(double);
		const size_t lds = ind_lds > col_lds ? ind_lds : col_lds;
		if (a.flush_blocks < 1) hipLaunchKernelGGL((k_estep_pair<2, 2, true, false>), grid, block, lds, s, a, r, marks);
		else if (!a.has_missing) hipLaunchKernelGGL((k_estep_pair<2, 2, false, true>), grid, block, lds, s, a, r, marks);
		else hipLaunchKernelGGL((k_estep_pair<2, 2, false, false>), grid, block, lds, s, a, r, marks);
	}
}
int col_slabs(const mchip_pass_args &a, int mix)
{
	if (mix) return a.count_bits ? mchip_col_slabs(a) : a.n_ichunks;
	return (a.sparse && a.count_bits && (CSPLIT == 1 || a.no_col_split)) ? mchip_col_slabs(a) : a.n_ichunks;
}
int ind_slabs(const mchip_pass_args &a) { return (a.sparse && SPLIT == 1) ? mchip_ind_slabs(a) : a.n_lchunks; }
int ind_ll_parts(const mchip_pass_args &a)
{
	if (a.sparse && SPLIT == 1) return ((a.I + 63) / 64) * mchip_ind_slabs(a);
	if (a.sparse) return ((a.I + QBLOCK / SPLIT - 1) / (QBLOCK / SPLIT)) * a.n_lchunks;
	return ((a.T + MCHIP_BLOCK - 1) / MCHIP_BLOCK) * a.n_ichunks;
}
void launch_loglik(const mchip_pass_args &a, hipStream_t s)
{
	if (a.sparse) { launch_sparse<false>(a, s); return; }
	if (a.ploidy == 2 && a.flush_blocks >= 1) hipLaunchKernelGGL((k_column_pass<2, false, false, true>), column_grid(a), dim3(MCHIP_BLOCK), 0, s, a);
	else if (a.ploidy == 2) hipLaunchKernelGGL((k_column_pass<2, false, true, true>), column_grid(a), dim3(MCHIP_BLOCK), 0, s, a);
	else hipLaunchKernelGGL((k_column_pass<0, false, true, true>), column_grid(a), dim3(MCHIP_BLOCK), 0, s, a);
}
void launch_accum_q(const mchip_pass_args &a, hipStream_t s)
{
	if (a.sparse) { launch_sparse<true>(a, s); return; }
	if (a.ploidy == 2) hipLaunchKernelGGL((k_individual_pass<2>), indiv_grid(a), dim3(QBLOCK), 0, s, a);
	else hipLaunchKernelGGL((k_individual_pass<0>), indiv_grid(a), dim3(QBLOCK), 0, s, a);
}
void launch_mix_gather(const mchip_pass_args &a, hipStream_t s)
{
	const size_t lds = 2 * (size_t)a.tile_cols * KP * sizeof(double);
	if (a.sparse) {
		if (a.ploidy == 2) hipLaunchKernelGGL((k_mix_gather<2, true>), indiv_grid(a), dim3(QBLOCK), lds, s, a);
		else hipLaunchKernelGGL((k_mix_gather<0, true>), indiv_grid(a), dim3(QBLOCK), lds, s, a);
	} else {
		if (a.ploidy == 2) hipLaunchKernelGGL((k_mix_gather<2, false>), indiv_grid(a), dim3(QBLOCK), 0, s, a);
		else hipLaunchKernelGGL((k_mix_gather<0, false>), indiv_grid(a), dim3(QBLOCK), 0, s, a);
	}
}
void launch_mix_finalize(int I, int n_lchunks, const double *Vpart, const double *eta, double *vik, double *llpart, int mode, const int *stop, hipStream_t s)
{
	hipLaunchKernelGGL(k_mix_finalize, dim3((I + MCHIP_BLOCK - 1) / MCHIP_BLOCK), dim3(MCHIP_BLOCK), 0, s, I, n_lchunks, Vpart, eta, vik, llpart, mode, stop);
}
void launch_mix_column(const mchip_pass_args &a, hipStream_t s)
{
	if (a.count_bits == 2) { hipLaunchKernelGGL((k_column_counts<2, true>), counts_grid(a), dim3(MCHIP_BLOCK), 0, s, a); return; }
	if (a.count_bits == 4) { hipLaunchKernelGGL((k_column_counts<4, true>), counts_grid(a), dim3(MCHIP_BLOCK), 0, s, a); return; }
	if (a.ploidy == 2) hipLaunchKernelGGL((k_mix_column<2>), column_grid(a), dim3(MCHIP_BLOCK), 0, s, a);
	else hipLaunchKernelGGL((k_mix_column<0>), column_grid(a), dim3(MCHIP_BLOCK), 0, s, a);
}
void launch_part_p(const mchip_pass_args &a, hipStream_t s)
{
	if (a.ploidy == 2) hipLaunchKernelGGL((k_partition_columns<2>), column_grid(a), dim3(MCHIP_BLOCK), 0, s, a);
	else if (a.ploidy == 4) hipLaunchKernelGGL((k_partition_columns<4>), column_grid(a), dim3(MCHIP_BLOCK), 0, s, a);
	else hipLaunchKernelGGL((k_partition_columns<0>), column_grid(a), dim3(MCHIP_BLOCK), 0, s, a);
}
void launch_part_q(const mchip_pass_args &a, hipStream_t s)
{
	if (a.ploidy == 2) hipLaunchKernelGGL((k_partition_individuals<2>), indiv_grid(a), dim3(QBLOCK), 0, s, a);
	else if (a.ploidy == 4) hipLaunchKernelGGL((k_partition_individuals<4>), indiv_grid(a), dim3(QBLOCK), 0, s, a);
	else hipLaunchKernelGGL((k_partition_individuals<0>), indiv_grid(a), dim3(QBLOCK), 0, s, a);
}
void launch_finalize_q(int I, int, int n_lchunks, const double *Spart, const double *Qfrom, int qstride_from,
		       double *Qto, double *sik, int do_mstep, int weighted, int do_projection, double lb, const int *stop, hipStream_t s,
		       double add)
{
	hipLaunchKernelGGL(k_finalize_q, dim3((I + FQ_IND - 1) / FQ_IND), dim3(MCHIP_BLOCK), 0, s,
			   I, n_lchunks, Spart, Qfrom, qstride_from, Qto, sik, do_mstep, weighted, do_projection, lb, stop, add);
}
void launch_finalize_qp(int I, int n_lchunks, const double *Spart, const double *Qfrom, int qstride_from, double *Qto, double *sik,
			int do_projection_q, double lb_q, const mchip_finalize_p_args &p, const int *stop, hipStream_t s)
{
	const int q_blocks = (I + FQ_IND - 1) / FQ_IND, p_blocks = (p.L + p.loci_per_block - 1) / p.loci_per_block;
	hipLaunchKernelGGL(k_finalize_qp, dim3(q_blocks + p_blocks), dim3(MCHIP_BLOCK), 0, s,
			   q_blocks, I, n_lchunks, Spart, Qfrom, qstride_from, Qto, sik, do_projection_q, lb_q, p, stop);
}
void launch_project_q(int nrows, int, double *Q, double lb, const int *stop, hipStream_t s)
{
	hipLaunchKernelGGL(k_project_q, dim3((nrows + MCHIP_BLOCK - 1) / MCHIP_BLOCK), dim3(MCHIP_BLOCK), 0, s, nrows, Q, lb, stop);
}

}

#define MCHIP_CAT2(a, b) a##b
#define MCHIP_CAT(a, b) MCHIP_CAT2(a, b)
const mchip_ktable *MCHIP_CAT(mchip_ktable_get_, MCHIP_K)()
{
	static mchip_ktable t = {
		launch_accum_p, launch_loglik, launch_accum_q, launch_part_p, launch_part_q, launch_finalize_q, launch_project_q,
		launch_mix_gather, launch_mix_finalize, launch_mix_column, dual_available, launch_accum_q_dual,
		col_slabs, ind_slabs, ind_ll_parts, launch_finalize_qp, pair_available, pair_blocks, launch_estep_pair,
	};
	return &t;
}
```

Before: 220.2 EM iterations/s.

## Fold stop check and step-size reduction into preceding kernels via last-block tickets

Adds a last-block ticket scheme so that the convergence stop check runs inside the fused Q/P finalize kernel and the SQUAREM step-size reduction runs inside the dots kernel, removing separate small launches. It also adds a fused extrapolate-plus-project kernel for the accelerated update and an accept/select/copy kernel that merges the likelihood comparison with the buffer selection. Pair profiling now writes per-launch spans with atomics instead of per-block marks followed by a separate reduction kernel. The aim is fewer kernel launches and passes over memory per iteration, at the cost of global atomics and ticket counters that have to be reset correctly between launches.

Result: no change. 217.6 EM iterations/s (median of 2 runs) (-1.2%).

```diff
diff --git a/multiclust_amd/csrc/mchip.hip b/multiclust_amd/csrc/mchip.hip
--- a/multiclust_amd/csrc/mchip.hip
+++ b/multiclust_amd/csrc/mchip.hip
@@ -52,6 +52,7 @@
 	return (K >= 1 && K <= MCHIP_MAX_K) ? tabs[K]() : nullptr;
 }
 
+constexpr size_t TICKET_WORDS = (size_t)(1 + MCHIP_TICKET_GROUPS) * MCHIP_TICKET_STRIDE;
 static void read_knobs(mchip_context *ctx)
 {
 	auto on = [](const char *name) { return getenv(name) != nullptr ? 1 : 0; };
@@ -65,6 +66,9 @@
 	ctx->knob.no_slab_sum = on("MCHIP_NO_SLAB_SUM");
 	ctx->knob.no_fused_finalize = on("MCHIP_NO_FUSED_FINALIZE");
 	ctx->knob.no_pair = on("MCHIP_NO_PAIR");
+	ctx->knob.no_fold = on("MCHIP_NO_FOLD");
+	const char *pc = getenv("MCHIP_PAIR_CACHED");
+	ctx->knob.pair_cached = (pc && atoi(pc) == 0) ? 0 : 1;
 	ctx->knob.no_col_split = on("MCHIP_NO_COL_SPLIT");
 	ctx->knob.part_no_tile = on("MCHIP_PART_NO_TILE");
 	ctx->knob.sim_no_tile = on("MCHIP_SIM_NO_TILE");
@@ -444,20 +448,6 @@
 	dst[idx] = src[c * K + k];
 }
 
-__device__ __forceinline__ double ordered_sum(double acc, const double *__restrict__ in, size_t first, size_t stride, int count)
-{
-	int x = 0;
-	for (; x + 8 <= count; x += 8) {
-		double v[8];
-#pragma unroll
-		for (int y = 0; y < 8; y++) v[y] = in[first + (size_t)(x + y) * stride];
-#pragma unroll
-		for (int y = 0; y < 8; y++) acc += v[y];
-	}
-	for (; x < count; x++) acc += in[first + (size_t)x * stride];
-	return acc;
-}
-
 __device__ __forceinline__ double block_ordered_sum(const double *__restrict__ in, int n, double *red)
 {
 	const double s = (int)threadIdx.x < n ? ordered_sum(0.0, in, threadIdx.x, MCHIP_BLOCK, (n - (int)threadIdx.x + MCHIP_BLOCK - 1) / MCHIP_BLOCK) : 0.0;
@@ -644,46 +634,7 @@
 {
 	__shared__ double red[MCHIP_BLOCK];
 	if (s->stopped) return;
-	if (part) {
-		const double acc = (int)threadIdx.x < n ? ordered_sum(0.0, part, threadIdx.x, MCHIP_BLOCK, (n - (int)threadIdx.x + MCHIP_BLOCK - 1) / MCHIP_BLOCK) : 0.0;
-		red[threadIdx.x] = acc;
-		__syncthreads();
-		for (int w = MCHIP_BLOCK / 2; w > 0; w >>= 1) {
-			if ((int)threadIdx.x < w) red[threadIdx.x] += red[threadIdx.x + w];
-			__syncthreads();
-		}
-		if (threadIdx.x == 0) *ll = red[0];
-	}
-	if (threadIdx.x) return;
-	const double loglik = part ? red[0] : *ll;
-	s->n_iter++;
-	if (loglik != loglik) {
-		s->fatal = 1;
-		s->bad_loglik = loglik;
-		s->stopped = 1;
-		return;
-	}
-	int stop;
-	if (s->max_iter && s->n_iter > s->max_iter) {
-		s->iter_stop = 1;
-		stop = 1;
-	} else {
-		double abs_diff = 0, rel_diff = 0;
-		stop = 1;
-		if (s->abs_error != 0) abs_diff = fabs(loglik - s->logL);
-		if (s->rel_error != 0) rel_diff = abs_diff / fabs(s->logL);
-		if (s->abs_error != 0 && abs_diff > s->abs_error) stop = 0;
-		if (s->rel_error != 0 && rel_diff > s->rel_error) stop = 0;
-		if (stop) s->converged = 1;
-	}
-	s->stopped = stop;
-	if (loglik < s->logL && !stop) {
-		s->fatal = 2;
-		s->bad_loglik = loglik;
-		s->stopped = 1;
-		return;
-	}
-	s->logL = loglik;
+	stop_check_body(s, ll, part, n, red);
 }
 
 __global__ void k_diff(const double *__restrict__ a, const double *__restrict__ b, double *out, size_t n, const int *stop = nullptr)
@@ -725,78 +676,6 @@
 	}
 }
 
-__device__ __forceinline__ void dots_slots_body(const double *__restrict__ x0, const double *__restrict__ x1, const double *__restrict__ x2,
-		size_t n, double *part, unsigned bid, unsigned gdim, double (*red)[MCHIP_BLOCK])
-{
-	double s0 = 0, s1 = 0, s2 = 0;
-	for (size_t x = (size_t)bid * MCHIP_BLOCK + threadIdx.x; x < n; x += (size_t)gdim * MCHIP_BLOCK) {
-		const double uu = x1[x] - x0[x], vv = x2[x] - x1[x];
-		const double d = vv - uu;
-		s0 += uu * uu; s1 += uu * d; s2 += d * d;
-	}
-	red[0][threadIdx.x] = s0; red[1][threadIdx.x] = s1; red[2][threadIdx.x] = s2;
-	__syncthreads();
-	for (int w = MCHIP_BLOCK / 2; w > 0; w >>= 1) {
-		if ((int)threadIdx.x < w) {
-			red[0][threadIdx.x] += red[0][threadIdx.x + w];
-			red[1][threadIdx.x] += red[1][threadIdx.x + w];
-			red[2][threadIdx.x] += red[2][threadIdx.x + w];
-		}
-		__syncthreads();
-	}
-	if (threadIdx.x == 0) {
-		part[bid] = red[0][0];
-		part[gdim + bid] = red[1][0];
-		part[2 * gdim + bid] = red[2][0];
-	}
-}
-__global__ __launch_bounds__(MCHIP_BLOCK) void k_dots_slots(const double *__restrict__ q0, const double *__restrict__ q1,
-		const double *__restrict__ q2, size_t nq, double *part_q, unsigned gq, const double *__restrict__ p0,
-		const double *__restrict__ p1, const double *__restrict__ p2, size_t np, double *part_p, const int *stop)
-{
-	__shared__ double red[3][MCHIP_BLOCK];
-	if (stop && *stop) return;
-	if (blockIdx.x < gq) dots_slots_body(q0, q1, q2, nq, part_q, blockIdx.x, gq, red);
-	else dots_slots_body(p0, p1, p2, np, part_p, blockIdx.x - gq, gridDim.x - gq, red);
-}
-__global__ void k_accel_update_slots(const double *__restrict__ q0, const double *q1, const double *__restrict__ q2, double *qout, size_t nq,
-				     const double *__restrict__ p0, const double *p1, const double *__restrict__ p2, double *pout, size_t np,
-				     int qn_form, const double *s_dev, const int *stop)
-{
-#pragma clang fp contract(off)
-	size_t idx = (size_t)blockIdx.x * blockDim.x + threadIdx.x;
-	if (idx >= nq + np || (stop && *stop)) return;
-	const double *x0 = q0, *x1 = q1, *x2 = q2;
-	double *out = qout;
-	if (idx >= nq) { idx -= nq; x0 = p0; x1 = p1; x2 = p2; out = pout; }
-	const double s = *s_dev;
-	const double u = x1[idx] - x0[idx], v = x2[idx] - x1[idx];
-	if (qn_form) out[idx] = x0[idx] + u + s * v;
-	else out[idx] = x0[idx] - 2 * s * u + s * s * (v - u);
-}
-
-__global__ void k_accel_update(const double *__restrict__ base, const double *__restrict__ u, const double *__restrict__ v,
-			       double *out, size_t n, double s, int qn_form, const double *s_dev = nullptr, const int *stop = nullptr)
-{
-#pragma clang fp contract(off)
-	const size_t idx = (size_t)blockIdx.x * blockDim.x + threadIdx.x;
-	if (idx >= n || (stop && *stop)) return;
-	if (s_dev) s = *s_dev;
-	if (qn_form) out[idx] = base[idx] + u[idx] + s * v[idx];
-	else out[idx] = base[idx] - 2 * s * u[idx] + s * s * (v[idx] - u[idx]);
-}
-__global__ void k_axpy2(const double *__restrict__ v, double *out, size_t n, double ca, double cb)
-{
-#pragma clang fp contract(off)
-	const size_t idx = (size_t)blockIdx.x * blockDim.x + threadIdx.x;
-	if (idx < n) out[idx] += v[idx] * ca * cb;
-}
-__global__ void k_add(const double *__restrict__ a, const double *__restrict__ b, double *out, size_t n)
-{
-	const size_t idx = (size_t)blockIdx.x * blockDim.x + threadIdx.x;
-	if (idx < n) out[idx] = a[idx] + b[idx];
-}
-
 __device__ __forceinline__ void step_size_body(double *sc, int scheme, int *cyc)
 {
 	const double utu = sc[16] + sc[20], utvu = sc[17] + sc[21], vutvu = sc[18] + sc[22];
@@ -809,11 +688,9 @@
 	sc[24] = s;
 	cyc[0] = (s != s || s - s != 0.0) ? 1 : 0;
 }
-__global__ __launch_bounds__(MCHIP_BLOCK) void k_reduce_dots_step(const double *__restrict__ part_q, int gq, const double *__restrict__ part_p,
-		int gp, double *sc, int scheme, int *cyc, const int *stop)
-{
-	__shared__ double red[MCHIP_BLOCK];
-	if (stop && *stop) return;
+__device__ __forceinline__ void reduce_dots_step_body(const double *part_q, int gq, const double *part_p, int gp, double *sc, int scheme, int *cyc,
+		double *red)
+{
 	for (int x = 0; x < 6; x++) {
 		const double *in = x < 3 ? part_q + (size_t)x * gq : part_p + (size_t)(x - 3) * gp;
 		const int n = x < 3 ? gq : gp;
@@ -822,6 +699,86 @@
 	}
 	if (threadIdx.x == 0) step_size_body(sc, scheme, cyc);
 }
+__global__ __launch_bounds__(MCHIP_BLOCK) void k_reduce_dots_step(const double *__restrict__ part_q, int gq, const double *__restrict__ part_p,
+		int gp, double *sc, int scheme, int *cyc, const int *stop)
+{
+	__shared__ double red[MCHIP_BLOCK];
+	if (stop && *stop) return;
+	reduce_dots_step_body(part_q, gq, part_p, gp, sc, scheme, cyc, red);
+}
+__device__ __forceinline__ void dots_slots_body(const double *__restrict__ x0, const double *__restrict__ x1, const double *__restrict__ x2,
+		size_t n, double *part, unsigned bid, unsigned gdim, double (*red)[MCHIP_BLOCK])
+{
+	double s0 = 0, s1 = 0, s2 = 0;
+	for (size_t x = (size_t)bid * MCHIP_BLOCK + threadIdx.x; x < n; x += (size_t)gdim * MCHIP_BLOCK) {
+		const double uu = x1[x] - x0[x], vv = x2[x] - x1[x];
+		const double d = vv - uu;
+		s0 += uu * uu; s1 += uu * d; s2 += d * d;
+	}
+	red[0][threadIdx.x] = s0; red[1][threadIdx.x] = s1; red[2][threadIdx.x] = s2;
+	__syncthreads();
+	for (int w = MCHIP_BLOCK / 2; w > 0; w >>= 1) {
+		if ((int)threadIdx.x < w) {
+			red[0][threadIdx.x] += red[0][threadIdx.x + w];
+			red[1][threadIdx.x] += red[1][threadIdx.x + w];
+			red[2][threadIdx.x] += red[2][threadIdx.x + w];
+		}
+		__syncthreads();
+	}
+	if (threadIdx.x == 0) {
+		part[bid] = red[0][0];
+		part[gdim + bid] = red[1][0];
+		part[2 * gdim + bid] = red[2][0];
+	}
+}
+__global__ __launch_bounds__(MCHIP_BLOCK) void k_dots_slots(const double *__restrict__ q0, const double *__restrict__ q1,
+		const double *__restrict__ q2, size_t nq, double *part_q, unsigned gq, const double *__restrict__ p0,
+		const double *__restrict__ p1, const double *__restrict__ p2, size_t np, double *part_p, const int *stop,
+		unsigned *ticket = nullptr, unsigned group = 1, double *sc = nullptr, int scheme = 0, int *cyc = nullptr)
+{
+	__shared__ double red[3][MCHIP_BLOCK];
+	__shared__ int last;
+	if (stop && *stop) return;
+	if (blockIdx.x < gq) dots_slots_body(q0, q1, q2, nq, part_q, blockIdx.x, gq, red);
+	else dots_slots_body(p0, p1, p2, np, part_p, blockIdx.x - gq, gridDim.x - gq, red);
+	if (!ticket || !last_ticket(ticket, group, &last, true)) return;
+	reduce_dots_step_body(part_q, (int)gq, part_p, (int)(gridDim.x - gq), sc, scheme, cyc, red[0]);
+}
+__global__ void k_accel_update_slots(const double *__restrict__ q0, const double *q1, const double *__restrict__ q2, double *qout, size_t nq,
+				     const double *__restrict__ p0, const double *p1, const double *__restrict__ p2, double *pout, size_t np,
+				     int qn_form, const double *s_dev, const int *stop)
+{
+	size_t idx = (size_t)blockIdx.x * blockDim.x + threadIdx.x;
+	if (idx >= nq + np || (stop && *stop)) return;
+	const double *x0 = q0, *x1 = q1, *x2 = q2;
+	double *out = qout;
+	if (idx >= nq) { idx -= nq; x0 = p0; x1 = p1; x2 = p2; out = pout; }
+	const double s = *s_dev;
+	out[idx] = accel_extrapolate(x0[idx], x1[idx], x2[idx], s, qn_form);
+}
+
+__global__ void k_accel_update(const double *__restrict__ base, const double *__restrict__ u, const double *__restrict__ v,
+			       double *out, size_t n, double s, int qn_form, const double *s_dev = nullptr, const int *stop = nullptr)
+{
+#pragma clang fp contract(off)
+	const size_t idx = (size_t)blockIdx.x * blockDim.x + threadIdx.x;
+	if (idx >= n || (stop && *stop)) return;
+	if (s_dev) s = *s_dev;
+	if (qn_form) out[idx] = base[idx] + u[idx] + s * v[idx];
+	else out[idx] = base[idx] - 2 * s * u[idx] + s * s * (v[idx] - u[idx]);
+}
+__global__ void k_axpy2(const double *__restrict__ v, double *out, size_t n, double ca, double cb)
+{
+#pragma clang fp contract(off)
+	const size_t idx = (size_t)blockIdx.x * blockDim.x + threadIdx.x;
+	if (idx < n) out[idx] += v[idx] * ca * cb;
+}
+__global__ void k_add(const double *__restrict__ a, const double *__restrict__ b, double *out, size_t n)
+{
+	const size_t idx = (size_t)blockIdx.x * blockDim.x + threadIdx.x;
+	if (idx < n) out[idx] = a[idx] + b[idx];
+}
+
 __global__ void k_accept(const double *sc, int *cyc, const int *stop)
 {
 	if (threadIdx.x || blockIdx.x || (stop && *stop)) return;
@@ -836,6 +793,38 @@
 	if (idx >= nq + np || (stop && *stop)) return;
 	if (idx < nq) qdst[idx] = cyc[1] ? q_if_accepted[idx] : q_otherwise[idx];
 	else { idx -= nq; pdst[idx] = cyc[1] ? p_if_accepted[idx] : p_otherwise[idx]; }
+}
+
+constexpr int SELECT_UNROLL = 4;
+__global__ __launch_bounds__(MCHIP_BLOCK) void k_accept_select_copy(const double *__restrict__ in1, const double *__restrict__ in2, int n, double *sc, int *cyc,
+		double *qdst, const double *__restrict__ q_if_accepted, const double *__restrict__ q_otherwise, size_t nq,
+		double *pdst, const double *__restrict__ p_if_accepted, const double *__restrict__ p_otherwise, size_t np, const int *stop)
+{
+	__shared__ double red[MCHIP_BLOCK];
+	if (stop && *stop) return;
+	const double v1 = in1 ? block_ordered_sum(in1, n, red) : sc[1];
+	const double v2 = block_ordered_sum(in2, n, red);
+	const bool accept = !cyc[0] && v2 > v1;
+	if (blockIdx.x == 0 && threadIdx.x == 0) {
+		if (in1) sc[1] = v1;
+		sc[2] = v2;
+		cyc[1] = accept ? 1 : 0;
+	}
+	const double *qsrc = accept ? q_if_accepted : q_otherwise, *psrc = accept ? p_if_accepted : p_otherwise;
+	const size_t n_all = nq + np, turn = (size_t)gridDim.x * MCHIP_BLOCK;
+	for (size_t base = (size_t)blockIdx.x * MCHIP_BLOCK + threadIdx.x; base < n_all; base += SELECT_UNROLL * turn) {
+		double v[SELECT_UNROLL];
+#pragma unroll
+		for (int y = 0; y < SELECT_UNROLL; y++) {
+			const size_t idx = base + (size_t)y * turn;
+			if (idx < n_all) v[y] = idx < nq ? qsrc[idx] : psrc[idx - nq];
+		}
+#pragma unroll
+		for (int y = 0; y < SELECT_UNROLL; y++) {
+			const size_t idx = base + (size_t)y * turn;
+			if (idx < n_all) { if (idx < nq) qdst[idx] = v[y]; else pdst[idx - nq] = v[y]; }
+		}
+	}
 }
 
 int check_slot(mchip_context *ctx, int slot)
@@ -858,60 +847,28 @@
 	if (start) ctx->ev_kind.push_back(kind);
 }
 
-constexpr size_t PAIR_SPAN_CHUNK = 1024;
-constexpr int PAIR_SPAN_THREADS = 1024;
-__global__ __launch_bounds__(PAIR_SPAN_THREADS) void k_pair_spans(const unsigned long long *__restrict__ marks, unsigned n_blocks, mchip_pair_runs runs,
-								  mchip_pair_span *out)
-{
-	__shared__ unsigned long long red[4][PAIR_SPAN_THREADS];
-	unsigned long long lo[2] = { ~0ull, ~0ull }, hi[2] = { 0ull, 0ull };
-	for (unsigned r = threadIdx.x; r < n_blocks / MCHIP_PAIR_RUN; r += PAIR_SPAN_THREADS) {
-		unsigned logical;
-		const int kind = mchip_pair_is_ind(r * MCHIP_PAIR_RUN, runs, &logical) ? 1 : 0;
-#pragma unroll
-		for (int x = 0; x < MCHIP_PAIR_RUN; x++) {
-			const size_t b = (size_t)r * MCHIP_PAIR_RUN + x;
-			const unsigned long long t0 = marks[2 * b], t1 = marks[2 * b + 1];
-			if (t0 > t1) continue;
-			lo[kind] = t0 < lo[kind] ? t0 : lo[kind];
-			hi[kind] = t1 > hi[kind] ? t1 : hi[kind];
-		}
-	}
-	red[0][threadIdx.x] = lo[0]; red[1][threadIdx.x] = lo[1]; red[2][threadIdx.x] = hi[0]; red[3][threadIdx.x] = hi[1];
-	__syncthreads();
-	for (int s = PAIR_SPAN_THREADS / 2; s > 0; s >>= 1) {
-		if ((int)threadIdx.x < s) {
-			for (int x = 0; x < 2; x++) {
-				const unsigned long long l2 = red[x][threadIdx.x + s], h2 = red[2 + x][threadIdx.x + s];
-				if (l2 < red[x][threadIdx.x]) red[x][threadIdx.x] = l2;
-				if (h2 > red[2 + x][threadIdx.x]) red[2 + x][threadIdx.x] = h2;
-			}
-		}
-		__syncthreads();
-	}
-	if (threadIdx.x == 0) {
-		out->start[0] = red[0][0]; out->start[1] = red[1][0];
-		out->end[0] = red[2][0]; out->end[1] = red[3][0];
-	}
-}
-
-static int pair_profile_slot(mchip_context *ctx, const mchip_pass_args &a, unsigned long long **marks)
-{
-	mchip_pair_runs runs;
-	const size_t n_blocks = ctx->kt->pair_blocks(a, &runs);
-	if (n_blocks > ctx->pair_marks_cap) {
-		HIPCHK(hipStreamSynchronize(ctx->stream));
-		dfree(ctx->d_pair_marks);
-		ctx->pair_marks_cap = 0;
-		HIPCHK(hipMalloc((void **)&ctx->d_pair_marks, 2 * n_blocks * sizeof(unsigned long long)));
-		ctx->pair_marks_cap = n_blocks;
-	}
+constexpr size_t PAIR_SPAN_CHUNK = 64;
+
+static hipError_t pair_spans_reset(mchip_pair_span *chunk, size_t n)
+{
+	mchip_pair_span fresh;
+	memset(&fresh, 0, sizeof fresh);
+	for (int x = 0; x < 2; x++)
+		for (int w = 0; w < MCHIP_SPAN_WAYS; w++) fresh.way[x][w].start = ~0ull;
+	const std::vector<mchip_pair_span> init(n, fresh);
+	return MCHIP_WAIT(hipMemcpy(chunk, init.data(), n * sizeof(mchip_pair_span), hipMemcpyHostToDevice));
+}
+
+static int pair_profile_slot(mchip_context *ctx, mchip_pair_span **span)
+{
 	if (ctx->pair_used / PAIR_SPAN_CHUNK >= ctx->pair_spans.size()) {
 		mchip_pair_span *chunk = nullptr;
 		HIPCHK(hipMalloc((void **)&chunk, PAIR_SPAN_CHUNK * sizeof(mchip_pair_span)));
 		ctx->pair_spans.push_back(chunk);
-	}
-	*marks = ctx->d_pair_marks;
+		HIPCHK(pair_spans_reset(chunk, PAIR_SPAN_CHUNK));
+	}
+	*span = ctx->pair_spans[ctx->pair_used / PAIR_SPAN_CHUNK] + ctx->pair_used % PAIR_SPAN_CHUNK;
+	ctx->pair_used++;
 	return MCHIP_OK;
 }
 
@@ -1038,6 +995,8 @@
 	    MCHIP_WAIT(hipMalloc((void **)&ctx->d_scalars, 64 * sizeof(double))) != hipSuccess ||
 	    MCHIP_WAIT(hipMalloc((void **)&ctx->d_run, sizeof(mchip_run_state))) != hipSuccess ||
 	    MCHIP_WAIT(hipMalloc((void **)&ctx->d_cyc, 4 * sizeof(int))) != hipSuccess ||
+	    MCHIP_WAIT(hipMalloc((void **)&ctx->d_ticket, 2 * TICKET_WORDS * sizeof(unsigned))) != hipSuccess ||
+	    MCHIP_WAIT(hipMemset(ctx->d_ticket, 0, 2 * TICKET_WORDS * sizeof(unsigned))) != hipSuccess ||
 	    MCHIP_WAIT(hipEventCreate(&ctx->ev_begin)) != hipSuccess || MCHIP_WAIT(hipEventCreate(&ctx->ev_end)) != hipSuccess) {
 		delete ctx;
 		return MCHIP_ERR_ALLOC;
@@ -1056,10 +1015,10 @@
 	free_data(ctx);
 	dfree(ctx->d_scalars);
 	dfree(ctx->d_cyc);
+	dfree(ctx->d_ticket);
 	dfree(ctx->d_run);
 	if (ctx->h_pinned) (void)MCHIP_WAIT(hipHostFree(ctx->h_pinned));
 	for (hipEvent_t e : ctx->ev_pool) (void)MCHIP_WAIT(hipEventDestroy(e));
-	dfree(ctx->d_pair_marks);
 	for (mchip_pair_span *&chunk : ctx->pair_spans) dfree(chunk);
 	(void)MCHIP_WAIT(hipEventDestroy(ctx->ev_begin));
 	(void)MCHIP_WAIT(hipEventDestroy(ctx->ev_end));
@@ -1700,26 +1659,20 @@
 static int run_estep(mchip_context *ctx, int from, int to, int do_mstep, const int *stop = nullptr, const int *skip_ind = nullptr,
 		     bool defer_ll = false)
 {
+	ctx->stop_folded = 0;
 	if (!ctx->admixture) return run_mixture(ctx, from, to, do_mstep, 0, stop, -1, defer_ll);
 	mchip_pass_args a = pass_args(ctx, from);
 	a.stop = stop;
 	a.skip_ind = skip_ind;
 	const bool s_cached = ctx->sparse && do_mstep && !stop && ctx->s_cache_slot == from;
-	const bool paired = do_mstep && !s_cached && !ctx->knob.no_pair && ctx->kt->pair_available(a);
+	const bool paired = do_mstep && !s_cached && !ctx->knob.no_pair && !(skip_ind && !ctx->knob.pair_cached) && ctx->kt->pair_available(a);
 	if (paired) {
-		unsigned long long *marks = nullptr;
+		mchip_pair_span *span = nullptr;
 		if (ctx->profiling) {
-			int rc = pair_profile_slot(ctx, a, &marks);
+			int rc = pair_profile_slot(ctx, &span);
 			if (rc) return rc;
 		}
-		ctx->kt->estep_pair(a, marks, ctx->stream);
-		if (marks) {
-			mchip_pair_runs runs;
-			const unsigned n_blocks = ctx->kt->pair_blocks(a, &runs);
-			hipLaunchKernelGGL(k_pair_spans, dim3(1), dim3(PAIR_SPAN_THREADS), 0, ctx->stream, marks, n_blocks, runs,
-					   ctx->pair_spans[ctx->pair_used / PAIR_SPAN_CHUNK] + ctx->pair_used % PAIR_SPAN_CHUNK);
-			ctx->pair_used++;
-		}
+		ctx->kt->estep_pair(a, span, ctx->stream);
 		ctx->ll_parts = ctx->kt->ind_ll_parts(a);
 		if (!defer_ll)
 			hipLaunchKernelGGL(k_reduce_sum, dim3(1), dim3(MCHIP_BLOCK), 0, ctx->stream, ctx->d_llpart, ctx->ll_parts, ctx->d_scalars, stop);
@@ -1749,8 +1702,11 @@
 		p.L = ctx->L; p.K = ctx->K; p.T = ctx->T; p.loci_per_block = p_loci; p.n_slabs = n_slabs; p.weighted = 1;
 		p.do_projection = ctx->do_projection; p.toff = ctx->d_toff; p.Apart = ctx->d_Apart; p.Pfrom = ctx->d_p[from];
 		p.Pto = ctx->d_p[to]; p.add_lb = 0.0; p.lb = ctx->p_lb;
+		const bool fold = defer_ll && stop && !ctx->knob.no_fold;
+		const mchip_stop_fold f = { ctx->d_run, ctx->d_scalars, ctx->d_llpart, ctx->ll_parts, ctx->d_ticket };
 		ctx->kt->finalize_qp(ctx->I, s_slabs, ctx->d_Spart, ctx->d_q[from], ctx->qstride, ctx->d_q[to], ctx->d_sik,
-				     ctx->do_projection, ctx->eta_lb, p, stop, ctx->stream);
+				     ctx->do_projection, ctx->eta_lb, p, stop, fold ? &f : nullptr, ctx->stream);
+		ctx->stop_folded = fold ? 1 : 0;
 		ctx->empty_rows_nan[to] = 1;
 		HIPCHK(hipGetLastError());
 		ctx->have_ll = 1;
@@ -1777,6 +1733,12 @@
 	return MCHIP_OK;
 }
 
+static void stop_check_after(mchip_context *ctx)
+{
+	if (ctx->stop_folded) return;
+	hipLaunchKernelGGL(k_stop_check, dim3(1), dim3(MCHIP_BLOCK), 0, ctx->stream, ctx->d_run, ctx->d_scalars, ctx->d_llpart, ctx->ll_parts);
+}
+
 int mchip_em_run(mchip_context *ctx, int slot, int n_steps, mchip_run_state *state)
 {
 	MCHIP_ENTRY();
@@ -1792,7 +1754,7 @@
 		hipGraph_t graph = nullptr;
 		if (MCHIP_WAIT(hipStreamBeginCapture(ctx->stream, hipStreamCaptureModeThreadLocal)) == hipSuccess) {
 			rc = run_estep(ctx, slot, slot, 1, stop, nullptr, true);
-			hipLaunchKernelGGL(k_stop_check, dim3(1), dim3(MCHIP_BLOCK), 0, ctx->stream, ctx->d_run, ctx->d_scalars, ctx->d_llpart, ctx->ll_parts);
+			stop_check_after(ctx);
 			const hipError_t e = MCHIP_WAIT(hipStreamEndCapture(ctx->stream, &graph));
 			if (rc || e != hipSuccess || !graph || MCHIP_WAIT(hipGraphInstantiate(&ctx->step_graph[slot], graph, nullptr, nullptr, 0)) != hipSuccess)
 				ctx->step_graph[slot] = nullptr;
@@ -1807,7 +1769,7 @@
 			continue;
 		}
 		if ((rc = run_estep(ctx, slot, slot, 1, stop, nullptr, true))) return rc;
-		hipLaunchKernelGGL(k_stop_check, dim3(1), dim3(MCHIP_BLOCK), 0, ctx->stream, ctx->d_run, ctx->d_scalars, ctx->d_llpart, ctx->ll_parts);
+		stop_check_after(ctx);
 	}
 	HIPCHK(hipGetLastError());
 	HIPCHK(hipMemcpyAsync(state, ctx->d_run, sizeof *state, hipMemcpyDeviceToHost, ctx->stream));
@@ -2236,9 +2198,9 @@
 	const size_t KT = (size_t)ctx->K * ctx->T, nq = (size_t)ctx->nq;
 	int rc;
 	if ((rc = run_estep(ctx, A, B, 1, stop, cyc + 1, true))) return rc;
-	hipLaunchKernelGGL(k_stop_check, dim3(1), dim3(MCHIP_BLOCK), 0, ctx->stream, ctx->d_run, ctx->d_scalars, ctx->d_llpart, ctx->ll_parts);
+	stop_check_after(ctx);
 	if ((rc = run_estep(ctx, B, C, 1, stop, nullptr, true))) return rc;
-	hipLaunchKernelGGL(k_stop_check, dim3(1), dim3(MCHIP_BLOCK), 0, ctx->stream, ctx->d_run, ctx->d_scalars, ctx->d_llpart, ctx->ll_parts);
+	stop_check_after(ctx);
 	mchip_pass_args dual = pass_args(ctx, B);
 	dual.stop = stop;
 	dual.P2 = ctx->d_p[C];
@@ -2259,13 +2221,27 @@
 		const int gq = (int)((ctx->nq + 4095) / 4096) > 512 ? 512 : (int)((ctx->nq + 4095) / 4096);
 		const int gp = (int)((KT + 4095) / 4096) > 512 ? 512 : (int)((KT + 4095) / 4096);
 		double *part_q = ctx->d_redpart, *part_p = ctx->d_redpart + 3 * 512;
-		hipLaunchKernelGGL(k_dots_slots, dim3(gq + gp), dim3(MCHIP_BLOCK), 0, ctx->stream, ctx->d_q[A], ctx->d_q[B], ctx->d_q[C], nq, part_q, (unsigned)gq,
-				   ctx->d_p[A], ctx->d_p[B], ctx->d_p[C], KT, part_p, stop);
-		hipLaunchKernelGGL(k_reduce_dots_step, dim3(1), dim3(MCHIP_BLOCK), 0, ctx->stream, part_q, gq, part_p, gp, ctx->d_scalars, scheme, cyc, stop);
-	}
-	hipLaunchKernelGGL(k_accel_update_slots, dim3(nblk(nq + KT)), dim3(256), 0, ctx->stream, ctx->d_q[A], ctx->d_q[B], ctx->d_q[C], ctx->d_q[B], nq,
-			   ctx->d_p[A], ctx->d_p[B], ctx->d_p[C], ctx->d_p[B], KT, scheme == 4, ctx->d_scalars + 24, stop);
-	if ((rc = project_slot(ctx, B, stop))) return rc;
+		if (!ctx->knob.no_fold) {
+			hipLaunchKernelGGL(k_dots_slots, dim3(gq + gp), dim3(MCHIP_BLOCK), 0, ctx->stream, ctx->d_q[A], ctx->d_q[B], ctx->d_q[C], nq, part_q, (unsigned)gq,
+					   ctx->d_p[A], ctx->d_p[B], ctx->d_p[C], KT, part_p, stop, ctx->d_ticket + TICKET_WORDS, mchip_ticket_group((unsigned)(gq + gp)), ctx->d_scalars, scheme, cyc);
+		} else {
+			hipLaunchKernelGGL(k_dots_slots, dim3(gq + gp), dim3(MCHIP_BLOCK), 0, ctx->stream, ctx->d_q[A], ctx->d_q[B], ctx->d_q[C], nq, part_q, (unsigned)gq,
+					   ctx->d_p[A], ctx->d_p[B], ctx->d_p[C], KT, part_p, stop, (unsigned *)nullptr, 1u, (double *)nullptr, 0, (int *)nullptr);
+			hipLaunchKernelGGL(k_reduce_dots_step, dim3(1), dim3(MCHIP_BLOCK), 0, ctx->stream, part_q, gq, part_p, gp, ctx->d_scalars, scheme, cyc, stop);
+		}
+	}
+	if (!ctx->knob.no_fold) {
+		mchip_update_args u;
+		u.nrows = ctx->qstride ? ctx->I : 1; u.L = ctx->L; u.K = ctx->K; u.qn_form = scheme == 4; u.do_projection = ctx->do_projection;
+		u.q0 = ctx->d_q[A]; u.q1 = ctx->d_q[B]; u.q2 = ctx->d_q[C]; u.p0 = ctx->d_p[A]; u.p1 = ctx->d_p[B]; u.p2 = ctx->d_p[C];
+		u.toff = ctx->d_toff; u.lb_q = ctx->eta_lb; u.lb_p = ctx->p_lb; u.flags = ctx->d_flags; u.s_dev = ctx->d_scalars + 24; u.stop = stop;
+		ctx->kt->update_project(u, ctx->stream);
+		HIPCHK(hipGetLastError());
+	} else {
+		hipLaunchKernelGGL(k_accel_update_slots, dim3(nblk(nq + KT)), dim3(256), 0, ctx->stream, ctx->d_q[A], ctx->d_q[B], ctx->d_q[C], ctx->d_q[B], nq,
+				   ctx->d_p[A], ctx->d_p[B], ctx->d_p[C], ctx->d_p[B], KT, scheme == 4, ctx->d_scalars + 24, stop);
+		if ((rc = project_slot(ctx, B, stop))) return rc;
+	}
 	if (!ctx->admixture) {
 		if ((rc = run_mixture(ctx, B, B, 0, 1, stop, 2))) return rc;
 	} else {
@@ -2280,6 +2256,14 @@
 			ctx->kt->accum_q(a, ctx->stream);
 			prof_mark(ctx, MCHIP_KERN_ACCUM_Q, false);
 		}
+	}
+	if (ctx->admixture && !ctx->knob.no_fold) {
+		const size_t want = nblk(nq + KT, MCHIP_BLOCK * SELECT_UNROLL), cap = 3 * (size_t)ctx->n_cu;
+		hipLaunchKernelGGL(k_accept_select_copy, dim3((unsigned)(want < cap ? want : cap)), dim3(MCHIP_BLOCK), 0, ctx->stream,
+				   use_dual ? ctx->d_llpart2 : (const double *)nullptr, ctx->d_llpart, ctx->kt->ind_ll_parts(dual), ctx->d_scalars, cyc,
+				   ctx->d_q[A], ctx->d_q[B], ctx->d_q[C], nq, ctx->d_p[A], ctx->d_p[B], ctx->d_p[C], KT, stop);
+		HIPCHK(hipGetLastError());
+		return MCHIP_OK;
 	}
 	if (ctx->admixture)
 		hipLaunchKernelGGL(k_reduce_accept, dim3(1), dim3(MCHIP_BLOCK), 0, ctx->stream, use_dual ? ctx->d_llpart2 : (const double *)nullptr, ctx->d_llpart,
@@ -2364,6 +2348,11 @@
 	ctx->profiling = 1;
 	ctx->ev_used = 0;
 	ctx->ev_kind.clear();
+	if (ctx->pair_used) {
+		HIPCHK(hipStreamSynchronize(ctx->stream));
+		for (size_t p = 0; p < ctx->pair_used; p += PAIR_SPAN_CHUNK)
+			HIPCHK(pair_spans_reset(ctx->pair_spans[p / PAIR_SPAN_CHUNK], ctx->pair_used - p < PAIR_SPAN_CHUNK ? ctx->pair_used - p : PAIR_SPAN_CHUNK));
+	}
 	ctx->pair_used = 0;
 	HIPCHK(hipEventRecord(ctx->ev_begin, ctx->stream));
 	return MCHIP_OK;
@@ -2394,10 +2383,16 @@
 		for (size_t p = 0; p < ctx->pair_used; p += PAIR_SPAN_CHUNK) {
 			const size_t n = ctx->pair_used - p < PAIR_SPAN_CHUNK ? ctx->pair_used - p : PAIR_SPAN_CHUNK;
 			HIPCHK(hipMemcpy(&spans[p], ctx->pair_spans[p / PAIR_SPAN_CHUNK], n * sizeof(mchip_pair_span), hipMemcpyDeviceToHost));
+			HIPCHK(pair_spans_reset(ctx->pair_spans[p / PAIR_SPAN_CHUNK], n));
 		}
 		for (const mchip_pair_span &sp : spans)
 			for (int x = 0; x < 2; x++) {
-				each.push_back(sp.end[x] > sp.start[x] ? (float)((double)(sp.end[x] - sp.start[x]) / khz) : 0.0f);
+				unsigned long long start = ~0ull, end = 0ull;
+				for (int w = 0; w < MCHIP_SPAN_WAYS; w++) {
+					if (sp.way[x][w].start < start) start = sp.way[x][w].start;
+					if (sp.way[x][w].end > end) end = sp.way[x][w].end;
+				}
+				each.push_back(end > start ? (float)((double)(end - start) / khz) : 0.0f);
 				kind_of.push_back(x ? MCHIP_KERN_ACCUM_Q : MCHIP_KERN_ACCUM_P);
 			}
 		ctx->pair_used = 0;
diff --git a/multiclust_amd/csrc/mchip_context.h b/multiclust_amd/csrc/mchip_context.h
--- a/multiclust_amd/csrc/mchip_context.h
+++ b/multiclust_amd/csrc/mchip_context.h
@@ -76,6 +76,8 @@
 	struct {
 		int no_bial, no_counts, force_dense, force_safe, no_graph, no_dual, no_slab_sum, no_col_split, part_no_tile, sim_no_tile;
 		int no_fused_finalize, no_pair;
+		int no_fold;
+		int pair_cached;
 		int per_cu_col, per_cu_ind, geometry_given, no_roundup;
 		double slab_frac;
 	} knob;
@@ -88,6 +90,8 @@
 	hipGraphExec_t step_graph[3];
 	hipGraphExec_t cycle_graph[3][5];
 	int *d_cyc;
+	unsigned *d_ticket;
+	int stop_folded;
 	int have_ll;
 	int ll_parts;
 	int s_cache_slot;
@@ -96,8 +100,6 @@
 	std::vector<hipEvent_t> ev_pool;
 	std::vector<int> ev_kind;
 	size_t ev_used;
-	unsigned long long *d_pair_marks;
-	size_t pair_marks_cap;
 	std::vector<mchip_pair_span *> pair_spans;
 	size_t pair_used;
 };
diff --git a/multiclust_amd/csrc/mchip_finalize.h b/multiclust_amd/csrc/mchip_finalize.h
--- a/multiclust_amd/csrc/mchip_finalize.h
+++ b/multiclust_amd/csrc/mchip_finalize.h
@@ -59,6 +59,125 @@
 	}
 }
 
+__device__ __forceinline__ double ordered_sum(double acc, const double *__restrict__ in, size_t first, size_t stride, int count)
+{
+	int x = 0;
+	for (; x + 8 <= count; x += 8) {
+		double v[8];
+#pragma unroll
+		for (int y = 0; y < 8; y++) v[y] = in[first + (size_t)(x + y) * stride];
+#pragma unroll
+		for (int y = 0; y < 8; y++) acc += v[y];
+	}
+	for (; x < count; x++) acc += in[first + (size_t)x * stride];
+	return acc;
+}
+
+__device__ __forceinline__ void stop_check_body(mchip_run_state *s, double *ll, const double *__restrict__ part, int n, double *red)
+{
+	if (part) {
+		const double acc = (int)threadIdx.x < n ? ordered_sum(0.0, part, threadIdx.x, MCHIP_BLOCK, (n - (int)threadIdx.x + MCHIP_BLOCK - 1) / MCHIP_BLOCK) : 0.0;
+		red[threadIdx.x] = acc;
+		__syncthreads();
+		for (int w = MCHIP_BLOCK / 2; w > 0; w >>= 1) {
+			if ((int)threadIdx.x < w) red[threadIdx.x] += red[threadIdx.x + w];
+			__syncthreads();
+		}
+		if (threadIdx.x == 0) *ll = red[0];
+	}
+	if (threadIdx.x) return;
+	const double loglik = part ? red[0] : *ll;
+	s->n_iter++;
+	if (loglik != loglik) {
+		s->fatal = 1;
+		s->bad_loglik = loglik;
+		s->stopped = 1;
+		return;
+	}
+	int stop;
+	if (s->max_iter && s->n_iter > s->max_iter) {
+		s->iter_stop = 1;
+		stop = 1;
+	} else {
+		double abs_diff = 0, rel_diff = 0;
+		stop = 1;
+		if (s->abs_error != 0) abs_diff = fabs(loglik - s->logL);
+		if (s->rel_error != 0) rel_diff = abs_diff / fabs(s->logL);
+		if (s->abs_error != 0 && abs_diff > s->abs_error) stop = 0;
+		if (s->rel_error != 0 && rel_diff > s->rel_error) stop = 0;
+		if (stop) s->converged = 1;
+	}
+	s->stopped = stop;
+	if (loglik < s->logL && !stop) {
+		s->fatal = 2;
+		s->bad_loglik = loglik;
+		s->stopped = 1;
+		return;
+	}
+	s->logL = loglik;
+}
+
+__device__ __forceinline__ bool last_ticket(unsigned *ticket, unsigned group, int *flag, bool fence)
+{
+	if (threadIdx.x == 0) {
+		if (fence) {
+			__threadfence();
+			asm volatile("s_waitcnt vmcnt(0)" ::: "memory");
+		}
+		const unsigned g = blockIdx.x / group, n_groups = (gridDim.x + group - 1) / group;
+		const unsigned mine = g + 1 < n_groups ? group : gridDim.x - g * group;
+		unsigned *own = ticket + (size_t)(1 + g) * MCHIP_TICKET_STRIDE;
+		bool last = false;
+		if (atomicAdd(own, 1u) == mine - 1) {
+			*own = 0u;
+			last = atomicAdd(ticket, 1u) == n_groups - 1;
+			if (last) *ticket = 0u;
+		}
+		*flag = last ? 1 : 0;
+	}
+	__syncthreads();
+	const bool last = *flag != 0;
+	if (last && fence) __threadfence();
+	return last;
+}
+
+__device__ __forceinline__ double accel_extrapolate(double x0, double x1, double x2, double s, int qn_form)
+{
+#pragma clang fp contract(off)
+	const double u = x1 - x0, v = x2 - x1;
+	if (qn_form) return x0 + u + s * v;
+	return x0 - 2 * s * u + s * s * (v - u);
+}
+
+template <bool EXTRAPOLATE>
+__device__ __forceinline__ void project_p_thread(int l, int k, int K, const int32_t *__restrict__ toff, double *P, double lb, uint8_t *flags,
+		int do_projection, const double *__restrict__ p0, const double *__restrict__ p2, double s, int qn_form)
+{
+	const int c0 = toff[l], M = toff[l + 1] - c0;
+	if (M <= 8) {
+		double v[8];
+#pragma unroll
+		for (int m = 0; m < 8; m++) {
+			v[m] = 0.0;
+			if (m < M) {
+				const size_t e = (size_t)(c0 + m) * K + k;
+				v[m] = EXTRAPOLATE ? accel_extrapolate(p0[e], P[e], p2[e], s, qn_form) : P[e];
+			}
+		}
+		if (do_projection) michelot_small(v, M, lb);
+#pragma unroll
+		for (int m = 0; m < 8; m++)
+			if (m < M) P[(size_t)(c0 + m) * K + k] = v[m];
+		return;
+	}
+	if (EXTRAPOLATE)
+		for (int m = 0; m < M; m++) {
+			const size_t e = (size_t)(c0 + m) * K + k;
+			P[e] = accel_extrapolate(p0[e], P[e], p2[e], s, qn_form);
+		}
+	if (do_projection) michelot_strided(P + (size_t)c0 * K + k, K, M, lb, flags ? flags + (size_t)c0 * K + k : nullptr);
+}
+
 constexpr int FP_TILE = 1024;
 __device__ __forceinline__ void finalize_p_tile_body(int block, double *tile, int L, int K, int T, const int32_t *__restrict__ toff, int loci_per_block,
 		int n_slabs, const double *__restrict__ Apart, const double *Pfrom, double *Pto,
diff --git a/multiclust_amd/csrc/mchip_internal.h b/multiclust_amd/csrc/mchip_internal.h
--- a/multiclust_amd/csrc/mchip_internal.h
+++ b/multiclust_amd/csrc/mchip_internal.h
@@ -103,7 +103,10 @@
 	*logical = (ind ? before : run - before) * MCHIP_PAIR_RUN + block % MCHIP_PAIR_RUN;
 	return ind;
 }
-struct mchip_pair_span { unsigned long long start[2], end[2]; };
+#define MCHIP_SPAN_WAYS 64
+struct mchip_pair_span {
+	struct { unsigned long long start, end, pad[30]; } way[2][MCHIP_SPAN_WAYS];
+};
 
 struct mchip_finalize_p_args {
 	int L, K, T, loci_per_block, n_slabs, weighted, do_projection;
@@ -111,6 +114,36 @@
 	const double *Apart, *Pfrom;
 	double *Pto;
 	double add_lb, lb;
+};
+
+#define MCHIP_TICKET_STRIDE 32
+#define MCHIP_TICKET_GROUPS 4096
+inline unsigned mchip_ticket_group(unsigned n_blocks)
+{
+	unsigned g = 1;
+	while ((unsigned long long)g * g < n_blocks) g++;
+	const unsigned least = (n_blocks + MCHIP_TICKET_GROUPS - 1) / MCHIP_TICKET_GROUPS;
+	return g > least ? g : (least ? least : 1);
+}
+
+struct mchip_stop_fold {
+	mchip_run_state *run;
+	double *ll;
+	const double *part;
+	int n_parts;
+	unsigned *ticket;
+	unsigned group;
+};
+
+struct mchip_update_args {
+	int nrows, L, K, qn_form, do_projection;
+	const double *q0, *q2, *p0, *p2;
+	double *q1, *p1;
+	const int32_t *toff;
+	double lb_q, lb_p;
+	uint8_t *flags;
+	const double *s_dev;
+	const int *stop;
 };
 
 struct mchip_ktable {
@@ -133,10 +166,12 @@
 	int (*ind_slabs)(const mchip_pass_args &a);
 	int (*ind_ll_parts)(const mchip_pass_args &a);
 	void (*finalize_qp)(int I, int n_slabs_q, const double *Spart, const double *Qfrom, int qstride_from, double *Qto, double *sik,
-			    int do_projection_q, double lb_q, const mchip_finalize_p_args &p, const int *stop, hipStream_t s);
+			    int do_projection_q, double lb_q, const mchip_finalize_p_args &p, const int *stop, const mchip_stop_fold *fold,
+			    hipStream_t s);
 	int (*pair_available)(const mchip_pass_args &a);
 	unsigned (*pair_blocks)(const mchip_pass_args &a, mchip_pair_runs *runs);
-	void (*estep_pair)(const mchip_pass_args &a, unsigned long long *marks, hipStream_t s);
+	void (*estep_pair)(const mchip_pass_args &a, mchip_pair_span *span, hipStream_t s);
+	void (*update_project)(const mchip_update_args &u, hipStream_t s);
 };
 
 const mchip_ktable *mchip_get_ktable(int K);
diff --git a/multiclust_amd/csrc/mchip_kernels_k.hip b/multiclust_amd/csrc/mchip_kernels_k.hip
--- a/multiclust_amd/csrc/mchip_kernels_k.hip
+++ b/multiclust_amd/csrc/mchip_kernels_k.hip
@@ -1076,7 +1076,7 @@
 }
 
 template <int BITS, int PL, bool SAFE, bool NOMISS>
-__global__ __launch_bounds__(MCHIP_BLOCK) void k_estep_pair(mchip_pass_args a, mchip_pair_runs runs, unsigned long long *marks)
+__global__ __launch_bounds__(MCHIP_BLOCK) void k_estep_pair(mchip_pass_args a, mchip_pair_runs runs, mchip_pair_span *span)
 {
 	static_assert(64 * MCHIP_IND_WAVES_MAX == MCHIP_BLOCK, "both bodies at 256 threads");
 	extern __shared__ __attribute__((aligned(16))) double lds[];
@@ -1084,17 +1084,11 @@
 	const bool ind = mchip_pair_is_ind(blockIdx.x, runs, &logical);
 	const unsigned n_col = (unsigned)((a.T + 63) / 64), n_mine = ind ? (unsigned)(((a.I + 63) / 64) * mchip_ind_slabs(a)) : n_col * (unsigned)mchip_col_slabs(a);
 	const bool idle = logical >= n_mine || (a.stop && *a.stop) || (ind && a.skip_ind && *a.skip_ind);
-	if (idle) {
-		if (marks && threadIdx.x == 0) {
-			marks[2 * (size_t)blockIdx.x] = ~0ull;
-			marks[2 * (size_t)blockIdx.x + 1] = 0ull;
-		}
-		return;
-	}
-	const unsigned long long t_start = marks ? __builtin_amdgcn_s_memrealtime() : 0ull;
+	if (idle) return;
+	const unsigned long long t_start = span ? __builtin_amdgcn_s_memrealtime() : 0ull;
 	if (ind) individual_sparse_w_body<PL, true, SAFE, NOMISS, false>(a, logical, lds);
 	else column_counts_body<BITS, false, SAFE>(a, (int)(logical % n_col), (int)(logical / n_col), reinterpret_cast<double (*)[64]>(lds));
-	if (marks) {
+	if (span) {
 		unsigned long long (*wave_mark)[MCHIP_COL_WAVES] = reinterpret_cast<unsigned long long (*)[MCHIP_COL_WAVES]>(lds);
 		if ((threadIdx.x & 63) == 0) {
 			wave_mark[0][threadIdx.x >> 6] = t_start;
@@ -1107,8 +1101,8 @@
 				t0 = wave_mark[0][w] < t0 ? wave_mark[0][w] : t0;
 				t1 = wave_mark[1][w] > t1 ? wave_mark[1][w] : t1;
 			}
-			marks[2 * (size_t)blockIdx.x] = t0;
-			marks[2 * (size_t)blockIdx.x + 1] = t1;
+			atomicMin(&span->way[ind ? 1 : 0][blockIdx.x % MCHIP_SPAN_WAYS].start, t0);
+			atomicMax(&span->way[ind ? 1 : 0][blockIdx.x % MCHIP_SPAN_WAYS].end, t1);
 		}
 	}
 }
@@ -1569,15 +1563,45 @@
 }
 __global__ __launch_bounds__(MCHIP_BLOCK) void k_finalize_qp(int q_blocks, int I, int n_lchunks, const double *__restrict__ Spart,
 		const double *__restrict__ Qfrom, int qstride_from, double *Qto, double *sik,
-		int do_projection_q, double lb_q, mchip_finalize_p_args p, const int *stop)
+		int do_projection_q, double lb_q, mchip_finalize_p_args p, const int *stop, mchip_stop_fold fold)
 {
 	__shared__ double lds[FQ_XCH > FP_TILE ? FQ_XCH : FP_TILE];
+	__shared__ int last;
+	static_assert(FP_TILE >= MCHIP_BLOCK, "the stopping rule's tree fits the tile");
 	if (stop && *stop) return;
 	if ((int)blockIdx.x < q_blocks)
 		finalize_q_body(blockIdx.x, lds, I, n_lchunks, Spart, Qfrom, qstride_from, Qto, sik, 1, 1, do_projection_q, lb_q, 0.0);
 	else
 		finalize_p_tile_body((int)blockIdx.x - q_blocks, lds, p.L, p.K, p.T, p.toff, p.loci_per_block, p.n_slabs, p.Apart, p.Pfrom, p.Pto,
 				     p.weighted, p.add_lb, p.do_projection, p.lb);
+	if (!fold.run) return;
+	__syncthreads();
+	if (!last_ticket(fold.ticket, fold.group, &last, false)) return;
+	if (fold.run->stopped) return;
+	stop_check_body(fold.run, fold.ll, fold.part, fold.n_parts, lds);
+}
+
+__global__ __launch_bounds__(MCHIP_BLOCK) void k_update_project(int q_blocks, mchip_update_args u)
+{
+	if (u.stop && *u.stop) return;
+	const double s = *u.s_dev;
+	if ((int)blockIdx.x < q_blocks) {
+		const int i = blockIdx.x * MCHIP_BLOCK + threadIdx.x;
+		if (i >= u.nrows) return;
+		double x[K];
+#pragma unroll
+		for (int k = 0; k < K; k++) {
+			const size_t e = (size_t)i * K + k;
+			x[k] = accel_extrapolate(u.q0[e], u.q1[e], u.q2[e], s, u.qn_form);
+		}
+		if (u.do_projection) michelot_k(x, u.lb_q);
+#pragma unroll
+		for (int k = 0; k < K; k++) u.q1[(size_t)i * K + k] = x[k];
+		return;
+	}
+	const size_t idx = (size_t)(blockIdx.x - q_blocks) * MCHIP_BLOCK + threadIdx.x;
+	if (idx >= (size_t)u.L * K) return;
+	project_p_thread<true>((int)(idx / K), (int)(idx % K), K, u.toff, u.p1, u.lb_p, u.flags, u.do_projection, u.p0, u.p2, s, u.qn_form);
 }
 
 __global__ __launch_bounds__(MCHIP_BLOCK) void k_project_q(int nrows, double *Q, double lb, const int *stop)
@@ -1704,16 +1728,16 @@
 	if (r.col_runs == 0 || r.ind_runs == 0) return 0;
 	return (unsigned long long)(r.col_runs + r.ind_runs) * r.ind_runs < (1ull << 32);
 }
-void launch_estep_pair(const mchip_pass_args &a, unsigned long long *marks, hipStream_t s)
+void launch_estep_pair(const mchip_pass_args &a, mchip_pair_span *span, hipStream_t s)
 {
 	if constexpr (K <= 12 && SPLIT == 1 && CSPLIT == 1) {
 		mchip_pair_runs r;
 		const dim3 grid(pair_blocks(a, &r)), block(MCHIP_BLOCK);
 		const size_t ind_lds = coop_lds_bytes(a, 1), col_lds = (size_t)K * 64 * sizeof(double);
 		const size_t lds = ind_lds > col_lds ? ind_lds : col_lds;
-		if (a.flush_blocks < 1) hipLaunchKernelGGL((k_estep_pair<2, 2, true, false>), grid, block, lds, s, a, r, marks);
-		else if (!a.has_missing) hipLaunchKernelGGL((k_estep_pair<2, 2, false, true>), grid, block, lds, s, a, r, marks);
-		else hipLaunchKernelGGL((k_estep_pair<2, 2, false, false>), grid, block, lds, s, a, r, marks);
+		if (a.flush_blocks < 1) hipLaunchKernelGGL((k_estep_pair<2, 2, true, false>), grid, block, lds, s, a, r, span);
+		else if (!a.has_missing) hipLaunchKernelGGL((k_estep_pair<2, 2, false, true>), grid, block, lds, s, a, r, span);
+		else hipLaunchKernelGGL((k_estep_pair<2, 2, false, false>), grid, block, lds, s, a, r, span);
 	}
 }
 int col_slabs(const mchip_pass_args &a, int mix)
@@ -1783,11 +1807,20 @@
 			   I, n_lchunks, Spart, Qfrom, qstride_from, Qto, sik, do_mstep, weighted, do_projection, lb, stop, add);
 }
 void launch_finalize_qp(int I, int n_lchunks, const double *Spart, const double *Qfrom, int qstride_from, double *Qto, double *sik,
-			int do_projection_q, double lb_q, const mchip_finalize_p_args &p, const int *stop, hipStream_t s)
+			int do_projection_q, double lb_q, const mchip_finalize_p_args &p, const int *stop, const mchip_stop_fold *fold, hipStream_t s)
 {
 	const int q_blocks = (I + FQ_IND - 1) / FQ_IND, p_blocks = (p.L + p.loci_per_block - 1) / p.loci_per_block;
+	mchip_stop_fold f = { nullptr, nullptr, nullptr, 0, nullptr, 1 };
+	if (fold) f = *fold;
+	f.group = mchip_ticket_group((unsigned)(q_blocks + p_blocks));
 	hipLaunchKernelGGL(k_finalize_qp, dim3(q_blocks + p_blocks), dim3(MCHIP_BLOCK), 0, s,
-			   q_blocks, I, n_lchunks, Spart, Qfrom, qstride_from, Qto, sik, do_projection_q, lb_q, p, stop);
+			   q_blocks, I, n_lchunks, Spart, Qfrom, qstride_from, Qto, sik, do_projection_q, lb_q, p, stop, f);
+}
+void launch_update_project(const mchip_update_args &u, hipStream_t s)
+{
+	const int q_blocks = (u.nrows + MCHIP_BLOCK - 1) / MCHIP_BLOCK;
+	const size_t p_blocks = ((size_t)u.L * K + MCHIP_BLOCK - 1) / MCHIP_BLOCK;
+	hipLaunchKernelGGL(k_update_project, dim3((unsigned)(q_blocks + p_blocks)), dim3(MCHIP_BLOCK), 0, s, q_blocks, u);
 }
 void launch_project_q(int nrows, int, double *Q, double lb, const int *stop, hipStream_t s)
 {
@@ -1803,7 +1836,7 @@
 	static mchip_ktable t = {
 		launch_accum_p, launch_loglik, launch_accum_q, launch_part_p, launch_part_q, launch_finalize_q, launch_project_q,
 		launch_mix_gather, launch_mix_finalize, launch_mix_column, dual_available, launch_accum_q_dual,
-		col_slabs, ind_slabs, ind_ll_parts, launch_finalize_qp, pair_available, pair_blocks, launch_estep_pair,
+		col_slabs, ind_slabs, ind_ll_parts, launch_finalize_qp, pair_available, pair_blocks, launch_estep_pair, launch_update_project,
 	};
 	return &t;
 }
```
